# Fireflies-17/Speech-Inpainting

Measured on AMD Instinct MI355X. Metric: real-time factor (audio-sec/wall-sec) per GPU, 4 s clips @16 kHz, 200 ms mask, higher is better.
Workload: dtype encoder GEMMs and attention products: bf16 MFMA, fp32 accumulate (softmax, LayerNorm, head, arg-max in fp32); vocoder: fp16 MFMA (operands rounded to fp16, saturating), fp32 accumulate, activations stored as fp16; 1 GPU; BASELINE configs[1]: batch=32 x 4 s clips per GPU, 200 ms mask, HuBERT-base + HiFi-GAN V1; step = masked log-mel front-end -> encoder -> arg-max/splice -> vocoder on resident raw clips; global_batch=32, clip_samples=64000, mask_frames=10, parallelism=utterance-sharded x1

## Files before the change

### include/si_hip.h

```cpp
#ifndef SI_HIP_H
#define SI_HIP_H

#include <stddef.h>
#include <stdint.h>

#ifdef __cplusplus
extern "C" {
#endif

#define SI_ABI_VERSION 3

enum {
    SI_OK = 0,
    SI_EINVAL = -1,
    SI_ENOMEM = -2,
    SI_EHIP = -3,
    SI_ESTATE = -4,
    SI_EWEIGHTS = -5
};

enum {
    SI_MATH_F32 = 0,
    SI_MATH_BF16 = 1,
    SI_MATH_BF16X3 = 2,
// ... 224 lines not shown
    const int32_t* host_k0;
    const int32_t* host_k1;
    const int32_t* start;
    const int32_t* len;
    const int32_t* span_win;
    const int32_t* span_lim;
    const int32_t* win_ctx;
    const int32_t* win_start;
    const int32_t* win_len;
    const int32_t* chunk;
    const int32_t* k0;
    const int32_t* k1;
    const float* ramp;
} si_region_table;

int si_patch_regions(si_ctx* ctx, const float* orig, int N22, const si_region_table* table, const float* gen, int Lrow, const float* gain,
                     float* out_f32, int16_t* out_pcm, si_stream_t stream);

#define SI_SAMPLE_F32 0
#define SI_SAMPLE_S16 1
#define SI_SAMPLE_S24 2

int si_quiet_runs(si_ctx* ctx, const void* x, int is_pcm16, int n, float threshold, int min_len, int32_t* runs, int max_runs,
                  int32_t* n_runs, si_stream_t stream);

typedef struct si_rate_table {
    int32_t struct_size;
    int32_t num_contexts;
    int32_t num_windows;
    int32_t num_spans;
    int32_t num_chunks;
    int32_t fade;
    const int32_t* host_start;
    const int32_t* host_len;
    const int32_t* host_span_win;
    const int32_t* host_span_lim;
    const int32_t* host_win_ctx;
    const int32_t* host_win_start;
    const int32_t* host_win_len;
    const int32_t* host_win_lim;
    const int32_t* host_chunk;
    const int32_t* host_k0;
    const int32_t* host_k1;
    const int32_t* start;
    const int32_t* len;
    const int32_t* span_win;
    const int32_t* span_lim;
    const int32_t* win_ctx;
    const int32_t* win_start;
    const int32_t* win_len;
    const int32_t* win_lim;
    const int32_t* chunk;
    const int32_t* k0;
    const int32_t* k1;
    const float* ramp;
} si_rate_table;

int si_patch_rate(si_ctx* ctx, const void* orig, int is_pcm16, int n_file, int sr, const si_rate_table* table, const float* gen, int Lrow,
                  const float* gain, const si_sinc_filter* filt, void* out, si_stream_t stream);

#define SI_CUT_RATE_TILE 512
int si_cut_rate(si_ctx* ctx, const void* x, int is_pcm16, int n_file, int sr, const int32_t* host_start, const int32_t* start, int C, int L,
                const si_sinc_filter* filt, float* out, si_stream_t stream);

#define SI_MAX_CHANNELS 8
int si_quiet_runs_ch(si_ctx* ctx, const void* x, int is_pcm16, int n, int channels, int channel, float threshold, int min_len, int32_t* runs,
                     int max_runs, int32_t* n_runs, si_stream_t stream);
int si_cut_rate_ch(si_ctx* ctx, const void* x, int is_pcm16, int n_file, int channels, int channel, int sr, const int32_t* host_start,
                   const int32_t* start, int C, int L, const si_sinc_filter* filt, float* out, si_stream_t stream);
int si_patch_rate_ch(si_ctx* ctx, const void* orig, int is_pcm16, int n_file, int channels, int channel, int sr, const si_rate_table* table,
                     const float* gen, int Lrow, const float* gain, const si_sinc_filter* filt, void* out, si_stream_t stream);

#define SI_CUT_PAIR_FRAMES 1
int si_cut_pair(si_ctx* ctx, const void* x, int is_pcm16, int n_file, int sr, const int32_t* host_frame, const int32_t* frame, int C, int L22,
                int L16, const si_sinc_filter* filt22, const si_sinc_filter* filt16, float* out22, float* out16, si_stream_t stream);
int si_cut_pair_ch(si_ctx* ctx, const void* x, int is_pcm16, int n_file, int channels, int channel, int sr, const int32_t* host_frame,
                   const int32_t* frame, int C, int L22, int L16, const si_sinc_filter* filt22, const si_sinc_filter* filt16, float* out22,
                   float* out16, si_stream_t stream);

#define SI_DEAD_QUIET 1
#define SI_DEAD_HELD 2
int si_dead_runs(si_ctx* ctx, const void* x, int is_pcm16, int n, int channels, int channel, int kind, float threshold, float rel_threshold,
                 float held_tol, int min_len, int32_t* runs, int max_runs, int32_t* n_runs, float* threshold_out, si_stream_t stream);

#define SI_LEVEL_MAX_HALF 1024
int si_level_runs(si_ctx* ctx, const void* x, int is_pcm16, int n, int channels, int channel, int half, float threshold, float rel_threshold,
                  int min_len, int32_t* runs, int max_runs, int32_t* n_runs, float* threshold_out, si_stream_t stream);

int si_burst_runs(si_ctx* ctx, const void* x, int is_pcm16, int n, int channels, int channel, int half, float threshold, float rel_threshold,
                  int min_len, int32_t* runs, int max_runs, int32_t* n_runs, float* threshold_out, si_stream_t stream);

int si_invalid_runs(si_ctx* ctx, const void* x, int is_pcm16, int n, int channels, int channel, float ceiling, int min_len, int32_t* runs,
                    int max_runs, int32_t* n_runs, si_stream_t stream);
int si_cut_rate_valid(si_ctx* ctx, const void* x, int is_pcm16, int n_file, int channels, int channel, int sr, const int32_t* host_start,
                      const int32_t* start, int C, int L, const si_sinc_filter* filt, float ceiling, float* out, si_stream_t stream);
int si_cut_pair_valid(si_ctx* ctx, const void* x, int is_pcm16, int n_file, int channels, int channel, int sr, const int32_t* host_frame,
                      const int32_t* frame, int C, int L22, int L16, const si_sinc_filter* filt22, const si_sinc_filter* filt16, float ceiling,
                      float* out22, float* out16, si_stream_t stream);
int si_cut_clips_valid(si_ctx* ctx, const float* src, int n_src, const int32_t* host_start, const int32_t* start, int C, int L, float ceiling,
                       float* out, si_stream_t stream);

#define SI_IMPULSE_MAX_ORDER 32
#define SI_IMPULSE_MAX_HALF 1024
#define SI_IMPULSE_MAX_GUARD 64
#define SI_IMPULSE_MAX_PAD 16
int si_impulse_runs(si_ctx* ctx, const void* x, int is_pcm16, int n, int channels, int channel, int order, int half, int guard, int pad,
                    float ratio, float threshold, float rel_threshold, int min_len, int32_t* runs, int max_runs, int32_t* n_runs,
                    float* threshold_out, si_stream_t stream);
int si_impulse_residual(si_ctx* ctx, const void* x, int is_pcm16, int n, int channels, int channel, int order, double* e, si_stream_t stream);

#define SI_MEND_MAX_LEN 64
#define SI_MEND_MAX_ORDER 32
#define SI_MEND_MAX_CONTEXT 1024
#define SI_MEND_MAX_RUNS 65536
#define SI_MEND_LONG 0
#define SI_MEND_AR 1
#define SI_MEND_LINE 2
#define SI_MEND_EDGE 3
#define SI_MEND_NEAR 4
#define SI_MEND_NONFINITE 5
#define SI_MEND_BADROW 6
int si_mend_runs(si_ctx* ctx, void* x, int is_pcm16, int n, int channels, int channel, const int32_t* runs, int n_runs, int max_len,
                 int order, int context, int32_t* status, si_stream_t stream);

int si_num_frames(const si_ctx* ctx, int N);
int si_vocoder_samples(const si_ctx* ctx, int Tm, int stretch);

typedef struct si_profile_entry {
    char name[48];
    int32_t launches;
    int32_t reserved;
    double ms;
    double flops;
    double bytes;
} si_profile_entry;
int si_profile_start(si_ctx* ctx, int max_launches);
int si_profile_filter(si_ctx* ctx, const char* family);
int si_profile_stop(si_ctx* ctx, si_profile_entry* out, int capacity, int* count);

int si_debug_capture(si_ctx* ctx, const char* name, float* dst, long capacity);
long si_debug_size(si_ctx* ctx, const char* name);

#define SI_WS_ENCODER 0
#define SI_WS_VOCODER 1
#define SI_WS_MEL 2
#define SI_WS_MAX_REGIONS 32
typedef struct si_ws_region {
    char name[24];
    uint64_t offset;
    uint64_t bytes;
} si_ws_region;
int si_debug_ws_regions(si_ctx* ctx, int which, si_ws_region* out, int capacity, int* count);

#ifdef __cplusplus
}
#endif
#endif
```

### speech_inpainting_amd/csrc/api.hip

```cpp
#include <cmath>
#include <cstdarg>
#include <cstdio>
#include <cstdlib>
#include <cstring>
#include <map>
#include <sstream>
#include <string>
#include <vector>

#include "common.h"

using namespace siw;

struct si_ctx {
    int device = 0;
    si_model_desc d{};
    char err[512] = {0};
    Layout lay;
    char* wdev = nullptr;
    bool weights_ready = false;
    bool weights_verified = false;
    std::map<std::string, long> dbg_size;
    std::map<std::string, std::pair<float*, long>> dbg_capture;
    struct ProfRec { int name; hipEvent_t a, b; double flops, bytes; };
    bool prof_on = false;
    std::string prof_filter;
    std::vector<std::string> prof_names;
    std::vector<ProfRec> prof_recs;
    std::vector<hipEvent_t> prof_pool;
    size_t prof_used = 0;
    int prof_open = -1;
    int num_cus = 0;
    std::map<const void*, size_t> dyn_lds;
    PackOpts popt;
    bool opt_enc_opready = true, opt_att_bf16 = true, opt_enc_lingemm = true;
    bool opt_enc_posconv = true;
    int opt_ln_fuse = 1;
    int opt_voc_upsgemm = 1;
    int opt_ffn_pad = 64;
    int opt_gemmcu = 1;
    int opt_voc_chain = 1;
    int opt_voc_fuse = 1;
    char* fe_dev = nullptr;
    size_t fe_dft = 0, fe_hann = 0, fe_basis = 0, fe_lo = 0, fe_hi = 0;
    std::vector<int32_t> vl_host;
    static constexpr int VL_SLOTS = 4;
    int32_t* vl_pin[VL_SLOTS] = {nullptr, nullptr, nullptr, nullptr};
    size_t vl_pin_ints[VL_SLOTS] = {0, 0, 0, 0};
    hipEvent_t vl_ev[VL_SLOTS] = {nullptr, nullptr, nullptr, nullptr};
    int vl_next = 0;
    float* km_cnorm = nullptr;
    int km_cnorm_cap = 0;
    char* det_scratch = nullptr;
    size_t det_scratch_cap = 0;
    size_t ws_zone = 0;
    struct WsRegion { const char* name; size_t offset, bytes; };
    struct WsLog { int n = 0; WsRegion r[SI_WS_MAX_REGIONS]; };
    WsLog ws_log[3];
};

int si_fail(si_ctx* ctx, int code, const char* fmt, ...) {
    char* dst = ctx ? ctx->err : g_create_err;
    va_list ap;
    va_start(ap, fmt);
    vsnprintf(dst, 512, fmt, ap);
    va_end(ap);
    return code;
}
int si_fail_hip(si_ctx* ctx, hipError_t e, const char* what, const char* file, int line) {
    return si_fail(ctx, SI_EHIP, "HIP error %d (%s) at %s:%d: %s", (int)e, hipGetErrorString(e), file, line, what);
}

struct TapSrc { const void* p; long n; int esize = 4; long cols = 0, ld = 0; };
static int si_tap(si_ctx* ctx, hipStream_t st, TapSrc s, const char* fmt, int a = 0, int b = 0, int c = 0) {
    if (ctx->dbg_capture.empty() && strchr(fmt, '%')) return SI_OK;
    char name[48];
    snprintf(name, sizeof(name), fmt, a, b, c);
    ctx->dbg_size[name] = s.n;
    auto it = ctx->dbg_capture.find(name);
    if (it == ctx->dbg_capture.end()) return SI_OK;
    const long m = s.n < it->second.second ? s.n : it->second.second;
    if (m <= 0) return SI_OK;
    if (s.ld > s.cols && s.cols > 0) {
        if (m / s.cols > 0)
            SI_HIP_CHECK(hipMemcpy2DAsync(it->second.first, (size_t)s.cols * s.esize, s.p, (size_t)s.ld * s.esize, (size_t)s.cols * s.esize,
                                          (size_t)(m / s.cols), hipMemcpyDeviceToDevice, st));
    } else {
        SI_HIP_CHECK(hipMemcpyAsync(it->second.first, s.p, (size_t)m * s.esize, hipMemcpyDeviceToDevice, st));
    }
    return SI_OK;
}

void si_prof_begin(si_ctx* ctx, const char* name, double flops, double bytes, hipStream_t st) {
    if (!ctx->prof_on || ctx->prof_used + 2 > ctx->prof_pool.size()) { ctx->prof_open = -1; return; }
    if (!ctx->prof_filter.empty() && ctx->prof_filter != name) { ctx->prof_open = -1; return; }
    int id = -1;
    for (size_t i = 0; i < ctx->prof_names.size(); ++i) if (ctx->prof_names[i] == name) { id = (int)i; break; }
    if (id < 0) { id = (int)ctx->prof_names.size(); ctx->prof_names.push_back(name); }
    si_ctx::ProfRec r{id, ctx->prof_pool[ctx->prof_used], ctx->prof_pool[ctx->prof_used + 1], flops, bytes};
    ctx->prof_used += 2;
    (void)hipEventRecord(r.a, st);
    ctx->prof_open = (int)ctx->prof_recs.size();
    ctx->prof_recs.push_back(r);
}
const char* si_prof_shape_name(const char* name, long M, int N, int K) {
    static const bool on = getenv("SI_PROF_SHAPES") && atoi(getenv("SI_PROF_SHAPES")) != 0;
    if (!on) return name;
    static thread_local char buf[48];
    snprintf(buf, sizeof(buf), "%s_%ldx%dx%d", name, M, N, K);
    return buf;
}
int si_ensure_dyn_lds(si_ctx* ctx, const void* kern, size_t bytes) {
    if (bytes <= 64 * 1024) return SI_OK;
    size_t& have = ctx->dyn_lds[kern];
    if (bytes > have) {
        SI_HIP_CHECK(hipFuncSetAttribute(kern, hipFuncAttributeMaxDynamicSharedMemorySize, (int)bytes));
        have = bytes;
    }
    return SI_OK;
}
int si_opt_gemmcu(const si_ctx* ctx) { return ctx->opt_gemmcu; }
int si_num_cus(si_ctx* ctx) {
    if (ctx->num_cus <= 0) {
        int n = 0;
        if (hipDeviceGetAttribute(&n, hipDeviceAttributeMultiprocessorCount, ctx->device) != hipSuccess || n <= 0) n = 256;
        ctx->num_cus = n;
    }
    return ctx->num_cus;
}
static int vl_upload(si_ctx* ctx, int32_t* dst, hipStream_t st) {
    const size_t n = ctx->vl_host.size();
    const int slot = ctx->vl_next;
    ctx->vl_next = (slot + 1) % si_ctx::VL_SLOTS;
    if (!ctx->vl_ev[slot]) SI_HIP_CHECK(hipEventCreateWithFlags(&ctx->vl_ev[slot], hipEventDisableTiming));
    else SI_HIP_CHECK(hipEventSynchronize(ctx->vl_ev[slot]));
    if (ctx->vl_pin_ints[slot] < n) {
        if (ctx->vl_pin[slot]) SI_HIP_CHECK(hipHostFree(ctx->vl_pin[slot]));
        ctx->vl_pin[slot] = nullptr; ctx->vl_pin_ints[slot] = 0;
        SI_HIP_CHECK(hipHostMalloc(reinterpret_cast<void**>(&ctx->vl_pin[slot]), std::max<size_t>(n, 4096) * sizeof(int32_t), hipHostMallocDefault));
        ctx->vl_pin_ints[slot] = std::max<size_t>(n, 4096);
    }
    memcpy(ctx->vl_pin[slot], ctx->vl_host.data(), n * sizeof(int32_t));
    SI_HIP_CHECK(hipMemcpyAsync(dst, ctx->vl_pin[slot], n * sizeof(int32_t), hipMemcpyHostToDevice, st));
    SI_HIP_CHECK(hipEventRecord(ctx->vl_ev[slot], st));
    return SI_OK;
}
void si_prof_end(si_ctx* ctx, hipStream_t st) {
    if (ctx->prof_open < 0) return;
    (void)hipEventRecord(ctx->prof_recs[ctx->prof_open].b, st);
    ctx->prof_open = -1;
}

namespace {

int stage_channels(const si_ctx* ctx, int i) { return siw::stage_channels(ctx->d, ctx->popt, i); }
BlobHeader blob_header(const si_ctx* ctx) { return siw::blob_header(ctx->d, ctx->popt, ctx->lay); }
Err ctx_err(si_ctx* ctx) { return ctx ? Err{ctx->err, sizeof(ctx->err)} : Err{g_create_err, sizeof(g_create_err)}; }

inline size_t align_up(size_t v, size_t a) { return (v + a - 1) / a * a; }

struct Carver {
    char* base; size_t cap; size_t zone; si_ctx::WsLog* log; size_t cur; bool ok = true;
    const char* failed = "";
    float* floats(size_t n, const char* name) { return reinterpret_cast<float*>(bytes(n * 4, name)); }
    char* bytes(size_t n, const char* name) {
        size_t o = cur; cur = align_up(cur + n, 256) + zone;
        if (cur > cap || log->n >= SI_WS_MAX_REGIONS) { if (ok) failed = name; ok = false; return base; }
        log->r[log->n++] = {name, o, n};
        return base + o;
    }
};
Carver carver(si_ctx* ctx, int which, void* workspace, size_t workspace_bytes) {
    ctx->ws_log[which].n = 0;
    return Carver{static_cast<char*>(workspace), workspace_bytes, ctx->ws_zone, &ctx->ws_log[which], ctx->ws_zone};
}
constexpr int ENC_WS_ZONES = 18, VOC_WS_ZONES = 15, MEL_WS_ZONES = 5;

struct VlTable { const int32_t* host = nullptr; int32_t* dev = nullptr; };
template <class Fill>
int vl_table(si_ctx* ctx, Carver& W, size_t ints, hipStream_t st, const char* what, VlTable& t, Fill fill) {
    ctx->vl_host.assign(ints, 0);
    if (int rc = fill(ctx->vl_host.data())) return rc;
    t.dev = reinterpret_cast<int32_t*>(W.bytes(ints * 4, "lengths"));
    if (!W.ok) return si_fail(ctx, SI_ENOMEM, "internal: %s workspace carve exceeded its own estimate at region '%s'", what, W.failed);
    if (int rc = vl_upload(ctx, t.dev, st)) return rc;
    t.host = ctx->vl_host.data();
    return SI_OK;
}

struct EncDims { int T; std::vector<int> L; };
EncDims enc_dims(const si_model_desc& d, int N) {
    EncDims e; e.L.push_back(N);
    int n = N;
    for (int i = 0; i < d.num_conv; ++i) { n = n >= d.conv_kernel[i] ? (n - d.conv_kernel[i]) / d.conv_stride[i] + 1 : 0; e.L.push_back(n); }
    e.T = n;
    return e;
}

size_t encoder_ws_bytes(const si_ctx* ctx, int B, int N) {
    const si_model_desc& d = ctx->d;
    EncDims e = enc_dims(d, N);
    size_t cmax = 0;
    for (int i = 0; i < d.num_conv; ++i) cmax = std::max(cmax, (size_t)e.L[i + 1] * d.conv_dim[i]);
    const size_t BT = (size_t)B * std::max(e.T, 1);
    size_t f = 2 * (size_t)B * cmax + BT * d.conv_dim[d.num_conv - 1] + BT * d.hidden_size * 3 + BT * 3 * d.hidden_size + BT * d.intermediate_size +
               (size_t)B * d.conv_dim[0] * 2 + BT * 2;
    const size_t h16 = (BT * d.conv_dim[d.num_conv - 1] + 2 * BT * d.hidden_size + BT * (d.intermediate_size + 128)) * 2;
    return f * 4 + h16 + (size_t)B * 16 + (size_t)B * 4 + si_conv0_partials_bytes(B, N) + 41 * 256 +
           align_up((size_t)(SI_MAX_CONV + 3) * (B + 1) * 4, 256) +
           ENC_WS_ZONES * ctx->ws_zone;
}

int vocoder_chunk(const si_model_desc& d, int B) { int c = d.vocoder_chunk > 0 ? d.vocoder_chunk : 32; return std::min(c, std::max(B, 1)); }

long voc_tout(int Tm, int stretch) { return stretch ? (long)std::floor((double)Tm * (441.0 / 256.0)) : Tm; }

size_t vocoder_ws_bytes(const si_ctx* ctx, int B, int Tm, int stretch) {
    const si_model_desc& d = ctx->d;
    const int Bc = vocoder_chunk(d, B);
    const long Tout = voc_tout(Tm, stretch);
    size_t lc_max = (size_t)Tout * d.up_initial_channel;
    long L = Tout; int c = d.up_initial_channel;
    for (int i = 0; i < d.num_ups; ++i) { L *= d.up_rates[i]; c = stage_channels(ctx, i); lc_max = std::max(lc_max, (size_t)L * c); }
    const size_t f = (size_t)Bc * Tout * ctx->lay.mel_ld + 9 * (size_t)Bc * lc_max;
    return f * 4 + 32 * 256 + align_up((size_t)(2 * SI_MAX_UPS + 3) * B * 4, 256) +
           VOC_WS_ZONES * ctx->ws_zone;
}

TapGemmParams gemm_params(const si_ctx* ctx, const GemmW& G) {
    TapGemmParams p{};
    p.w = ctx->wdev + G.w;
    p.w_lo = G.math == SI_MATH_BF16X3 ? ctx->wdev + G.w_lo : nullptr;
    p.bias = G.has_bias ? reinterpret_cast<const float*>(ctx->wdev + G.bias) : nullptr;
    p.Cin = G.Cin; p.N = G.N; p.Npad = G.Npad; p.ntaps = G.ntaps; p.groups = G.groups;
    p.stride = 1; p.dil = 1; p.pad = 0; p.pro_slope = 1.f; p.act = SI_ACT_NONE; p.alpha = 1.f; p.accumulate = 0;
    p.out16_slope = 1.f;
    p.nseg = 1;
    return p;
}

struct UpsGeom { int u, pad; long Lout; int M; };
UpsGeom ups_geom(const si_model_desc& d, int i, long Lin) {
    const int u = d.up_rates[i], pad = (d.up_kernels[i] - u) / 2;
    const long Lout = Lin * u;
    return UpsGeom{u, pad, Lout, (int)((pad + Lout - 1) / u + 1)};
}

struct ResLn { const float* stats = nullptr; const float* gamma = nullptr; const float* beta = nullptr; };
struct LinearIo { const unsigned short* x16 = nullptr; unsigned short* y16 = nullptr; int ld_in = 0, ld_out = 0; ResLn res_ln; };
int linear(si_ctx* ctx, const GemmW& G, const float* x, float* y, long rows, int act, const float* res, hipStream_t st, const LinearIo& io = LinearIo()) {
    TapGemmParams p = gemm_params(ctx, G);
    p.x = io.x16 ? nullptr : x; p.x16 = io.x16; p.out = y; p.out16 = io.y16; p.res = res; p.act = act;
    p.res_stats = io.res_ln.stats; p.res_gamma = io.res_ln.gamma; p.res_beta = io.res_ln.beta;
    p.nseg = 1; p.Lin = (int)rows; p.M = (int)rows; p.ldx = io.ld_in ? io.ld_in : G.Cin; p.x_seg_stride = 0;
    p.ldo = io.ld_out ? io.ld_out : G.N; p.o_seg_stride = 0; p.ooff = 0; p.olimit = rows * p.ldo;
    p.lingemm = ctx->opt_enc_lingemm;
    return si_launch_tapgemm(ctx, G.math, p, st);
}

const float* wf(const si_ctx* ctx, size_t off) { return reinterpret_cast<const float*>(ctx->wdev + off); }

}

static int hubert_run(si_ctx* ctx, const float* wav, const int32_t* mask_start, const int32_t* mask_len, const int32_t* valid_len,
                      int normalize, float norm_eps, const double* pre_add, int output_layer, int B, int N, float* out_feats, float* out_hidden,
                      void* workspace, size_t workspace_bytes, si_stream_t stream, const int32_t* host_len = nullptr, const SiSpans* spans = nullptr);

static int check_span_table(si_ctx* ctx, const char* who, const si_span_table* t, int B, SiSpans& out) {
    if (!t || t->struct_size != (int32_t)sizeof(si_span_table)) return si_fail(ctx, SI_EINVAL, "%s: si_span_table size mismatch", who);
    if (!t->host_off || !t->span_off) return si_fail(ctx, SI_EINVAL, "%s: span table with NULL offsets", who);
    if (t->num_clips != B) return si_fail(ctx, SI_EINVAL, "%s: span table for %d clips, batch of %d", who, t->num_clips, B);
    if (t->host_off[0] != 0 || t->host_off[B] != t->num_spans || t->num_spans < 0)
        return si_fail(ctx, SI_EINVAL, "%s: span offsets run 0 .. %d but the table holds %d spans", who, t->host_off[B], t->num_spans);
    if (t->num_spans > 0 && (!t->host_start || !t->host_len || !t->span_start || !t->span_len))
        return si_fail(ctx, SI_EINVAL, "%s: span table with NULL start / len", who);
    for (int b = 0; b < B; ++b) {
        const int k0 = t->host_off[b], k1 = t->host_off[b + 1];
        if (k1 < k0 || k1 > t->num_spans) return si_fail(ctx, SI_EINVAL, "%s: span offsets of clip %d decrease or leave the table", who, b);
        if (k1 - k0 > SI_MAX_SPANS) return si_fail(ctx, SI_EINVAL, "%s: clip %d has %d spans, more than SI_MAX_SPANS = %d", who, b, k1 - k0, SI_MAX_SPANS);
        for (int k = k0; k < k1; ++k) {
            const long s = t->host_start[k], l = t->host_len[k];
            if (s < 0 || l < 0 || s + l > 0x7fffffffL) return si_fail(ctx, SI_EINVAL, "%s: clip %d span %d = [%ld, +%ld) is not a sample range", who, b, k - k0, s, l);
            if (k > k0 && s < (long)t->host_start[k - 1] + t->host_len[k - 1])
                return si_fail(ctx, SI_EINVAL, "%s: clip %d span %d overlaps or precedes span %d (spans must be sorted and disjoint)", who, b, k - k0, k - k0 - 1);
        }
    }
    out = SiSpans{t->span_off, t->span_start, t->span_len};
    return SI_OK;
}

extern "C" {

int si_version(void) { return SI_ABI_VERSION; }

const char* si_last_error(const si_ctx* ctx) { return ctx ? ctx->err : g_create_err; }

int si_create(si_ctx** out, int device_id, const si_model_desc* desc) {
    if (!out) return si_fail(nullptr, SI_EINVAL, "si_create: out is NULL");
    *out = nullptr;
    int rc = check_desc(desc, ctx_err(nullptr));
    if (rc) return rc;
    int ndev = 0;
    if (hipGetDeviceCount(&ndev) != hipSuccess || device_id < 0 || device_id >= ndev)
        return si_fail(nullptr, SI_EHIP, "si_create: device %d not available (%d HIP devices visible)", device_id, ndev);
    si_ctx* ctx = new si_ctx();
    ctx->device = device_id;
    ctx->d = *desc;
    ctx->popt = pack_opts_from_env();
    ctx->opt_voc_fuse = getenv("SI_VOC_FUSE") ? atoi(getenv("SI_VOC_FUSE")) : 1;
    ctx->opt_voc_chain = getenv("SI_VOC_CHAIN") ? atoi(getenv("SI_VOC_CHAIN")) : 1;
    ctx->opt_enc_opready = env_flag("SI_ENC_OPREADY");
    ctx->opt_att_bf16 = env_flag("SI_ATT_BF16");
    ctx->opt_enc_lingemm = env_flag("SI_ENC_LINGEMM");
    ctx->opt_enc_posconv = env_flag("SI_ENC_POSCONV");
    ctx->opt_gemmcu = getenv("SI_ENC_GEMMCU") ? atoi(getenv("SI_ENC_GEMMCU")) : 1;
    ctx->opt_ln_fuse = getenv("SI_ENC_LNFUSE") ? atoi(getenv("SI_ENC_LNFUSE")) : 1;
    ctx->opt_voc_upsgemm = getenv("SI_VOC_UPSGEMM") ? atoi(getenv("SI_VOC_UPSGEMM")) : 1;
    ctx->opt_ffn_pad = getenv("SI_ENC_FFNPAD") ? std::min(128, std::max(0, atoi(getenv("SI_ENC_FFNPAD")) / 8 * 8)) : 64;
    ctx->ws_zone = getenv("SI_WS_REDZONE") ? (size_t)std::min(1L << 20, std::max(0L, atol(getenv("SI_WS_REDZONE")))) / 256 * 256 : 0;
    plan_layout(ctx->d, ctx->popt, ctx->lay);
    *out = ctx;
    return SI_OK;
}

void si_destroy(si_ctx* ctx) {
    if (!ctx) return;
    if (ctx->wdev) { (void)hipSetDevice(ctx->device); (void)hipFree(ctx->wdev); }
    if (ctx->fe_dev) { (void)hipSetDevice(ctx->device); (void)hipFree(ctx->fe_dev); }
    if (ctx->km_cnorm) { (void)hipSetDevice(ctx->device); (void)hipFree(ctx->km_cnorm); }
    if (ctx->det_scratch) { (void)hipSetDevice(ctx->device); (void)hipFree(ctx->det_scratch); }
    for (hipEvent_t e : ctx->prof_pool) (void)hipEventDestroy(e);
    for (int i = 0; i < si_ctx::VL_SLOTS; ++i) {
        if (ctx->vl_ev[i]) { (void)hipEventSynchronize(ctx->vl_ev[i]); (void)hipEventDestroy(ctx->vl_ev[i]); }
        if (ctx->vl_pin[i]) (void)hipHostFree(ctx->vl_pin[i]);
    }
    delete ctx;
}

int si_alloc_weights(si_ctx* ctx) {
    if (!ctx) return SI_EINVAL;
    SI_HIP_CHECK(hipSetDevice(ctx->device));
    if (!ctx->wdev) SI_HIP_CHECK(hipMalloc(reinterpret_cast<void**>(&ctx->wdev), ctx->lay.total));
    ctx->weights_ready = true;
    ctx->weights_verified = false;
    return SI_OK;
}

int si_load_weights(si_ctx* ctx, const void* host_blob, size_t nbytes, const char* index) {
    if (!ctx || !host_blob || !index) return si_fail(ctx, SI_EINVAL, "si_load_weights: NULL argument");
    std::vector<char> image;
    int rc = pack_image(ctx->d, ctx->popt, ctx->lay, host_blob, nbytes, index, image, ctx_err(ctx));
    if (rc) return rc;
    SI_HIP_CHECK(hipSetDevice(ctx->device));
    if (!ctx->wdev) SI_HIP_CHECK(hipMalloc(reinterpret_cast<void**>(&ctx->wdev), ctx->lay.total));
    SI_HIP_CHECK(hipMemcpy(ctx->wdev, image.data(), ctx->lay.total, hipMemcpyHostToDevice));
    ctx->weights_ready = true;
    ctx->weights_verified = true;
    return SI_OK;
}

int si_weights_check(si_ctx* ctx) {
    if (!ctx) return SI_EINVAL;
    if (!ctx->wdev) return si_fail(ctx, SI_ESTATE, "weights are not allocated: call si_load_weights or si_alloc_weights first");
    SI_HIP_CHECK(hipSetDevice(ctx->device));
    BlobHeader got{};
    SI_HIP_CHECK(hipMemcpy(&got, ctx->wdev, sizeof(got), hipMemcpyDeviceToHost));
    const BlobHeader want = blob_header(ctx);
    if (got.magic != want.magic || got.version != want.version || got.fingerprint != want.fingerprint || got.total != want.total)
        return si_fail(ctx, SI_EWEIGHTS, "the weight blob in this context was packed for a different layout (fingerprint %016llx / %llu bytes, this "
                       "context plans %016llx / %llu): the source rank's model desc or SI_VOC_* environment differs, or the broadcast has not arrived",
                       (unsigned long long)got.fingerprint, (unsigned long long)got.total, (unsigned long long)want.fingerprint, (unsigned long long)want.total);
    ctx->weights_verified = true;
    return SI_OK;
}

int si_weights_device_ptr(si_ctx* ctx, void** ptr, size_t* nbytes) {
    if (!ctx || !ptr || !nbytes) return si_fail(ctx, SI_EINVAL, "si_weights_device_ptr: NULL argument");
    if (!ctx->wdev) return si_fail(ctx, SI_ESTATE, "weights are not allocated: call si_load_weights or si_alloc_weights first");
    *ptr = ctx->wdev;
    *nbytes = ctx->lay.total;
    return SI_OK;
}

int si_num_frames(const si_ctx* ctx, int N) { return ctx ? enc_dims(ctx->d, N).T : SI_EINVAL; }

int si_vocoder_samples(const si_ctx* ctx, int Tm, int stretch) {
    if (!ctx) return SI_EINVAL;
    long L = voc_tout(Tm, stretch);
    for (int i = 0; i < ctx->d.num_ups; ++i) L *= ctx->d.up_rates[i];
    return (int)L;
}

int si_workspace_bytes(si_ctx* ctx, int B, int N, int Tm, size_t* out) {
    if (!ctx || !out || B <= 0) return si_fail(ctx, SI_EINVAL, "si_workspace_bytes: bad argument");
    size_t a = N > 0 ? encoder_ws_bytes(ctx, B, N) : 0;
    size_t b = Tm > 0 ? vocoder_ws_bytes(ctx, B, Tm, 1) : 0;
    *out = std::max(a, b);
    return SI_OK;
}

int si_hubert_forward(si_ctx* ctx, const float* wav, const int32_t* mask_start, const int32_t* mask_len, int normalize, int B, int N,
                      float* out_feats, void* workspace, size_t workspace_bytes, si_stream_t stream) {
    return si_hubert_forward_padded(ctx, wav, mask_start, mask_len, nullptr, normalize, B, N, out_feats, workspace, workspace_bytes, stream);
}

int si_hubert_forward_padded(si_ctx* ctx, const float* wav, const int32_t* mask_start, const int32_t* mask_len, const int32_t* valid_len,
                             int normalize, int B, int N, float* out_feats, void* workspace, size_t workspace_bytes, si_stream_t stream) {
    if (!ctx) return SI_EINVAL;
    if (!out_feats) return si_fail(ctx, SI_EINVAL, "si_hubert_forward: NULL / empty argument");
    return hubert_run(ctx, wav, mask_start, mask_len, valid_len, normalize, 1e-7f, nullptr, 0, B, N, out_feats, nullptr, workspace,
                      workspace_bytes, stream);
}

int si_hubert_forward_varlen(si_ctx* ctx, const float* wav, const int32_t* mask_start, const int32_t* mask_len, const int32_t* sample_len,
                             int normalize, int B, int N, float* out_feats, void* workspace, size_t workspace_bytes, si_stream_t stream) {
    if (!ctx) return SI_EINVAL;
    if (!out_feats || !sample_len) return si_fail(ctx, SI_EINVAL, "si_hubert_forward_varlen: NULL argument");
    return hubert_run(ctx, wav, mask_start, mask_len, nullptr, normalize, 1e-7f, nullptr, 0, B, N, out_feats, nullptr, workspace, workspace_bytes,
                      stream, sample_len);
}

int si_hubert_extract_features(si_ctx* ctx, const si_extract_desc* x, const float* wav, const int32_t* mask_start, const int32_t* mask_len,
                               const double* pre_mask_add, int B, int N, float* out_hidden, void* workspace, size_t workspace_bytes,
                               si_stream_t stream) {
    if (!ctx) return SI_EINVAL;
    if (!x || x->struct_size != (int32_t)sizeof(si_extract_desc)) return si_fail(ctx, SI_EINVAL, "si_hubert_extract_features: si_extract_desc size mismatch");
    if (!out_hidden) return si_fail(ctx, SI_EINVAL, "si_hubert_extract_features: NULL output");
    if (x->output_layer < 1 || x->output_layer > ctx->d.num_layers)
        return si_fail(ctx, SI_EINVAL, "output_layer %d outside 1..%d", x->output_layer, ctx->d.num_layers);
    if (x->normalize < 0 || x->normalize > 2) return si_fail(ctx, SI_EINVAL, "normalize mode %d unknown (0 none, 1 processor, 2 layer_norm)", x->normalize);
    return hubert_run(ctx, wav, mask_start, mask_len, nullptr, x->normalize != 0, x->normalize == 2 ? 1e-5f : 1e-7f, pre_mask_add,
                      x->output_layer, B, N, nullptr, out_hidden, workspace, workspace_bytes, stream);
}

int si_hubert_forward_spans(si_ctx* ctx, const float* wav, const si_span_table* spans, const int32_t* sample_len, int normalize,
                            int B, int N, float* out_feats, void* workspace, size_t workspace_bytes, si_stream_t stream) {
    if (!ctx) return SI_EINVAL;
    if (!out_feats || B <= 0) return si_fail(ctx, SI_EINVAL, "si_hubert_forward_spans: NULL / empty argument");
    SiSpans sp;
    if (int rc = check_span_table(ctx, "si_hubert_forward_spans", spans, B, sp)) return rc;
    return hubert_run(ctx, wav, nullptr, nullptr, nullptr, normalize, 1e-7f, nullptr, 0, B, N, out_feats, nullptr, workspace, workspace_bytes,
                      stream, sample_len, &sp);
}

int si_code_splice(si_ctx* ctx, const int64_t* code_clean, const int64_t* code_masked, const int32_t* first, const int32_t* last, int B, int T,
                   int64_t* out, si_stream_t stream) {
    if (!ctx) return SI_EINVAL;
    if (!code_clean || !code_masked || !first || !last || !out || B <= 0 || T <= 0) return si_fail(ctx, SI_EINVAL, "si_code_splice: NULL / empty argument");
    SI_HIP_CHECK(hipSetDevice(ctx->device));
    return si_launch_code_splice(ctx, code_clean, code_masked, first, last, B, T, out, static_cast<hipStream_t>(stream));
}

}

static int hubert_run(si_ctx* ctx, const float* wav, const int32_t* mask_start, const int32_t* mask_len, const int32_t* valid_len,
                      int normalize, float norm_eps, const double* pre_add, int output_layer, int B, int N, float* out_feats, float* out_hidden,
                      void* workspace, size_t workspace_bytes, si_stream_t stream, const int32_t* host_len, const SiSpans* spans) {
    if (!ctx->weights_ready) return si_fail(ctx, SI_ESTATE, "si_hubert_forward before weights were loaded");
    if (!ctx->weights_verified) if (int rcw = si_weights_check(ctx)) return rcw;
    if (!wav || !workspace || B <= 0) return si_fail(ctx, SI_EINVAL, "si_hubert_forward: NULL / empty argument");
    const si_model_desc& d = ctx->d;
    const Layout& L = ctx->lay;
    hipStream_t st = static_cast<hipStream_t>(stream);
// ... 408 lines not shown
            int Tc = T, cin = d->in_width;
            for (int i = 0; i < d->down_t; ++i) {
                const int To = (Tc + 2 * ds.pad - ds.k) / d->stride_t + 1;
                macs += (double)B * To * d->width * (double)cin * ds.k + (double)d->depth * B * To * ((double)d->n_state * d->width * 3 + (double)d->width * d->n_state);
                Tc = To; cin = d->width;
            }
            macs += (double)B * Tc * d->out_width * (double)d->width * 3;
            const int frc = si_launch_f0enc_fused(ctx, weights, f0, B, T, h_out, d->in_width, d->out_width, d->width, d->n_state, d->depth, d->down_t,
                                                  d->stride_t, d->dilation_growth, ds.k, ds.pad, macs, st);
            if (frc <= 0) return frc;
        }
    }
    const size_t slot = need / 3 / sizeof(float);
    float* buf[3] = {static_cast<float*>(workspace), static_cast<float*>(workspace) + slot, static_cast<float*>(workspace) + 2 * slot};
    const float* w = weights;
    const float* x = f0;
    int cin = d->in_width, Tc = T, cur = -1;
    int rc;
    for (int i = 0; i < d->down_t; ++i) {
        const int To = (Tc + 2 * ds.pad - ds.k) / d->stride_t + 1;
        const float* cw = w; w += (size_t)d->width * cin * ds.k;
        const float* cb = w; w += d->width;
        const int o = (cur + 1) % 3;
        if ((rc = si_launch_small_conv1d(ctx, x, cw, cb, nullptr, buf[o], B, cin, Tc, d->width, To, ds.k, d->stride_t, 1, ds.pad, 0, 0, st))) return rc;
        cur = o; x = buf[cur]; cin = d->width; Tc = To;
        long dil = 1;
        for (int j = 0; j < d->depth; ++j) {
            const float* w3 = w; w += (size_t)d->n_state * d->width * 3;
            const float* b3 = w; w += d->n_state;
            const float* w1 = w; w += (size_t)d->width * d->n_state;
            const float* b1 = w; w += d->width;
            const int t1 = (cur + 1) % 3, t2 = (cur + 2) % 3;
            if ((rc = si_launch_small_conv1d(ctx, x, w3, b3, nullptr, buf[t1], B, d->width, Tc, d->n_state, Tc, 3, 1, (int)dil, (int)dil, 1, 0, st))) return rc;
            if ((rc = si_launch_small_conv1d(ctx, buf[t1], w1, b1, x, buf[t2], B, d->n_state, Tc, d->width, Tc, 1, 1, 1, 0, 1, 0, st))) return rc;
            cur = t2; x = buf[cur];
            dil *= d->dilation_growth;
            if (dil > (1 << 20)) return si_fail(ctx, SI_EINVAL, "si_f0_encoder_forward: dilation overflow");
        }
    }
    const float* fw = w; w += (size_t)d->out_width * d->width * 3;
    return si_launch_small_conv1d(ctx, x, fw, w, nullptr, h_out, B, d->width, Tc, d->out_width, Tc, 3, 1, 1, 1, 0, 1, st);
}

int si_unit_frontend(si_ctx* ctx, const int64_t* code, int Fc, const int64_t* f0_code, int Fp, const float* spk_emb, const float* emb_c,
                     int Kc, const float* emb_p, int Kp, int E, int B, float* out, si_stream_t stream) {
    if (!ctx) return SI_EINVAL;
    if (!code || !emb_c || !out || B <= 0 || Fc <= 0 || E <= 0 || Kc <= 0) return si_fail(ctx, SI_EINVAL, "si_unit_frontend: NULL / empty argument");
    if (f0_code && (!emb_p || Fp <= 0 || Kp <= 0)) return si_fail(ctx, SI_EINVAL, "si_unit_frontend: f0_code needs its embedding table");
    if (f0_code) {
        const int F = Fp > Fc ? Fp : Fc, s = Fp > Fc ? Fc : Fp;
        if (F % s) return si_fail(ctx, SI_EINVAL, "si_unit_frontend: %d and %d frames: misalignment between condition features", Fc, Fp);
    }
    SI_HIP_CHECK(hipSetDevice(ctx->device));
    return si_launch_unit_frontend(ctx, code, Fc, f0_code, Fp, spk_emb, emb_c, Kc, emb_p, Kp, E, B, out, static_cast<hipStream_t>(stream));
}

int si_resample_poly(si_ctx* ctx, const float* x, int B, int n_in, const float* taps, int ntaps, int up, int down,
                     int pre_remove, int n_out, float* y, si_stream_t stream) {
    if (!ctx) return SI_EINVAL;
    if (!x || !taps || !y || B <= 0 || n_in <= 0) return si_fail(ctx, SI_EINVAL, "si_resample_poly: NULL / empty argument");
    SI_HIP_CHECK(hipSetDevice(ctx->device));
    return si_launch_resample_poly(ctx, x, B, n_in, taps, ntaps, up, down, pre_remove, n_out, y, static_cast<hipStream_t>(stream));
}

static int hifigan_run(si_ctx* ctx, const float* mel, int B, int Tm, int stretch, float* wav_out, void* workspace,
                       size_t workspace_bytes, si_stream_t stream, const int32_t* host_len);

int si_resample_sinc(si_ctx* ctx, const float* x, const int32_t* n_len, int B, int n_in, const si_sinc_filter* f, int n_out, float* y,
                     si_stream_t stream) {
    if (!ctx) return SI_EINVAL;
    if (!x || !y || !f || !f->win || !f->dwin || !f->time_reg || B <= 0 || n_in <= 0) return si_fail(ctx, SI_EINVAL, "si_resample_sinc: NULL / empty argument");
    if (f->struct_size != (int32_t)sizeof(si_sinc_filter)) return si_fail(ctx, SI_EINVAL, "si_resample_sinc: si_sinc_filter size mismatch");
    if (n_out > f->n_time) return si_fail(ctx, SI_EINVAL, "si_resample_sinc: %d outputs but the time-register table holds %d", n_out, f->n_time);
    SI_HIP_CHECK(hipSetDevice(ctx->device));
    return si_launch_resample_sinc(ctx, x, n_len, B, n_in, f->win, f->dwin, f->nwin, f->num_table, f->step, f->scale, f->ratio, f->time_reg, n_out, y,
                                   static_cast<hipStream_t>(stream));
}

int si_extend_mel(si_ctx* ctx, const float* mel, int B, int Tm, float* out, si_stream_t stream) {
    if (!ctx) return SI_EINVAL;
    if (!mel || !out || B <= 0 || Tm <= 0) return si_fail(ctx, SI_EINVAL, "si_extend_mel: NULL / empty argument");
    const long Tout = voc_tout(Tm, 1);
    if (Tout < 1) return si_fail(ctx, SI_EINVAL, "mel of %d frames stretches to nothing", Tm);
    SI_HIP_CHECK(hipSetDevice(ctx->device));
    return si_launch_extend_mel_cf(ctx, mel, B, ctx->d.num_mels, Tm, (int)Tout, out, static_cast<hipStream_t>(stream));
}

int si_pcm16(si_ctx* ctx, const float* wav, int64_t n, int16_t* out, si_stream_t stream) {
    if (!ctx) return SI_EINVAL;
    if (!wav || !out || n < 0) return si_fail(ctx, SI_EINVAL, "si_pcm16: NULL / bad argument");
    SI_HIP_CHECK(hipSetDevice(ctx->device));
    return si_launch_pcm16(ctx, wav, (long)n, out, static_cast<hipStream_t>(stream));
}

int si_hifigan_forward(si_ctx* ctx, const float* mel, int B, int Tm, int stretch, float* wav_out, void* workspace,
                       size_t workspace_bytes, si_stream_t stream) {
    return hifigan_run(ctx, mel, B, Tm, stretch, wav_out, workspace, workspace_bytes, stream, nullptr);
}

int si_hifigan_forward_varlen(si_ctx* ctx, const float* mel, const int32_t* mel_len, int B, int Tm, int stretch, float* wav_out, void* workspace,
                              size_t workspace_bytes, si_stream_t stream) {
    if (!ctx) return SI_EINVAL;
    if (!mel_len) return si_fail(ctx, SI_EINVAL, "si_hifigan_forward_varlen: NULL lengths");
    return hifigan_run(ctx, mel, B, Tm, stretch, wav_out, workspace, workspace_bytes, stream, mel_len);
}

static int hifigan_run(si_ctx* ctx, const float* mel, int B, int Tm, int stretch, float* wav_out, void* workspace,
                       size_t workspace_bytes, si_stream_t stream, const int32_t* host_len) {
    if (!ctx) return SI_EINVAL;
    if (!ctx->weights_ready) return si_fail(ctx, SI_ESTATE, "si_hifigan_forward before weights were loaded");
    if (!ctx->weights_verified) if (int rcw = si_weights_check(ctx)) return rcw;
    if (!mel || !wav_out || !workspace || B <= 0 || Tm <= 0) return si_fail(ctx, SI_EINVAL, "si_hifigan_forward: NULL / empty argument");
    const si_model_desc& d = ctx->d;
    const Layout& Ly = ctx->lay;
    hipStream_t st = static_cast<hipStream_t>(stream);
    const size_t need = vocoder_ws_bytes(ctx, B, Tm, stretch);
    if (workspace_bytes < need) return si_fail(ctx, SI_ENOMEM, "workspace of %zu bytes < %zu needed for B=%d Tm=%d", workspace_bytes, need, B, Tm);
    SI_HIP_CHECK(hipSetDevice(ctx->device));
    const int Bc_max = vocoder_chunk(d, B);
    const long Tout = voc_tout(Tm, stretch);
    if (Tout < 1) return si_fail(ctx, SI_EINVAL, "mel of %d frames stretches to nothing", Tm);
    size_t lc_max = (size_t)Tout * d.up_initial_channel;
    {
        long L = Tout; int c = d.up_initial_channel;
        for (int i = 0; i < d.num_ups; ++i) { L *= d.up_rates[i]; c = stage_channels(ctx, i); lc_max = std::max(lc_max, (size_t)L * c); }
    }
    const long Lwav = si_vocoder_samples(ctx, Tm, stretch);
    Carver W = carver(ctx, SI_WS_VOCODER, workspace, workspace_bytes);
    const bool vl = host_len != nullptr;
    VlTable tab;
    if (vl) {
        if (int trc = vl_table(ctx, W, (size_t)(2 * d.num_ups + 2) * B, st, "vocoder", tab, [&](int32_t* t) -> int {
            for (int b = 0; b < B; ++b) {
                if (host_len[b] < 1 || host_len[b] > Tm) return si_fail(ctx, SI_EINVAL, "ragged batch: clip %d holds %d mel frames, outside 1..%d", b, host_len[b], Tm);
                long Lb = voc_tout(host_len[b], stretch);
                if (Lb < 1) return si_fail(ctx, SI_EINVAL, "ragged batch: clip %d (%d mel frames) stretches to nothing", b, host_len[b]);
                t[b] = host_len[b];
                t[(size_t)B + b] = (int32_t)Lb;
                for (int i = 0; i < d.num_ups; ++i) {
                    const UpsGeom g = ups_geom(d, i, Lb);
                    t[(size_t)(2 + i) * B + b] = (int32_t)g.Lout;
                    t[(size_t)(2 + d.num_ups + i) * B + b] = g.M;
                    Lb = g.Lout;
                }
            }
            return SI_OK;
        })) return trc;
        SI_HIP_CHECK(hipMemsetAsync(wav_out, 0, (size_t)B * Lwav * sizeof(float), st));
    }
    float* ext_ws = W.floats((size_t)Bc_max * Tout * Ly.mel_ld, "ext");
    const size_t nbuf = (size_t)Bc_max * lc_max;
    float* buf_ws[6] = {W.floats(nbuf, "buf0"), W.floats(nbuf, "buf1"), W.floats(nbuf, "buf2"), W.floats(nbuf, "buf3"), W.floats(nbuf, "buf4"), W.floats(nbuf, "buf5")};
    char* const h16_raw[6] = {W.bytes(nbuf * 2, "h16_0"), W.bytes(nbuf * 2, "h16_1"), W.bytes(nbuf * 2, "h16_2"),
                              W.bytes(nbuf * 2, "h16_3"), W.bytes(nbuf * 2, "h16_4"), W.bytes(nbuf * 2, "h16_5")};
    unsigned short* h16_ws[6];
    for (int i = 0; i < 6; ++i) h16_ws[i] = reinterpret_cast<unsigned short*>(h16_raw[i]);
    const bool opr = ctx->popt.voc_opready && (d.vocoder_math == SI_MATH_BF16 || d.vocoder_math == SI_MATH_F16);
    const bool r16 = opr && ctx->popt.voc_res16 && d.vocoder_math == SI_MATH_F16;
    const int fuse_mask = ctx->opt_voc_fuse == 1 ? ~0 : ctx->opt_voc_fuse;
    if (!W.ok) return si_fail(ctx, SI_ENOMEM, "internal: vocoder workspace carve exceeded its own estimate at region '%s'", W.failed);
    const int nk = d.num_rb;
    static const char* upn[] = {"ups0", "ups1", "ups2", "ups3", "ups4", "ups5", "ups6", "ups7"};
    static const char* stn[] = {"stage0", "stage1", "stage2", "stage3", "stage4", "stage5", "stage6", "stage7"};

    auto run = [&](int b0, int Bc, float* ext, float* const* buf, unsigned short* const* h16, hipStream_t st) -> int {
        int rc;
        auto tap16 = [&](const void* src, long n, const char* fmt, int a = 0, int b = 0, int c = 0) -> int {
            return (r16 && !ctx->dbg_capture.empty()) ? si_tap(ctx, st, {src, n, 2}, fmt, a, b, c) : SI_OK;
        };
        auto tap32 = [&](TapSrc s, const char* fmt, int a = 0, int b = 0, int c = 0) -> int {
            return (!r16 && !ctx->dbg_capture.empty()) ? si_tap(ctx, st, s, fmt, a, b, c) : SI_OK;
        };
        const int32_t* dTm = vl ? tab.dev + b0 : nullptr;
        auto dLs = [&](int sidx) -> const int32_t* { return vl ? tab.dev + (size_t)(1 + sidx) * B + b0 : nullptr; };
        auto hLs = [&](int sidx) -> const int32_t* { return vl ? tab.host + (size_t)(1 + sidx) * B + b0 : nullptr; };
        auto rows_of = [&](const int32_t* h, long uniform) { if (!h) return (double)Bc * uniform; double r = 0; for (int b = 0; b < Bc; ++b) r += h[b]; return r; };
        auto stage_conv = [&](const GemmW& G, int sidx, long L, int ld_in, int cin, int dil) {
            TapGemmParams p = gemm_params(ctx, G);
            p.nseg = Bc; p.Lin = (int)L; p.M = (int)L; p.ldx = ld_in; p.x_seg_stride = L * ld_in;
            p.dil = dil; p.pad = dil * (G.ntaps - 1) / 2; p.ldo = G.N; p.o_seg_stride = L * G.N; p.olimit = p.o_seg_stride;
            p.algo_macs = rows_of(hLs(sidx), L) * G.N * (double)cin * G.ntaps;
            if (vl) { p.seg_lin = p.seg_m = p.seg_orows = dLs(sidx); p.olim_mul = p.ldo; p.seg_m_host = hLs(sidx); }
            return p;
        };
        auto ups_desc = [&](int i, long Lc, int c, const float* x, const unsigned short* x16, float* U, unsigned short* U16) {
            const UpsGeom g = ups_geom(d, i, Lc);
            const int cout = stage_channels(ctx, i);
            TapGemmParams p = gemm_params(ctx, Ly.ups[i]);
            p.x = x; p.out = U;
            if (opr) { p.x = nullptr; p.x16 = x16; p.out16 = U16; p.out16_slope = r16 ? 1.f : 0.1f; }
            if (r16) p.out = nullptr;
            p.nseg = Bc; p.Lin = (int)Lc; p.M = g.M; p.ldx = c; p.x_seg_stride = Lc * c;
            p.dil = -1; p.ldo = g.u * cout; p.o_seg_stride = g.Lout * cout; p.ooff = -(long)g.pad * cout; p.olimit = g.Lout * cout;
            p.algo_macs = rows_of(hLs(i), Lc) * (double)(d.up_initial_channel >> i) * (double)(d.up_initial_channel >> (i + 1)) * d.up_kernels[i];
            const size_t mrow = (size_t)(2 + d.num_ups + i) * B + b0;
            if (vl) { p.seg_lin = dLs(i); p.seg_m = tab.dev + mrow; p.seg_orows = dLs(i + 1); p.olim_mul = cout; p.seg_m_host = tab.host + mrow; }
            return p;
        };
        auto ups_takes_activated = [&](int i, long Lc, int c) -> bool {
            if (!r16 || !ctx->opt_voc_upsgemm || i >= d.num_ups || Ly.ups[i].math != SI_MATH_F16 || !Ly.ups[i].has_bias) return false;
            return si_gemmcu_tc_covers(ctx, ups_desc(i, Lc, c, nullptr, h16[0], nullptr, h16[2]), true);
        };
        if ((rc = si_launch_extend_mel(ctx, mel + (size_t)b0 * d.num_mels * Tm, Bc, d.num_mels, Tm, (int)Tout, stretch, ext, Ly.mel_ld, st, dTm, dLs(0)))) return rc;
        float *x = buf[0], *xs = buf[1];
        unsigned short *x16 = h16[0], *xs16 = h16[1], *U16 = h16[2], *t16 = h16[3];
        const float in_slope = (opr && !r16) ? 1.f : 0.1f;
        bool act_in = ups_takes_activated(0, Tout, d.up_initial_channel);
        TapGemmParams pre = stage_conv(Ly.pre, 0, Tout, Ly.mel_ld, d.num_mels, 1);
        pre.x = ext; pre.out = x;
        if (opr) { pre.out16 = x16; pre.out16_slope = (r16 && !act_in) ? 1.f : 0.1f; }
        if (r16) pre.out = nullptr;
        if ((rc = si_launch_tapgemm(ctx, Ly.pre.math, pre, st))) return rc;
        if ((rc = tap16(x16, (long)Bc * Tout * d.up_initial_channel, "pre.f16"))) return rc;
        if ((rc = tap32({x, (long)Bc * Tout * d.up_initial_channel}, "pre"))) return rc;
        long Lc = Tout; int c = d.up_initial_channel;
        for (int i = 0; i < d.num_ups; ++i) {
            const GemmW& G = Ly.ups[i];
            const int cout = stage_channels(ctx, i);
            const long Lo = Lc * d.up_rates[i];
            float* U = buf[2];
            TapGemmParams p = ups_desc(i, Lc, c, x, x16, U, U16);
            bool ups_done = false;
            if (r16 && (fuse_mask & 2) && d.up_rates[i] == 2 && d.up_kernels[i] == 4 &&
                G.has_bias && G.Npad == G.N && G.math == SI_MATH_F16) {
                UpsampleParams q{};
                q.x16 = p.x16; q.w = static_cast<const unsigned short*>(p.w); q.bias = p.bias; q.out16 = p.out16;
                q.B = p.nseg; q.Lin = p.Lin; q.M = p.M; q.Cin = p.ldx; q.N = p.ldo; q.taps = p.ntaps;
                q.ooff = -p.ooff; q.o_clip_stride = p.o_seg_stride; q.o_clip_elems = p.olimit;
                q.lens_lin = p.seg_lin; q.lens_m = p.seg_m; q.lens_m_host = p.seg_m_host;
                rc = si_launch_upsample_stream(ctx, q, st);
                if (rc < 0) return rc;
                ups_done = rc == 0;
            }
            if (!ups_done) {
                p.pro_slope = act_in ? 1.f : in_slope;
                const int urc = act_in ? si_launch_gemmcu_tc(ctx, p, st, true) : 1;
                if (urc < 0) return urc;
                if (urc > 0 && (rc = si_launch_tapgemm(ctx, G.math, p, st))) return rc;
            }
            const long nst = (long)Bc * Lo * cout;
            if (!r16 && (rc = si_tap(ctx, st, {U, nst}, upn[i]))) return rc;
            if ((rc = tap16(U16, nst, "ups%d.f16", i))) return rc;
            const bool act_next = ups_takes_activated(i + 1, Lo, cout);
            struct BlockOut { float alpha; int accumulate; bool copy16; float slope16; };
            auto block_out = [&](int j, bool last) {
                const bool completes = last && j == nk - 1;
                return BlockOut{last ? 1.0f / nk : 1.f, last && j > 0, r16 || !last || (completes && i + 1 < d.num_ups),
                                (r16 && !(completes && act_next)) ? 1.f : 0.1f};
            };
            for (int j = 0; j < nk; ++j) {
                const ResW& R = Ly.rbs[(size_t)i * nk + j];
                const int rk = d.rb_kernels[j];
                const float* y = U;
                const unsigned short* y16 = U16;
                const BlockOut whole = block_out(j, true);
                if (r16 && d.resblock_type != 2 && (fuse_mask & cout) && ctx->opt_voc_chain && d.num_dil == 3 && whole.slope16 == 1.f) {
                    ResChainParams cp{};
                    cp.y16 = U16; cp.out16 = xs16; cp.B = Bc; cp.L = (int)Lo; cp.k = rk; cp.alpha = whole.alpha; cp.accumulate = whole.accumulate;
                    cp.lens = dLs(i + 1); cp.lens_host = hLs(i + 1);
                    for (int n = 0; n < 3; ++n) {
                        const TapGemmParams w1 = gemm_params(ctx, R.c1[n]), w2 = gemm_params(ctx, R.c2[n]);
                        cp.w1[n] = static_cast<const unsigned short*>(w1.w); cp.w2[n] = static_cast<const unsigned short*>(w2.w);
                        cp.b1[n] = w1.bias; cp.b2[n] = w2.bias; cp.dil[n] = d.rb_dilations[j][n];
                    }
                    const int crc = si_launch_reschain(ctx, cout, cp, st);
                    if (crc < 0) return crc;
                    if (crc == 0) {
                        if ((rc = tap16(xs16, nst, "stage%d.rb%d.p%d.f16", i, j, d.num_dil - 1))) return rc;
                        continue;
                    }
                }
                for (int n = 0; n < d.num_dil; ++n) {
                    const int dl = d.rb_dilations[j][n];
                    const bool last = (n == d.num_dil - 1);
                    float* ynext = last ? xs : buf[4 + (n & 1)];
                    unsigned short* ynext16 = last ? xs16 : h16[4 + (n & 1)];
                    const BlockOut o = block_out(j, last);
                    auto residual_conv = [&](const GemmW& G, int dil, float slope, const float* in, const unsigned short* in16) {
                        TapGemmParams q = stage_conv(G, i + 1, Lo, cout, cout, dil);
                        q.x = in; q.out = ynext; q.res = y; q.pro_slope = slope;
                        if (opr) {
                            q.x = nullptr; q.x16 = in16;
                            if (r16) { q.res = nullptr; q.res16 = y16; q.out = nullptr; }
                            if (o.copy16) { q.out16 = ynext16; q.out16_slope = o.slope16; }
                        }
                        q.alpha = o.alpha; q.accumulate = o.accumulate; q.acc16 = r16 && o.accumulate;
                        return si_launch_tapgemm(ctx, G.math, q, st);
                    };
                    if (d.resblock_type == 2) {
                        if ((rc = residual_conv(R.c1[n], dl, in_slope, y, y16))) return rc;
                    } else {
                        int frc = 1;
                        if (r16 && (fuse_mask & cout)) {
                            const TapGemmParams w1 = gemm_params(ctx, R.c1[n]), w2 = gemm_params(ctx, R.c2[n]);
                            frc = si_launch_respair(ctx, cout, y16, ynext16, w1.w, w2.w, w1.bias, w2.bias, Bc, (int)Lo, rk, dl, o.alpha, o.accumulate, st,
                                                    dLs(i + 1), hLs(i + 1), o.slope16);
                            if (frc < 0) return frc;
                        }
                        if (frc > 0) {
                            float* t = buf[3];
                            TapGemmParams p = stage_conv(R.c1[n], i + 1, Lo, cout, cout, dl);
                            p.x = y; p.out = t; p.pro_slope = in_slope;
                            if (opr) { p.x = nullptr; p.x16 = y16; p.out = nullptr; p.out16 = t16; p.out16_slope = 0.1f; }
                            if ((rc = si_launch_tapgemm(ctx, R.c1[n].math, p, st))) return rc;
                            if ((rc = !opr ? tap32({t, nst}, "stage%d.rb%d.t%d", i, j, n)
                                           : tap32({t16, nst, 2}, d.vocoder_math == SI_MATH_F16 ? "stage%d.rb%d.t%d.f16" : "stage%d.rb%d.t%d.bf16", i, j, n))) return rc;
                            if ((rc = residual_conv(R.c2[n], 1, opr ? 1.f : 0.1f, t, t16))) return rc;
                        }
                    }
                    if ((rc = tap16(ynext16, nst, "stage%d.rb%d.p%d.f16", i, j, n))) return rc;
                    if ((rc = tap32({ynext, nst}, "stage%d.rb%d.p%d", i, j, n))) return rc;
                    y = ynext;
                    y16 = ynext16;
                }
            }
            if (!r16 && (rc = si_tap(ctx, st, {xs, nst}, stn[i]))) return rc;
            if ((rc = tap16(xs16, nst, "stage%d.f16", i))) return rc;
            std::swap(x, xs);
            std::swap(x16, xs16);
            Lc = Lo; c = cout; act_in = act_next;
        }
        return si_launch_conv_post(ctx, x, wf(ctx, Ly.post_w), wf(ctx, Ly.post_b), Bc, (int)Lc, c, 7, wav_out + (size_t)b0 * Lwav, st,
                                   r16 ? x16 : nullptr, dLs(d.num_ups), hLs(d.num_ups));
    };

    for (int b0 = 0; b0 < B; b0 += Bc_max) {
        const int Bc = std::min(Bc_max, B - b0);
        if (int rc = run(b0, Bc, ext_ws, buf_ws, h16_ws, st)) return rc;
    }
    return SI_OK;
}

}

namespace {

constexpr int FE_NFFT = 1024, FE_HOP = 441, FE_PAD = 312, FE_NMEL = 80, FE_SR = 22050, FE_NBIN = FE_NFFT / 2 + 1;
constexpr double FE_FMIN = 0.0, FE_FMAX = 8000.0;
constexpr int FE_KC = 528, FE_KS = 512;
constexpr int FE_FRAME = FE_KC + FE_KS;
constexpr int FE_IMOFF = 516;
constexpr int FE_LDSPEC = 1032;

double hz_to_mel(double f) {
    const double f_sp = 200.0 / 3, min_log_hz = 1000.0, min_log_mel = min_log_hz / f_sp, logstep = std::log(6.4) / 27.0;
    return f >= min_log_hz ? min_log_mel + std::log(f / min_log_hz) / logstep : f / f_sp;
}
double mel_to_hz(double m) {
    const double f_sp = 200.0 / 3, min_log_hz = 1000.0, min_log_mel = min_log_hz / f_sp, logstep = std::log(6.4) / 27.0;
    return m >= min_log_mel ? min_log_hz * std::exp(logstep * (m - min_log_mel)) : f_sp * m;
}

size_t fe_round(size_t b) { return (b + 255) / 256 * 256; }

int ensure_frontend(si_ctx* ctx) {
    if (ctx->fe_dev) return SI_OK;
    const int npad = si_round_up(FE_NBIN, si_pick_bn(FE_NBIN));
    ctx->fe_dft = 0;
    ctx->fe_hann = ctx->fe_dft + fe_round((size_t)npad * FE_FRAME * 4);
    ctx->fe_basis = ctx->fe_hann + fe_round((size_t)FE_NFFT * 4);
    ctx->fe_lo = ctx->fe_basis + fe_round((size_t)FE_NBIN * FE_NMEL * 4);
    ctx->fe_hi = ctx->fe_lo + fe_round((size_t)FE_NMEL * 4);
    const size_t total = ctx->fe_hi + fe_round((size_t)FE_NMEL * 4);
    std::vector<char> host(total, 0);
    float* dft = reinterpret_cast<float*>(host.data() + ctx->fe_dft);
    float* hann = reinterpret_cast<float*>(host.data() + ctx->fe_hann);
    float* basis_t = reinterpret_cast<float*>(host.data() + ctx->fe_basis);
    int32_t* lo = reinterpret_cast<int32_t*>(host.data() + ctx->fe_lo);
    int32_t* hi = reinterpret_cast<int32_t*>(host.data() + ctx->fe_hi);
    const double two_pi = 6.283185307179586476925286766559;
    for (int k = 0; k < FE_NFFT; ++k) hann[k] = (float)(0.5 - 0.5 * std::cos(two_pi * k / FE_NFFT));
    float* dsin = dft + (size_t)npad * FE_KC;
    for (int n = 0; n < FE_NBIN; ++n)
        for (int k = 0; k <= FE_NFFT / 2; ++k) {
            const double a = two_pi * ((long)n * k % FE_NFFT) / FE_NFFT;
            dft[(size_t)n * FE_KC + k] = (float)std::cos(a);
            if (k >= 1 && k < FE_NFFT / 2) dsin[(size_t)n * FE_KS + k] = (float)-std::sin(a);
        }
    std::vector<double> mel_f(FE_NMEL + 2);
    const double m0 = hz_to_mel(FE_FMIN), m1 = hz_to_mel(FE_FMAX);
    for (int i = 0; i < FE_NMEL + 2; ++i) mel_f[i] = mel_to_hz(m0 + (m1 - m0) * i / (FE_NMEL + 1));
    for (int i = 0; i < FE_NMEL; ++i) {
        const double enorm = 2.0 / (mel_f[i + 2] - mel_f[i]);
        int first = FE_NBIN, last = -1;
        for (int f = 0; f < FE_NBIN; ++f) {
            const double hz = (double)FE_SR / 2.0 * f / (FE_NBIN - 1);
            const double lower = (hz - mel_f[i]) / (mel_f[i + 1] - mel_f[i]);
            const double upper = (mel_f[i + 2] - hz) / (mel_f[i + 2] - mel_f[i + 1]);
            const double w = std::max(0.0, std::min(lower, upper)) * enorm;
            const float wf32 = (float)w;
            basis_t[(size_t)f * FE_NMEL + i] = wf32;
            if (wf32 != 0.f) { first = std::min(first, f); last = f; }
        }
        lo[i] = last < 0 ? 0 : first;
        hi[i] = last < 0 ? 0 : last + 1;
    }
    SI_HIP_CHECK(hipSetDevice(ctx->device));
    char* dev = nullptr;
    SI_HIP_CHECK(hipMalloc(reinterpret_cast<void**>(&dev), total));
    hipError_t e = hipMemcpy(dev, host.data(), total, hipMemcpyHostToDevice);
    if (e != hipSuccess) { (void)hipFree(dev); return si_fail_hip(ctx, e, "front-end table upload", __FILE__, __LINE__); }
    ctx->fe_dev = dev;
    return SI_OK;
}

size_t mel_ws_bytes(const si_ctx* ctx, int B, int N22) {
    const long Tm = (N22 + 2 * FE_PAD - FE_NFFT) / FE_HOP + 1;
    if (Tm < 1) return 0;
    return fe_round((size_t)B * 4) + fe_round((size_t)B * Tm * FE_FRAME * 4) + fe_round((size_t)B * Tm * FE_LDSPEC * 4) + 256 +
           fe_round((size_t)2 * B * 4) +
           MEL_WS_ZONES * ctx->ws_zone;
}

}

extern "C" {

int si_mel_frames(int n22) { return n22 + 2 * FE_PAD < FE_NFFT ? 0 : (n22 + 2 * FE_PAD - FE_NFFT) / FE_HOP + 1; }

int si_mel_workspace_bytes(si_ctx* ctx, int B, int N22, size_t* out) {
    if (!ctx || !out || B <= 0 || si_mel_frames(N22) < 1) return si_fail(ctx, SI_EINVAL, "si_mel_workspace_bytes: bad argument");
    *out = mel_ws_bytes(ctx, B, N22);
    return SI_OK;
}

static int mel_run(si_ctx* ctx, const float* wave22, const int32_t* mask_start, const int32_t* mask_end, int normalize, int B,
                   int N22, float* mel_out, void* workspace, size_t workspace_bytes, si_stream_t stream, const int32_t* host_len,
                   const SiSpans* spans = nullptr);

// ... 739 lines not shown
```

### speech_inpainting_amd/csrc/common.h

```cpp
#pragma once
#include <hip/hip_runtime.h>
#include <stdint.h>

#include <type_traits>

#include "../../include/si_hip.h"
#include "weights_host.h"

#define SI_HIP_CHECK(expr)                                                                      \
    do {                                                                                        \
        hipError_t _e = (expr);                                                                 \
        if (_e != hipSuccess) return si_fail_hip(ctx, _e, #expr, __FILE__, __LINE__);           \
    } while (0)

int si_fail_hip(si_ctx* ctx, hipError_t e, const char* what, const char* file, int line);
int si_fail(si_ctx* ctx, int code, const char* fmt, ...);
void si_prof_begin(si_ctx* ctx, const char* name, double flops, double bytes, hipStream_t st);
void si_prof_end(si_ctx* ctx, hipStream_t st);
const char* si_prof_shape_name(const char* name, long M, int N, int K);
int si_ensure_dyn_lds(si_ctx* ctx, const void* kern, size_t bytes);
int si_num_cus(si_ctx* ctx);

typedef unsigned short bf16_t;

struct SiS24 {
    uint8_t b[3];
    SiS24() = default;
    __host__ __device__ explicit SiS24(int v) : b{(uint8_t)v, (uint8_t)(v >> 8), (uint8_t)(v >> 16)} {}
    __host__ __device__ int value() const { return (int)((unsigned)b[0] << 8 | (unsigned)b[1] << 16 | (unsigned)b[2] << 24) >> 8; }
};
static_assert(sizeof(SiS24) == 3 && alignof(SiS24) == 1, "SiS24 is three packed bytes");

inline int si_sample_format(int is_pcm16) { return is_pcm16 == SI_SAMPLE_S24 ? SI_SAMPLE_S24 : is_pcm16 != 0 ? SI_SAMPLE_S16 : SI_SAMPLE_F32; }
inline double si_sample_bytes(int fmt) { return fmt == SI_SAMPLE_S24 ? 3.0 : fmt == SI_SAMPLE_S16 ? 2.0 : 4.0; }
template <class F>
inline void si_with_sample(int fmt, F&& f) {
    if (fmt == SI_SAMPLE_S24) f(static_cast<const SiS24*>(nullptr));
    else if (fmt == SI_SAMPLE_S16) f(static_cast<const int16_t*>(nullptr));
    else f(static_cast<const float*>(nullptr));
}

__device__ __forceinline__ bool si_invalid(float v, float c) { return !(__builtin_fabsf(v) <= __builtin_fminf(c, __FLT_MAX__)); }
__device__ __forceinline__ bool si_invalid(int16_t v, float c) { const int a = v; return !((float)(a < 0 ? -a : a) <= c); }
__device__ __forceinline__ bool si_invalid(SiS24 v, float c) { const int a = v.value(); return !((float)(a < 0 ? -a : a) <= c); }

struct SiVlTile { int b, row0, L; };
#ifdef __HIPCC__
__device__ __forceinline__ SiVlTile si_vl_tile(const int32_t* __restrict__ lens, int B, int step, int t) {
    const int lane = (int)__builtin_amdgcn_mbcnt_hi(~0u, __builtin_amdgcn_mbcnt_lo(~0u, 0u));
    int base = 0;
    for (int s0 = 0; s0 < B; s0 += 64) {
        const int s = s0 + lane;
        const int Lb = s < B ? lens[s] : 0;
        const int nb = Lb > 0 ? (Lb + step - 1) / step : 0;
        int incl = nb;
#pragma unroll
        for (int o = 1; o < 64; o <<= 1) {
            const int v = __shfl_up(incl, o, 64);
            if (lane >= o) incl += v;
        }
        const int tot = __shfl(incl, 63, 64);
        if (t < base + tot) {
            const unsigned long long m = __ballot(base + incl > t);
            const int l = (int)__builtin_ctzll(m);
            SiVlTile r;
            r.b = s0 + l;
            r.row0 = (t - base - __shfl(incl - nb, l, 64)) * step;
            r.L = __shfl(Lb, l, 64);
            return r;
        }
        base += tot;
    }
    return SiVlTile{B, 0, 0};
}
#endif
static inline long si_vl_tiles(const int32_t* lens, int B, int step) {
    long n = 0;
    for (int b = 0; b < B; ++b) if (lens[b] > 0) n += (lens[b] + step - 1) / step;
    return n;
}

enum { SI_ACT_NONE = 0, SI_ACT_GELU = 1 };

struct TapGemmParams {
    const float* x;
    const unsigned short* x16;
    const void* w;
    const void* w_lo;
    const float* bias;
    const float* res;
    const float* res_stats; const float* res_gamma; const float* res_beta;
    const unsigned short* res16;
    int acc16;
    float* out;
    unsigned short* out16;
    float out16_slope;
    int nseg, Lin, M;
    int ldx;
    long x_seg_stride;
    int Cin;
    int N, Npad;
    int ntaps, stride, dil, pad;
    int groups;
    int ldo;
    long o_seg_stride;
    long ooff;
    long olimit;
    float pro_slope;
    int act;
    float alpha;
    int accumulate;
    double algo_macs;
    int wide_epilogue;
    int lingemm;
    const int32_t* seg_lin;
    const int32_t* seg_m;
    const int32_t* seg_orows;
    int olim_mul;
    const int32_t* seg_row_off;
    const int32_t* seg_m_host;
};


int si_launch_tapgemm(si_ctx* ctx, int math, const TapGemmParams& p, hipStream_t st);

struct LinGemmParams {
    const unsigned short* x16; int x_bytes;
    int lda; long x_seg_stride;
    int nseg, M, K;
    const unsigned short* w; int w_bytes;
    int N, Cin, ntaps; long w_tap_stride;
    const float* bias; const float* res;
    const float* res_stats; const float* res_gamma; const float* res_beta;
    float* out; unsigned short* out16;
    int ldo; long o_seg_stride;
    int act;
    int xcd_rows;
    const int32_t* seg_m;
    const int32_t* seg_m_host;
    int tc_dil, tc_rows_in; float tc_slope; long tc_ooff, tc_olimit;
    const int32_t* tc_seg_lin; const int32_t* tc_seg_orows; int tc_olim_mul;
};
int si_launch_lingemm(si_ctx* ctx, const LinGemmParams& p, hipStream_t st);
int si_launch_gemmcu(si_ctx* ctx, const LinGemmParams& p, hipStream_t st);
int si_launch_gemmcu_tc(si_ctx* ctx, const TapGemmParams& p, hipStream_t st, bool always = false);
bool si_gemmcu_tc_covers(si_ctx* ctx, const TapGemmParams& p, bool always = false);
int si_opt_gemmcu(const si_ctx* ctx);

struct WaveNormParams {
    const float* wav;
    const int32_t* mask_start;
    const int32_t* mask_len;
    int B, N, L1;
    int C, K, S;
    int normalize;
// ... 57 lines not shown

int si_launch_codebook_splice(si_ctx* ctx, const float* feats, int B, int T, int D, const si_cb_frames& fr, const float* cb_centered ,
                              const float* cb_raw , const float* cb_rnorm , int K, float* mel, int Tm, int64_t* labels,
                              hipStream_t st);

int si_launch_code_splice(si_ctx* ctx, const int64_t* clean, const int64_t* masked, const int32_t* first, const int32_t* last, int B, int T,
                          int64_t* out, hipStream_t st);

int si_launch_codebook_gather(si_ctx* ctx, const int64_t* labels, int B, int D, const si_cb_frames& fr, const float* cb_raw, int K, float* mel,
                              int Tm, hipStream_t st);

int si_launch_kmeans_assign(si_ctx* ctx, const float* x, long rows, int D, const float* cent, int K, int64_t* labels, float* dist,
                            hipStream_t st, float* cnorm_scratch = nullptr);

int si_launch_codebook_metrics(si_ctx* ctx, const float* feats, int B, int T, int D, const si_cb_frames& fr, const float* cb_centered,
                               const float* cb_rnorm, int K, const int64_t* target, float* terms, float* loss, int64_t* pred, float* cos_pt,
                               hipStream_t st);

int si_launch_mel_metrics(si_ctx* ctx, const float* a, const float* b, int B, int D, int L, const float* center, float* out, hipStream_t st);
int si_launch_sisdr(si_ctx* ctx, const float* est, const float* ref, int B, int n, float* out, hipStream_t st);

int si_launch_wave_peak(si_ctx* ctx, const float* wav, const int32_t* ms, const int32_t* me, int B, int N, float* peak,
                        hipStream_t st, const int32_t* n_len = nullptr, const SiSpans* sp = nullptr );
int si_launch_mel_frames(si_ctx* ctx, const float* wav, const int32_t* ms, const int32_t* me, const float* peak,
                         const float* hann, int B, int N, int Tm, int hop, int pad, int nfft, int kc, int normalize, float* frames,
                         hipStream_t st, const int32_t* n_len = nullptr, const int32_t* tm_len = nullptr, const SiSpans* sp = nullptr);
int si_launch_mel_project(si_ctx* ctx, const float* spec, int ld_spec, int nbin, int im_off, const float* basis_t, const int32_t* lo,
                          const int32_t* hi, int nmel, int B, int Tm, float* mel, hipStream_t st, const int32_t* tm_len = nullptr);

int si_launch_resample_poly(si_ctx* ctx, const float* x, int B, int n_in, const float* taps, int ntaps, int up, int down,
                            int pre_remove, int n_out, float* y, hipStream_t st);

int si_launch_resample_sinc(si_ctx* ctx, const float* x, const int32_t* n_len, int B, int n_in, const double* win, const double* dwin, int nwin,
                            int num_table, int step, double scale, double ratio, const double* time_reg, int n_out, float* y, hipStream_t st);
int si_launch_pcm16(si_ctx* ctx, const float* wav, long n, int16_t* out, hipStream_t st);

struct SiPatch { const int32_t* win_start; const int32_t* win_len; const int32_t* span_win; const int32_t* lim; const float* ramp; int fade; };
int si_launch_gather_windows(si_ctx* ctx, const float* ext, const int32_t* win, int W, int D, int Tout, int Wmax, float* out, hipStream_t st);
int si_launch_patch_compose(si_ctx* ctx, const float* orig, const SiSpans& sp, const SiPatch& pt, const float* gen, int Lrow, const float* gain,
                            int B, int N22, float* out, int16_t* pcm, hipStream_t st);
int si_launch_cut_clips(si_ctx* ctx, const float* src, const int32_t* start, int C, int L, float* out, hipStream_t st);
struct SiRegions {
    const int32_t* start; const int32_t* len; const int32_t* span_win; const int32_t* span_lim;
    const int32_t* win_ctx; const int32_t* win_start; const int32_t* chunk; const int32_t* k0; const int32_t* k1;
    const float* ramp; int fade;
};
int si_launch_patch_regions(si_ctx* ctx, const float* orig, const SiRegions& rt, int Q, const float* gen, int Lrow, const float* gain,
                            int N22, float* out, int16_t* pcm, hipStream_t st);

size_t si_detect_scratch_bytes(int n);
enum SiDetRoute {
    SI_DET_QUIET,
    SI_DET_DEAD,
    SI_DET_LEVEL,
    SI_DET_BURST,
    SI_DET_INVALID,
    SI_DET_IMPULSE,
};
struct SiDetect {
    int route;
    float rel;
    float* thr_out;
    int half;
    int kind;
    float tol;
    float ceiling;
    int order, guard, pad;
    float ratio;
};
int si_launch_detect(si_ctx* ctx, const void* x, int fmt, int n, int channels, int channel, float thr, int min_len, int32_t* runs, int max_runs,
                     int32_t* n_runs, char* scratch, hipStream_t st, SiDetect d);
int si_launch_impulse_residual(si_ctx* ctx, const void* x, int fmt, int n, int channels, int channel, int order, double* e, hipStream_t st);

struct SiRate {
    const int32_t* start; const int32_t* len; const int32_t* span_win; const int32_t* span_lim;
    const int32_t* win_ctx; const int32_t* win_start; const int32_t* win_len; const int32_t* win_lim;
    const int32_t* chunk; const int32_t* k0; const int32_t* k1;
    const float* ramp; int fade;
    const double* win; const double* dwin; int nwin, num_table, step; double scale;
    int P, Q, H, row_cap;
};
int si_launch_patch_rate(si_ctx* ctx, const void* orig, int fmt, int n_file, const SiRate& rt, int num_chunks, const float* gen, int Lrow,
                         const float* gain, void* out, hipStream_t st);
int si_launch_patch_rate_ch(si_ctx* ctx, const void* orig, int fmt, int n_file, int ch, int channel, const SiRate& rt, int num_chunks,
                            const float* gen, int Lrow, const float* gain, void* out, hipStream_t st);

constexpr int RF_TILE = SI_CUT_RATE_TILE;
struct SiFeed {
    const double* win; const double* dwin; int nwin, num_table, step; double scale;
    int P, Q, H, cap, N22;
};
int si_launch_cut_rate(si_ctx* ctx, const void* x, int fmt, int n_file, const int32_t* start, int C, int L, const SiFeed& fd, float* out,
                       hipStream_t st);
int si_launch_cut_rate_ch(si_ctx* ctx, const void* x, int fmt, int n_file, int ch, int channel, const int32_t* start, int C, int L,
                          const SiFeed& fd, float* out, hipStream_t st);

constexpr int RF_PAIR_FRAMES = SI_CUT_PAIR_FRAMES;
struct SiPairRate {
    const double* win; const double* dwin; int nwin, num_table, step; double scale;
    int P, Q, H;
};
struct SiPair {
    SiPairRate r22, r16;
    int cap, N22, N16, lim16, direct16;
};
int si_launch_cut_pair(si_ctx* ctx, const void* x, int fmt, int n_file, int ch, int channel, const int32_t* frame, int C, int L22, int L16,
                       const SiPair& pr, float* out22, float* out16, hipStream_t st);

int si_launch_cut_rate_valid(si_ctx* ctx, const void* x, int fmt, int n_file, int ch, int channel, const int32_t* start, int C, int L,
                             const SiFeed& fd, float ceiling, float* out, hipStream_t st);
int si_launch_cut_pair_valid(si_ctx* ctx, const void* x, int fmt, int n_file, int ch, int channel, const int32_t* frame, int C, int L22,
                             int L16, const SiPair& pr, float ceiling, float* out22, float* out16, hipStream_t st);
int si_launch_cut_clips_valid(si_ctx* ctx, const float* src, const int32_t* start, int C, int L, float ceiling, float* out, hipStream_t st);

int si_launch_mend_runs(si_ctx* ctx, void* x, int fmt, int n, int ch, int channel, const int32_t* runs, int n_runs, int max_len, int order,
                        int context, int32_t* status, hipStream_t st);

__device__ __forceinline__ float si_gelu_fast(float x) {
    const float z = x * 0.70710678118654752440f;
    const float az = __builtin_fabsf(z);
    const float t = __builtin_amdgcn_rcpf(fmaf(0.3275911f, az, 1.0f));
    float poly = fmaf(1.061405429f, t, -1.453152027f);
    poly = fmaf(poly, t, 1.421413741f);
    poly = fmaf(poly, t, -0.284496736f);
    poly = fmaf(poly, t, 0.254829592f);
    poly *= t;
    const float e = __builtin_amdgcn_exp2f(-az * az * 1.4426950408889634f);
    const float erf = __builtin_copysignf(fmaf(-poly, e, 1.0f), z);
    return 0.5f * x * (1.0f + erf);
}

__device__ __forceinline__ float si_ln_apply(float x, float mean, float rstd, float g, float b) { return fmaf((x - mean) * rstd, g, b); }

__device__ __forceinline__ float si_lrelu01(float v) {
    float r;
    asm("v_max_f32 %0, %1, %2" : "=v"(r) : "v"(v), "v"(0.1f * v));
    return r;
}

struct UpsampleParams {
    const unsigned short* x16;
    const unsigned short* w;
    const float* bias;
    unsigned short* out16;
    int B, Lin, M;
    int Cin, N, taps;
    long ooff;
    long o_clip_stride, o_clip_elems;
    const int32_t* lens_lin; const int32_t* lens_m; const int32_t* lens_m_host;
    int total_tiles;
};
int si_launch_upsample_stream(si_ctx* ctx, const UpsampleParams& p, hipStream_t st);

struct ResPairParams {
    const unsigned short* y16;
    unsigned short* out16;
    const unsigned short* w1;
    const unsigned short* w2;
    const float* b1;
    const float* b2;
    int B, L, k, dil;
    float alpha;
    int accumulate;
    const int32_t* lens; const int32_t* lens_host;
    int total_tiles;
    float out_slope;
};
int si_launch_respair_wide(si_ctx* ctx, int C, const ResPairParams& p, hipStream_t st);
struct ResChainParams {
    const unsigned short* y16;
    unsigned short* out16;
    const unsigned short* w1[3];
    const unsigned short* w2[3];
    const float* b1[3];
    const float* b2[3];
    int B, L, k;
    int dil[3];
    float alpha;
    int accumulate;
    const int32_t* lens; const int32_t* lens_host;
    int total_tiles;
};
int si_launch_reschain(si_ctx* ctx, int C, const ResChainParams& p, hipStream_t st);
int si_launch_respair(si_ctx* ctx, int C, const unsigned short* y16, unsigned short* out16, const void* w1, const void* w2,
                      const float* b1, const float* b2, int B, int L, int k, int dil, float alpha, int accumulate, hipStream_t st,
                      const int32_t* lens = nullptr, const int32_t* lens_host = nullptr, float out_slope = 1.f);

int si_launch_extend_mel(si_ctx* ctx, const float* mel, int B, int D, int Tm, int Tout, int stretch, float* out, int ldo,
                         hipStream_t st, const int32_t* tm_len = nullptr, const int32_t* tout_len = nullptr);
int si_launch_extend_mel_cf(si_ctx* ctx, const float* mel, int B, int D, int Tm, int Tout, float* out, hipStream_t st);
int si_launch_small_conv1d(si_ctx* ctx, const float* x, const float* w, const float* bias, const float* res, float* y, int B, int Cin,
                           int Tin, int Cout, int Tout, int K, int stride, int dil, int pad, int relu_in, int channels_last, hipStream_t st);
int si_launch_f0enc_fused(si_ctx* ctx, const float* weights, const float* f0, int B, int T, float* h_out, int in_width, int out_width, int width,
                          int n_state, int depth, int down_t, int stride_t, int growth, int dk, int dpad, double macs, hipStream_t st);
int si_launch_unit_frontend(si_ctx* ctx, const int64_t* code, int Fc, const int64_t* f0_code, int Fp, const float* spk_emb,
                            const float* emb_c, int Kc, const float* emb_p, int Kp, int E, int B, float* out, hipStream_t st);
int si_launch_conv_post(si_ctx* ctx, const float* x, const float* w , const float* bias, int B, int L, int C, int k,
                        float* wav, hipStream_t st, const unsigned short* x16 = nullptr ,
                        const int32_t* lens = nullptr, const int32_t* lens_host = nullptr);
```

### speech_inpainting_amd/csrc/respair.hip

```cpp
#include <algorithm>
#include <cstdio>
#include <cstdlib>
#include <type_traits>

#include "common.h"

typedef float f32x4 __attribute__((ext_vector_type(4)));
typedef unsigned int u32x4 __attribute__((ext_vector_type(4)));
typedef unsigned int u32x2 __attribute__((ext_vector_type(2)));
typedef _Float16 f16x8 __attribute__((ext_vector_type(8)));
typedef _Float16 f16x4 __attribute__((ext_vector_type(4)));

constexpr int RPN_HALO = 50;

template <int ROWB>
__device__ __forceinline__ int rpn_swz(int row) {
    if constexpr (ROWB == 128) return (row & 7) << 4;
    else return ((row >> 1) & 3) << 4;
}

template <int C, int R1, int WARPS_M, int TPS, bool ACC, bool VL>
__global__ __launch_bounds__(64 * WARPS_M, 2) void respair_kernel(const ResPairParams p) {
    static_assert(R1 == WARPS_M * 64 && (C == 32 || C == 64), "64-row wave tiles over all C channels");
    constexpr int NT = 64 * WARPS_M;
    constexpr int ROWB = C * 2;
    constexpr int ROWBO = C * 4;
    constexpr int CPR = C / 8;
    constexpr int KS = C / 32;
    constexpr int TN = C / 16;
    constexpr int YPAD = C == 64 ? 32 : 0;
    constexpr int YS = ROWB + YPAD;
    constexpr int YBYTES = (R1 + RPN_HALO) * YS;
    constexpr int WBYTES = TPS * C * ROWB;
    constexpr int WSLOTS = (WBYTES / 16 + NT - 1) / NT;
    constexpr int YRPP = NT / CPR;
    constexpr int YSLOTS = (R1 + RPN_HALO + YRPP - 1) / YRPP;
    constexpr int OXM = (C / 4 - 1) < 15 ? (C / 4 - 1) : 15;
    static_assert(R1 * ROWBO <= YBYTES + 2 * WBYTES, "the output image reuses the operand region (not the biases behind it)");

    __builtin_amdgcn_s_setreg((0 << 11) | (23 << 6) | 1, 1);
    extern __shared__ __attribute__((aligned(16))) char smem[];
    char* const Ys = smem;
    char* const Ws = smem + YBYTES;
    float* const Bs = reinterpret_cast<float*>(smem + YBYTES + 2 * WBYTES);

    const int tid = threadIdx.x, lane = tid & 63, wave = tid >> 6;
    const int r16 = lane & 15, kg = lane >> 4;
    const int wm0 = wave * 64;
    const int k = p.k, d = p.dil;
    const int p1 = d * (k - 1) / 2, p2 = (k - 1) / 2;
    const int BMo = R1 - (k - 1);
    const int R0 = R1 + (k - 1) * d;
    const int tiles_x = (p.L + BMo - 1) / BMo;
    const int total = VL ? p.total_tiles : tiles_x * p.B;
    auto tile_of = [&](int t, int& tb, int& tm0, int& tL) {
        if constexpr (VL) { const SiVlTile v = si_vl_tile(p.lens, p.B, BMo, t); tb = v.b; tm0 = v.row0; tL = v.L; }
        else { tb = t / tiles_x; tm0 = (t - tb * tiles_x) * BMo; tL = p.L; }
    };
    const __amdgpu_buffer_rsrc_t w1rsrc = __builtin_amdgcn_make_buffer_rsrc(const_cast<unsigned short*>(p.w1), 0, k * C * C * 2, 0x00020000);
    const __amdgpu_buffer_rsrc_t w2rsrc = __builtin_amdgcn_make_buffer_rsrc(const_cast<unsigned short*>(p.w2), 0, k * C * C * 2, 0x00020000);

    const int NS1 = (k + TPS - 1) / TPS, NS = 2 * NS1;
    u32x4 rw[WSLOTS];
    auto issueW = [&](int s) {
        const bool second = s >= NS1;
        const int soff = __builtin_amdgcn_readfirstlane((second ? s - NS1 : s) * WBYTES);
#pragma unroll
        for (int i = 0; i < WSLOTS; ++i)
            rw[i] = __builtin_amdgcn_raw_buffer_load_b128(second ? w2rsrc : w1rsrc, (tid + i * NT) * 16, soff, 0);
    };
    auto storeW = [&](char* dst) {
#pragma unroll
        for (int i = 0; i < WSLOTS; ++i) {
            const int q = tid + i * NT;
            if (WBYTES / 16 % NT == 0 || q < WBYTES / 16) {
                const int r = q / CPR, c = q - r * CPR;
                *reinterpret_cast<u32x4*>(dst + r * ROWB + ((c << 4) ^ rpn_swz<ROWB>(r))) = rw[i];
            }
        }
    };

    const int yc = tid % CPR, yr0 = tid / CPR;
    u32x4 ry[YSLOTS];
    auto issueY = [&](int t) {
        int tb, tm0, tL;
        tile_of(t, tb, tm0, tL);
        const int trow0 = tm0 - p2 - p1;
        const __amdgpu_buffer_rsrc_t rs = __builtin_amdgcn_make_buffer_rsrc(const_cast<unsigned short*>(p.y16 + (long)tb * p.L * C), 0, tL * C * 2, 0x00020000);
#pragma unroll
        for (int i = 0; i < YSLOTS; ++i)
            ry[i] = __builtin_amdgcn_raw_buffer_load_b128(rs, ((trow0 + yr0 + i * YRPP) * C + 8 * yc) * 2, 0, 0);
    };

    issueW(0);
    issueY(blockIdx.x);
    if (tid < C / 2) {
        const int which = tid / (C / 4), c4 = (tid % (C / 4)) * 4;
        *reinterpret_cast<f32x4*>(Bs + which * C + c4) = *reinterpret_cast<const f32x4*>((which ? p.b2 : p.b1) + c4);
    }

  for (int tile = blockIdx.x; tile < total; tile += gridDim.x) {
    const int nxt = tile + (int)gridDim.x < total ? tile + (int)gridDim.x : tile;
    int b, m0, Lb;
    tile_of(tile, b, m0, Lb);
    const int t_row0 = m0 - p2;
    const long seg = (long)b * p.L * C;
    const __amdgpu_buffer_rsrc_t yrsrc = __builtin_amdgcn_make_buffer_rsrc(const_cast<unsigned short*>(p.y16 + seg), 0, Lb * C * 2, 0x00020000);
    const __amdgpu_buffer_rsrc_t orsrc = __builtin_amdgcn_make_buffer_rsrc(p.out16 + seg, 0, Lb * C * 2, 0x00020000);

    storeW(Ws);
    issueW(1);
#pragma unroll
    for (int i = 0; i < YSLOTS; ++i) {
        const int r = yr0 + i * YRPP;
        if ((i + 1) * YRPP <= R1 || r < R0) {
            f16x8 h = __builtin_bit_cast(f16x8, ry[i]);
            h = __builtin_elementwise_max(h, h * (_Float16)0.1f);
            *reinterpret_cast<f16x8*>(Ys + r * YS + (YPAD ? yc << 4 : (yc << 4) ^ rpn_swz<ROWB>(r))) = h;
        }
    }
    __syncthreads();

    f32x4 acc[4][TN];
    auto init_acc = [&](const float* bias) {
#pragma unroll
        for (int j = 0; j < TN; ++j) {
            const f32x4 bv = *reinterpret_cast<const f32x4*>(bias + 16 * j + 4 * kg);
#pragma unroll
            for (int i = 0; i < 4; ++i) acc[i][j] = bv;
        }
    };
    init_acc(Bs);
    const int lin0 = (wm0 + r16) * YS + (kg << 4);
    int preW[KS];
#pragma unroll
    for (int ks = 0; ks < KS; ++ks) preW[ks] = r16 * ROWB + (rpn_swz<ROWB>(r16) ^ (kg << 4) ^ (ks * 64));
    auto compute = [&](int tap0, bool second, int ntap, const char* Wc) {
        const int nsteps = ntap * KS;
        auto load = [&](f16x8 (&y)[4], f16x8 (&w)[TN], int q, const int ks) {
            const int tl = KS == 1 ? q : q >> 1;
            const int soff = (second ? tap0 + tl : (tap0 + tl) * d) * YS + ks * 64;
            const int lin = lin0 + soff;
            const char* yp = Ys + (YPAD ? lin : lin ^ ((lin >> 3) & 0x30));
#pragma unroll
            for (int i = 0; i < 4; ++i) y[i] = *reinterpret_cast<const f16x8*>(yp + i * (16 * YS));
            const char* wp = Wc + tl * (C * ROWB) + preW[ks];
#pragma unroll
            for (int j = 0; j < TN; ++j) w[j] = *reinterpret_cast<const f16x8*>(wp + j * (16 * ROWB));
        };
        auto mma = [&](const f16x8 (&y)[4], const f16x8 (&w)[TN]) {
#pragma unroll
            for (int i = 0; i < 4; ++i)
#pragma unroll
                for (int j = 0; j < TN; ++j) acc[i][j] = __builtin_amdgcn_mfma_f32_16x16x32_f16(w[j], y[i], acc[i][j], 0, 0, 0);
        };
        f16x8 ya[4], wa[TN], yb[4], wb[TN];
        load(ya, wa, 0, 0);
        for (int q = 0; q < nsteps; q += 2) {
            load(yb, wb, q + 1 < nsteps ? q + 1 : nsteps - 1, KS - 1);
            __builtin_amdgcn_sched_barrier(0);
            __builtin_amdgcn_s_setprio(1);
            mma(ya, wa);
            __builtin_amdgcn_s_setprio(0);
            __builtin_amdgcn_sched_barrier(0);
            load(ya, wa, q + 2 < nsteps ? q + 2 : nsteps - KS, 0);
            __builtin_amdgcn_sched_barrier(0);
            if (q + 1 < nsteps) {
                __builtin_amdgcn_s_setprio(1);
                mma(yb, wb);
                __builtin_amdgcn_s_setprio(0);
            }
            __builtin_amdgcn_sched_barrier(0);
        }
    };

    for (int s = 0; s < NS; ++s) {
        const bool second = s >= NS1;
        const int q = second ? s - NS1 : s;
        const int tap0 = q * TPS;
        if (s == NS - 1) {
            issueW(0);
            if constexpr (!ACC) issueY(nxt);
        }
        compute(tap0, second, min(TPS, k - tap0), Ws + (s & 1) * WBYTES);
        if (s == NS1 - 1) {
            __syncthreads();
            auto epi1 = [&](auto edge_tag) {
                constexpr bool EDGE = decltype(edge_tag)::value;
#pragma unroll
            for (int ip = 0; ip < 2; ++ip) {
                float inside[2];
#pragma unroll
                for (int u = 0; u < 2; ++u) {
                    const int grow = t_row0 + wm0 + 16 * (2 * ip + u) + r16;
                    inside[u] = (!EDGE || (grow >= 0 && grow < Lb)) ? 1.f : 0.f;
                }
                const int ms = wm0 + 16 * (2 * ip + (kg & 1)) + r16;
#pragma unroll
                for (int j = 0; j < TN; ++j) {
                    u32x2 pk[2];
#pragma unroll
                    for (int u = 0; u < 2; ++u) {
                        f16x4 hv;
#pragma unroll
                        for (int e = 0; e < 4; ++e) hv[e] = (_Float16)(EDGE ? si_lrelu01(acc[2 * ip + u][j][e]) * inside[u] : si_lrelu01(acc[2 * ip + u][j][e]));
                        pk[u] = __builtin_bit_cast(u32x2, hv);
                    }
#pragma unroll
                    for (int q = 0; q < 2; ++q) {
                        const auto r = __builtin_amdgcn_permlane16_swap(pk[0][q], pk[1][q], false, false);
                        pk[0][q] = r[0]; pk[1][q] = r[1];
                    }
                    const int ch = 2 * j + (kg >> 1);
                    *reinterpret_cast<u32x4*>(Ys + ms * YS + (YPAD ? ch << 4 : (ch << 4) ^ rpn_swz<ROWB>(ms))) = u32x4{pk[0][0], pk[0][1], pk[1][0], pk[1][1]};
                }
            }
            };
            if (t_row0 >= 0 && t_row0 + R1 <= Lb) epi1(std::false_type{});
            else epi1(std::true_type{});
            init_acc(Bs + C);
        }
        if (s + 1 < NS) {
            storeW(Ws + ((s + 1) & 1) * WBYTES);
            if (s + 2 < NS) issueW(s + 2);
        }
        __syncthreads();
    }

    constexpr int ORPP = NT / CPR;
    constexpr int OPASS = R1 / ORPP;
    const int c8 = tid % CPR, or0 = tid / CPR;
    u32x4 res[OPASS], prev[ACC ? OPASS : 1];
    int goff[OPASS];
#pragma unroll
    for (int it = 0; it < OPASS; ++it) {
        const int o = or0 + it * ORPP;
        const int grow = m0 + o;
        goff[it] = (o < BMo && grow < Lb) ? (grow * C + 8 * c8) * 2 : (int)0x80000000;
        res[it] = __builtin_amdgcn_raw_buffer_load_b128(yrsrc, goff[it], 0, 0);
        if constexpr (ACC) prev[it] = __builtin_amdgcn_raw_buffer_load_b128(orsrc, goff[it], 0, 0);
    }
#pragma unroll
    for (int i = 0; i < 4; ++i) {
        const int m = wm0 + 16 * i + r16;
#pragma unroll
        for (int j = 0; j < TN; ++j) {
            const int co = 4 * j + kg;
            *reinterpret_cast<f32x4*>(smem + m * ROWBO + ((co ^ (m & OXM)) << 4)) = acc[i][j];
        }
    }
    __syncthreads();
    {
#pragma unroll
        for (int it = 0; it < OPASS; ++it) {
            const int o = or0 + it * ORPP;
            const f32x4 a0 = *reinterpret_cast<const f32x4*>(smem + o * ROWBO + (((2 * c8) ^ (o & OXM)) << 4));
            const f32x4 a1 = *reinterpret_cast<const f32x4*>(smem + o * ROWBO + (((2 * c8 + 1) ^ (o & OXM)) << 4));
            const f16x8 rh = __builtin_bit_cast(f16x8, res[it]);
            f16x8 ph = {};
            if constexpr (ACC) ph = __builtin_bit_cast(f16x8, prev[it]);
            f16x8 out;
#pragma unroll
            for (int e = 0; e < 8; ++e) {
                const float a = e < 4 ? a0[e] : a1[e - 4];
                float v = (a + (float)rh[e]) * p.alpha;
                if constexpr (ACC) v += (float)ph[e];
                out[e] = (_Float16)v;
            }
            __builtin_amdgcn_raw_buffer_store_b128(__builtin_bit_cast(u32x4, out), orsrc, goff[it], 0, 0);
        }
    }
    if constexpr (ACC) issueY(nxt);
    __syncthreads();
  }
}

template <int C, int R1, int WARPS_M, int TPS>
static int respair_launch(si_ctx* ctx, const ResPairParams& p, hipStream_t st) {
    const int BMo = R1 - (p.k - 1);
    const size_t lds = (size_t)(R1 + RPN_HALO) * (C * 2 + (C == 64 ? 32 : 0)) + 2 * (size_t)TPS * C * C * 2 + 2 * (size_t)C * 4;
    const bool vl = p.lens != nullptr;
    auto kern = vl ? (p.accumulate ? respair_kernel<C, R1, WARPS_M, TPS, true, true> : respair_kernel<C, R1, WARPS_M, TPS, false, true>)
                   : (p.accumulate ? respair_kernel<C, R1, WARPS_M, TPS, true, false> : respair_kernel<C, R1, WARPS_M, TPS, false, false>);
    if (int rc = si_ensure_dyn_lds(ctx, reinterpret_cast<const void*>(kern), lds)) return rc;
    const int total = vl ? (int)si_vl_tiles(p.lens_host, p.B, BMo) : ((p.L + BMo - 1) / BMo) * p.B;
    if (total <= 0) return SI_OK;
    ResPairParams pk = p;
    pk.total_tiles = total;
    const int grid = std::min(total, si_num_cus(ctx) * (WARPS_M == 4 ? 2 : 1));
    char name[48];
    snprintf(name, sizeof(name), p.accumulate ? "respair_f16_c%d_acc" : "respair_f16_c%d", C);
    double rows = (double)p.B * p.L;
    if (vl) { rows = 0; for (int b = 0; b < p.B; ++b) rows += p.lens_host[b]; }
    const double elems = rows * C;
    si_prof_begin(ctx, name, 2.0 * 2.0 * elems * C * p.k, elems * (2.0 + 2.0 + (p.accumulate ? 2.0 : 0.0)) + 2.0 * 2.0 * p.k * C * C, st);
    hipLaunchKernelGGL(kern, dim3(grid), dim3(64 * WARPS_M), lds, st, pk);
    si_prof_end(ctx, st);
    SI_HIP_CHECK(hipGetLastError());
    return SI_OK;
}

int si_launch_respair(si_ctx* ctx, int C, const unsigned short* y16, unsigned short* out16, const void* w1, const void* w2,
                      const float* b1, const float* b2, int B, int L, int k, int dil, float alpha, int accumulate, hipStream_t st,
                      const int32_t* lens, const int32_t* lens_host, float out_slope) {
    if ((C != 32 && C != 64 && C != 128 && C != 256) || k < 3 || k > 11 || (k & 1) == 0 || (k - 1) * dil > 50 ||
        ((long)L + 1024) * C * 2 >= (1L << 31)) return 1;
    if (!b1 || !b2) return 1;
    if ((lens == nullptr) != (lens_host == nullptr)) return si_fail(ctx, SI_EINVAL, "respair: ragged batches need the lengths on the device and on the host");
    ResPairParams p{y16, out16, static_cast<const unsigned short*>(w1), static_cast<const unsigned short*>(w2), b1, b2, B, L, k, dil, alpha, accumulate, lens, lens_host, 0, out_slope};
    if (out_slope != 1.f && C < 128) return 1;
    if (C >= 128) return si_launch_respair_wide(ctx, C, p, st);
    return C == 32 ? respair_launch<32, 256, 4, 11>(ctx, p, st) : respair_launch<64, 512, 8, 4>(ctx, p, st);
}
```

### speech_inpainting_amd/csrc/respair_wide.hip

```cpp
#include <algorithm>
#include <cstdio>
#include <cstdlib>

#include "common.h"

typedef float f32x4 __attribute__((ext_vector_type(4)));
typedef unsigned int u32x4 __attribute__((ext_vector_type(4)));
typedef unsigned int u32x2 __attribute__((ext_vector_type(2)));
typedef _Float16 f16x8 __attribute__((ext_vector_type(8)));
typedef _Float16 f16x4 __attribute__((ext_vector_type(4)));

template <int ROWB>
__device__ __forceinline__ int swz16(int row) {
    if constexpr (ROWB >= 256) return (row & 7) << 5;
    else return ((row >> 1) & 3) << 5;
}

#ifdef RPW_TIMELINE
__device__ unsigned long long rpw_tl[2][10];
#define RPW_TL_DECL unsigned long long tl_t = wall_clock64(); unsigned long long tl_acc[6] = {0, 0, 0, 0, 0, 0}; unsigned long long tl_tiles = 0; unsigned long long tl_w = 0, tl_sub[2] = {0, 0};
#define RPW_TL_W0 tl_w = wall_clock64();
#define RPW_TL_W1(q) tl_sub[q] += wall_clock64() - tl_w;
#define RPW_TL(ph) { const unsigned long long n_ = wall_clock64(); tl_acc[ph] += n_ - tl_t; tl_t = n_; }
#define RPW_TL_TILE ++tl_tiles;
#define RPW_TL_FLUSH if (threadIdx.x == 0) { for (int q_ = 0; q_ < 6; ++q_) atomicAdd(&rpw_tl[C == 256][q_], tl_acc[q_]); atomicAdd(&rpw_tl[C == 256][6], tl_tiles); atomicAdd(&rpw_tl[C == 256][7], 1ull); atomicAdd(&rpw_tl[C == 256][8], tl_sub[0]); atomicAdd(&rpw_tl[C == 256][9], tl_sub[1]); }
extern "C" int si_debug_rpw_timeline(unsigned long long* out, int reset) {
    if (hipMemcpyFromSymbol(out, HIP_SYMBOL(rpw_tl), sizeof(rpw_tl)) != hipSuccess) return -1;
    if (reset) { unsigned long long z[2][10] = {}; if (hipMemcpyToSymbol(HIP_SYMBOL(rpw_tl), z, sizeof(z)) != hipSuccess) return -1; }
    return 0;
}
#else
#define RPW_TL_DECL
#define RPW_TL_W0
#define RPW_TL_W1(q)
#define RPW_TL(ph)
#define RPW_TL_TILE
#define RPW_TL_FLUSH
#endif

constexpr int RPW_HALO = 50;

template <int C, int R1, int WARPS_M, int WARPS_N, int BKW, bool ACC, bool VL>
__global__ __launch_bounds__(64 * WARPS_M * WARPS_N, 2) void respair_wide_kernel(const ResPairParams p) {
    static_assert((WARPS_M * WARPS_N == 8 || WARPS_M * WARPS_N == 4) && R1 == WARPS_M * 64 && C == WARPS_N * 64, "64 x 64 wave tiles");
    static_assert(BKW == 128 || BKW == 64, "weight-slab depth");
    constexpr int NT = 64 * WARPS_M * WARPS_N;
    constexpr int ROWBY = C * 2;
    constexpr int ROWBW = BKW * 2;
    constexpr int ROWBO = C * 4;
    constexpr int CPRY = C / 8, CPRW = BKW / 8;
    constexpr int NCH = C / BKW;
    constexpr int KS = BKW / 32;
    constexpr int YBYTES = (R1 + RPW_HALO) * ROWBY;
    constexpr int WBYTES = C * ROWBW;
    constexpr int WSLOTS = C * CPRW / NT;
    constexpr int YSLOTS = ((R1 + RPW_HALO) * CPRY + NT - 1) / NT;
    constexpr int YRPP = NT / CPRY, WRPP = NT / CPRW;
    static_assert(C * CPRW % NT == 0 && NT % CPRY == 0 && NT % CPRW == 0, "staging maps");
    static_assert(R1 * ROWBO <= YBYTES + 2 * WBYTES, "the output image reuses the operand region (not the biases behind it)");

    __builtin_amdgcn_s_setreg((0 << 11) | (23 << 6) | 1, 1);
    extern __shared__ __attribute__((aligned(16))) char smem[];
    char* const Ys = smem;
    char* const Ws = smem + YBYTES;
    float* const Bs = reinterpret_cast<float*>(smem + YBYTES + 2 * WBYTES);

    const int tid = threadIdx.x, lane = tid & 63, wave = tid >> 6;
    const int r16 = lane & 15, kg = lane >> 4;
    const int wm0 = (wave / WARPS_N) * 64, wn0 = (wave % WARPS_N) * 64;
    const int k = p.k, d = p.dil;
    const int p1 = d * (k - 1) / 2, p2 = (k - 1) / 2;
    const int BMo = R1 - (k - 1);
    const int R0 = R1 + (k - 1) * d;
    const int tiles_x = (p.L + BMo - 1) / BMo;
    const int total = VL ? p.total_tiles : tiles_x * p.B;
    auto tile_of = [&](int t, int& tb, int& tm0, int& tL) {
        if constexpr (VL) { const SiVlTile v = si_vl_tile(p.lens, p.B, BMo, t); tb = v.b; tm0 = v.row0; tL = v.L; }
        else { tb = t / tiles_x; tm0 = (t - tb * tiles_x) * BMo; tL = p.L; }
    };
    const __amdgpu_buffer_rsrc_t w1rsrc = __builtin_amdgcn_make_buffer_rsrc(const_cast<unsigned short*>(p.w1), 0, k * C * C * 2, 0x00020000);
    const __amdgpu_buffer_rsrc_t w2rsrc = __builtin_amdgcn_make_buffer_rsrc(const_cast<unsigned short*>(p.w2), 0, k * C * C * 2, 0x00020000);

    const int NS1 = k * NCH, NS = 2 * NS1;
    const int wc = tid % CPRW, wr0 = tid / CPRW;
    u32x4 rw[WSLOTS];
    auto issueW1 = [&](int s, int i) {
        const bool second = s >= NS1;
        const int q = second ? s - NS1 : s;
        const int tap = q / NCH, ch = q - tap * NCH;
        const int soff = __builtin_amdgcn_readfirstlane((tap * C * C + ch * BKW) * 2);
        const int n = wr0 + i * WRPP;
        rw[i] = __builtin_amdgcn_raw_buffer_load_b128(second ? w2rsrc : w1rsrc, (n * C + 8 * wc) * 2, soff, 0);
    };
    auto issueW = [&](int s) {
#pragma unroll
        for (int i = 0; i < WSLOTS; ++i) issueW1(s, i);
    };
    auto storeW1 = [&](char* dst, int i) {
        const int n = wr0 + i * WRPP;
        *reinterpret_cast<u32x4*>(dst + n * ROWBW + ((wc << 4) ^ swz16<ROWBW>(n))) = rw[i];
    };
    auto storeW = [&](char* dst) {
#pragma unroll
        for (int i = 0; i < WSLOTS; ++i) storeW1(dst, i);
    };
    const int yc = tid % CPRY, yr0 = tid / CPRY;
    u32x4 ry[YSLOTS];
    auto issueY = [&](int t) {
        int tb, tm0, tL;
        tile_of(t, tb, tm0, tL);
        const int trow0 = tm0 - p2 - p1;
        const __amdgpu_buffer_rsrc_t rs = __builtin_amdgcn_make_buffer_rsrc(const_cast<unsigned short*>(p.y16 + (long)tb * p.L * C), 0, tL * C * 2, 0x00020000);
#pragma unroll
        for (int i = 0; i < YSLOTS; ++i)
            ry[i] = __builtin_amdgcn_raw_buffer_load_b128(rs, ((trow0 + yr0 + i * YRPP) * C + 8 * yc) * 2, 0, 0);
    };

    if (tid < C / 2) {
        const int which = tid / (C / 4), c4 = (tid % (C / 4)) * 4;
        *reinterpret_cast<f32x4*>(Bs + which * C + c4) = *reinterpret_cast<const f32x4*>((which ? p.b2 : p.b1) + c4);
    }
    const int preW = (wn0 + r16) * ROWBW + (swz16<ROWBW>(wn0 + r16) ^ (kg << 4));
    issueW(0);
    issueY(blockIdx.x);
    RPW_TL_DECL

  for (int tile = blockIdx.x; tile < total; tile += gridDim.x) {
    const int nxt = tile + (int)gridDim.x < total ? tile + (int)gridDim.x : tile;
    int b, m0, Lb;
    tile_of(tile, b, m0, Lb);
    const int t_row0 = m0 - p2;
    const long seg = (long)b * p.L * C;
    const __amdgpu_buffer_rsrc_t yrsrc = __builtin_amdgcn_make_buffer_rsrc(const_cast<unsigned short*>(p.y16 + seg), 0, Lb * C * 2, 0x00020000);
    const __amdgpu_buffer_rsrc_t orsrc = __builtin_amdgcn_make_buffer_rsrc(p.out16 + seg, 0, Lb * C * 2, 0x00020000);

    storeW(Ws);
    issueW(1);
#pragma unroll
    for (int i = 0; i < YSLOTS; ++i) {
        const int r = yr0 + i * YRPP;
        if ((i + 1) * YRPP <= R1 || r < R0) {
            f16x8 h = __builtin_bit_cast(f16x8, ry[i]);
            h = __builtin_elementwise_max(h, h * (_Float16)0.1f);
            *reinterpret_cast<f16x8*>(Ys + r * ROWBY + ((yc << 4) ^ swz16<ROWBY>(r))) = h;
        }
    }
    __syncthreads();
    RPW_TL(0)

    f32x4 acc[4][4];
    auto init_acc = [&](const float* bias) {
#pragma unroll
        for (int j = 0; j < 4; ++j) {
            const f32x4 bv = *reinterpret_cast<const f32x4*>(bias + wn0 + 16 * j + 4 * kg);
#pragma unroll
            for (int i = 0; i < 4; ++i) acc[i][j] = bv;
        }
    };
    init_acc(Bs);
    auto compute = [&](int roff, int cb16, const char* Wc, auto&& hook) {
        const int r0 = wm0 + r16 + roff;
        const int preY = r0 * ROWBY + (swz16<ROWBY>(r0) ^ (kg << 4));
        auto load = [&](f16x8 (&y)[4], f16x8 (&w)[4], int ks) {
            const char* yp = Ys + (preY ^ (cb16 + ks * 64));
            const char* wp = Wc + (preW ^ (ks * 64));
#pragma unroll
            for (int i = 0; i < 4; ++i) y[i] = *reinterpret_cast<const f16x8*>(yp + i * (16 * ROWBY));
#pragma unroll
            for (int j = 0; j < 4; ++j) w[j] = *reinterpret_cast<const f16x8*>(wp + j * (16 * ROWBW));
        };
        auto mma = [&](const f16x8 (&y)[4], const f16x8 (&w)[4]) {
#pragma unroll
            for (int i = 0; i < 4; ++i)
#pragma unroll
                for (int j = 0; j < 4; ++j) acc[i][j] = __builtin_amdgcn_mfma_f32_16x16x32_f16(w[j], y[i], acc[i][j], 0, 0, 0);
        };
        f16x8 ya[4], wa[4], yb[4], wb[4];
        load(ya, wa, 0);
#pragma unroll
        for (int ks = 0; ks < KS; ks += 2) {
            load(yb, wb, ks + 1);
            __builtin_amdgcn_sched_barrier(0);
            __builtin_amdgcn_s_setprio(1);
            mma(ya, wa);
            __builtin_amdgcn_s_setprio(0);
            __builtin_amdgcn_sched_barrier(0);
            hook(ks);
            if (ks + 2 < KS) load(ya, wa, ks + 2);
            __builtin_amdgcn_sched_barrier(0);
            __builtin_amdgcn_s_setprio(1);
            mma(yb, wb);
            __builtin_amdgcn_s_setprio(0);
            __builtin_amdgcn_sched_barrier(0);
            hook(ks + 1);
        }
    };

    int tap = 0, ch = 0;
    for (int s = 0; s < NS - 1; ++s) {
        const bool second = s >= NS1;
        char* const Wn = Ws + ((s + 1) & 1) * WBYTES;
        static_assert(WSLOTS % KS == 0, "the slab's stores are spread evenly over its k-steps");
        compute(second ? tap : tap * d, ch * (BKW * 2), Ws + (s & 1) * WBYTES, [&](int ks) {
            const int s2 = s + 2 < NS ? s + 2 : NS - 1;
#pragma unroll
            for (int i = 0; i < WSLOTS / KS; ++i) {
                storeW1(Wn, ks * (WSLOTS / KS) + i);
                issueW1(s2, ks * (WSLOTS / KS) + i);
            }
        });
        if (s == NS1 - 1) {
            __syncthreads();
            RPW_TL(1)
#pragma unroll
            for (int ip = 0; ip < 2; ++ip) {
                float inside[2];
#pragma unroll
                for (int u = 0; u < 2; ++u) {
                    const int grow = t_row0 + wm0 + 16 * (2 * ip + u) + r16;
                    inside[u] = (grow >= 0 && grow < Lb) ? 1.f : 0.f;
                }
                const int ms = wm0 + 16 * (2 * ip + (kg & 1)) + r16;
#pragma unroll
                for (int j = 0; j < 4; ++j) {
                    u32x2 pk[2];
#pragma unroll
                    for (int u = 0; u < 2; ++u) {
                        f16x4 hv;
#pragma unroll
                        for (int e = 0; e < 4; ++e) hv[e] = (_Float16)(si_lrelu01(acc[2 * ip + u][j][e]) * inside[u]);
                        pk[u] = __builtin_bit_cast(u32x2, hv);
                    }
#pragma unroll
                    for (int q = 0; q < 2; ++q) {
                        const auto r = __builtin_amdgcn_permlane16_swap(pk[0][q], pk[1][q], false, false);
                        pk[0][q] = r[0]; pk[1][q] = r[1];
                    }
                    const int ch = ((wn0 + 16 * j) >> 3) + (kg >> 1);
                    *reinterpret_cast<u32x4*>(Ys + ms * ROWBY + ((ch << 4) ^ swz16<ROWBY>(ms))) = u32x4{pk[0][0], pk[0][1], pk[1][0], pk[1][1]};
                }
            }
            init_acc(Bs + C);
            RPW_TL(2)
        }
        if (++ch == NCH) { ch = 0; if (++tap == k) tap = 0; }
        __syncthreads();
    }
    if constexpr (!ACC) issueY(nxt);
    __builtin_amdgcn_sched_barrier(0);
    compute(tap, ch * (BKW * 2), Ws + ((NS - 1) & 1) * WBYTES, [](int) {});
    RPW_TL(3)
    constexpr int ORPP = NT / CPRY;
    constexpr int OPASS = R1 / ORPP;
    const int c8 = tid % CPRY, or0 = tid / CPRY;
    u32x4 res[OPASS], prev[ACC ? OPASS : 1];
    int goff[OPASS];
#pragma unroll
    for (int it = 0; it < OPASS; ++it) {
        const int o = or0 + it * ORPP;
        const int grow = m0 + o;
        goff[it] = (o < BMo && grow < Lb) ? (grow * C + 8 * c8) * 2 : (int)0x80000000;
        res[it] = __builtin_amdgcn_raw_buffer_load_b128(yrsrc, goff[it], 0, 0);
        if constexpr (ACC) prev[it] = __builtin_amdgcn_raw_buffer_load_b128(orsrc, goff[it], 0, 0);
    }
    RPW_TL_W0
    __syncthreads();
    RPW_TL_W1(0)
    RPW_TL_W0

#pragma unroll
    for (int i = 0; i < 4; ++i) {
        const int m = wm0 + 16 * i + r16;
#pragma unroll
        for (int j = 0; j < 4; ++j) {
            const int co = ((wn0 + 16 * j) >> 2) + kg;
            *reinterpret_cast<f32x4*>(smem + m * ROWBO + ((co ^ (m & 15)) << 4)) = acc[i][j];
        }
    }
    RPW_TL_W1(1)
    __syncthreads();
    RPW_TL(4)
    issueW(0);
    {
        const bool oact = p.out_slope != 0.f && p.out_slope != 1.f;
#pragma unroll
        for (int it = 0; it < OPASS; ++it) {
            const int o = or0 + it * ORPP;
            const f32x4 a0 = *reinterpret_cast<const f32x4*>(smem + o * ROWBO + (((2 * c8) ^ (o & 15)) << 4));
            const f32x4 a1 = *reinterpret_cast<const f32x4*>(smem + o * ROWBO + (((2 * c8 + 1) ^ (o & 15)) << 4));
            const f16x8 rh = __builtin_bit_cast(f16x8, res[it]);
            f16x8 ph = {};
            if constexpr (ACC) ph = __builtin_bit_cast(f16x8, prev[it]);
            f16x8 out;
#pragma unroll
            for (int e = 0; e < 8; ++e) {
                const float a = e < 4 ? a0[e] : a1[e - 4];
                float v = (a + (float)rh[e]) * p.alpha;
                if constexpr (ACC) v += (float)ph[e];
                if (oact) v = v > 0.f ? v : v * p.out_slope;
                out[e] = (_Float16)v;
            }
            __builtin_amdgcn_raw_buffer_store_b128(__builtin_bit_cast(u32x4, out), orsrc, goff[it], 0, 0);
        }
    }
    if constexpr (ACC) issueY(nxt);
    __syncthreads();
    RPW_TL(5)
    RPW_TL_TILE
  }
  RPW_TL_FLUSH
}

template <int C, int R1, int WARPS_M, int WARPS_N, int BKW>
static int respair_wide_launch(si_ctx* ctx, const ResPairParams& p0, hipStream_t st) {
    const ResPairParams& p = p0;
    const int BMo = R1 - (p.k - 1);
    const size_t lds = (size_t)(R1 + RPW_HALO) * C * 2 + 2 * (size_t)C * BKW * 2 + 2 * (size_t)C * 4;
    const bool vl = p0.lens != nullptr;
    auto kern = vl ? (p.accumulate ? respair_wide_kernel<C, R1, WARPS_M, WARPS_N, BKW, true, true> : respair_wide_kernel<C, R1, WARPS_M, WARPS_N, BKW, false, true>)
                   : (p.accumulate ? respair_wide_kernel<C, R1, WARPS_M, WARPS_N, BKW, true, false> : respair_wide_kernel<C, R1, WARPS_M, WARPS_N, BKW, false, false>);
    if (int rc = si_ensure_dyn_lds(ctx, reinterpret_cast<const void*>(kern), lds)) return rc;
    const int total = vl ? (int)si_vl_tiles(p.lens_host, p.B, BMo) : ((p.L + BMo - 1) / BMo) * p.B;
    if (total <= 0) return SI_OK;
    ResPairParams pk = p0;
    pk.total_tiles = total;
    const int grid = std::min(total, si_num_cus(ctx) * (WARPS_M * WARPS_N == 4 ? 2 : 1));
    char name[48];
    snprintf(name, sizeof(name), p.accumulate ? "respair_f16_c%d_acc" : "respair_f16_c%d", C);
    double rows = (double)p.B * p.L;
    if (vl) { rows = 0; for (int b = 0; b < p.B; ++b) rows += p.lens_host[b]; }
    const double elems = rows * C;
    si_prof_begin(ctx, name, 2.0 * 2.0 * elems * C * p.k, elems * (2.0 + 2.0 + (p.accumulate ? 2.0 : 0.0)) + 2.0 * 2.0 * p.k * C * C, st);
    hipLaunchKernelGGL(kern, dim3(grid), dim3(64 * WARPS_M * WARPS_N), lds, st, pk);
    si_prof_end(ctx, st);
    SI_HIP_CHECK(hipGetLastError());
    return SI_OK;
}

int si_launch_respair_wide(si_ctx* ctx, int C, const ResPairParams& p, hipStream_t st) {
    if (C == 128) return respair_wide_launch<128, 256, 4, 2, 128>(ctx, p, st);
    if (C == 256) return respair_wide_launch<256, 128, 2, 4, 64>(ctx, p, st);
    return 1;
}
```

### speech_inpainting_amd/native.py

```python
from __future__ import annotations

import ctypes as C
import os
from typing import Optional, Tuple

import numpy as np
import torch

from .arch import HubertArch, VocoderArch

_HERE = os.path.dirname(os.path.abspath(__file__))
LIB_PATH = os.environ.get("SI_HIP_LIB") or os.path.join(_HERE, "libsi_hip.so")

SI_MATH = {"fp32": 0, "f32": 0, "bf16": 1, "bf16x3": 2, "fp16": 3, "f16": 3}
SI_MAX_CONV, SI_MAX_UPS, SI_MAX_RB, SI_MAX_DIL = 8, 8, 4, 4

EXPORTS = ["si_version", "si_create", "si_destroy", "si_last_error", "si_load_weights", "si_alloc_weights",
           "si_weights_device_ptr", "si_weights_check", "si_workspace_bytes", "si_hubert_forward", "si_hubert_forward_padded", "si_hubert_forward_varlen", "si_hubert_extract_features", "si_code_splice", "si_codebook_splice",
           "si_codebook_splice_varlen", "si_hifigan_forward_varlen", "si_mel_frontend_varlen",
           "si_codebook_splice_labels", "si_codebook_metrics", "si_kmeans_assign", "si_mel_metrics", "si_sisdr", "si_unit_frontend",
           "si_f0_encoder_weight_floats", "si_f0_encoder_frames", "si_f0_encoder_workspace_bytes", "si_f0_encoder_forward",
           "si_resample_poly", "si_resample_sinc", "si_pcm16", "si_extend_mel", "si_hifigan_forward", "si_mel_frames", "si_mel_workspace_bytes", "si_mel_frontend", "si_num_frames",
           "si_vocoder_samples", "si_profile_start", "si_profile_filter", "si_profile_stop",
           "si_debug_capture", "si_debug_size", "si_debug_ws_regions",
           "si_hubert_forward_spans", "si_mel_frontend_spans", "si_codebook_splice_spans", "si_codebook_splice_labels_spans",
           "si_codebook_metrics_spans", "si_wave_peak", "si_gather_windows", "si_patch_compose",
           "si_cut_clips", "si_patch_regions", "si_quiet_runs", "si_patch_rate", "si_cut_rate",
           "si_quiet_runs_ch", "si_cut_rate_ch", "si_patch_rate_ch", "si_dead_runs", "si_level_runs", "si_cut_pair", "si_cut_pair_ch",
           "si_plan_weights", "si_pack_weights_host", "si_burst_runs",
           "si_invalid_runs", "si_cut_rate_valid", "si_cut_pair_valid", "si_cut_clips_valid", "si_mend_runs",
           "si_impulse_runs", "si_impulse_residual"]
SI_MAX_SPANS = 16
SI_MAX_CHANNELS = 8
SAMPLE_F32, SAMPLE_S16, SAMPLE_S24 = 0, 1, 2
DEAD_QUIET, DEAD_HELD = 1, 2
LEVEL_MAX_HALF = 1024
IMPULSE_MAX_ORDER, IMPULSE_MAX_HALF, IMPULSE_MAX_GUARD, IMPULSE_MAX_PAD = 32, 1024, 64, 16
MEND_MAX_LEN, MEND_MAX_ORDER, MEND_MAX_CONTEXT, MEND_MAX_RUNS = 64, 32, 1024, 65536
MEND_LONG, MEND_AR, MEND_LINE, MEND_EDGE, MEND_NEAR, MEND_NONFINITE, MEND_BADROW = 0, 1, 2, 3, 4, 5, 6
MEND_STATUS = ("LONG", "AR", "LINE", "EDGE", "NEAR", "NONFINITE", "BADROW")
CUT_RATE_TILE = 512
CUT_PAIR_FRAMES = 1


def cut_pair_lds_floats(sr: int, reach22: int, reach16: int) -> int:
    return -(-CUT_PAIR_FRAMES * int(sr) // 50) + 2 + 2 * max(int(reach22), int(reach16))


class _F0EncStruct(C.Structure):
    _fields_ = [(n, C.c_int32) for n in ("in_width", "out_width", "width", "n_state", "depth", "down_t", "stride_t", "dilation_growth")]


class F0EncDesc:

    def __init__(self, in_width=1, out_width=128, width=32, depth=4, down_t=4, stride_t=2, dilation_growth=3, m_conv=1.0):
        self.in_width, self.out_width, self.width, self.depth = int(in_width), int(out_width), int(width), int(depth)
        self.down_t, self.stride_t, self.dilation_growth = int(down_t), int(stride_t), int(dilation_growth)
        self.n_state = int(m_conv * width)

    def as_struct(self) -> _F0EncStruct:
        return _F0EncStruct(self.in_width, self.out_width, self.width, self.n_state, self.depth, self.down_t, self.stride_t, self.dilation_growth)

    def down_kernel(self):
        s = self.stride_t
        return (2 * s, s // 2) if s % 2 == 0 else (2 * s + 1, s // 2 + 1)


class SincFilter(C.Structure):
    _fields_ = [("struct_size", C.c_int32), ("nwin", C.c_int32), ("num_table", C.c_int32), ("step", C.c_int32), ("n_time", C.c_int32),
                ("reserved", C.c_int32), ("scale", C.c_double), ("ratio", C.c_double), ("win", C.c_void_p), ("dwin", C.c_void_p),
                ("time_reg", C.c_void_p)]


class SpanTableStruct(C.Structure):
    _fields_ = [("struct_size", C.c_int32), ("num_clips", C.c_int32), ("num_spans", C.c_int32), ("reserved", C.c_int32),
                ("host_off", C.c_void_p), ("host_start", C.c_void_p), ("host_len", C.c_void_p),
                ("span_off", C.c_void_p), ("span_start", C.c_void_p), ("span_len", C.c_void_p)]


class SpanTable:

    @staticmethod
    def words(spans) -> int:
        return len(spans) + 2 + 2 * sum(len(c) for c in spans)

    def __init__(self, spans, device, staged=None):
        from .gaps import csr
        off, st, ln = csr(spans)
        self.B, self.n = len(off) - 1, len(st)
        vals = np.array(off + st + ln + [0], dtype=np.int32)
        if staged is None:
            self.host = np.ascontiguousarray(vals)
            self.dev = torch.from_numpy(self.host).to(device, non_blocking=True)
        else:
            self.host, self.dev = staged
            if self.host.size != vals.size or self.dev.numel() != vals.size:
                raise ValueError(f"SpanTable: staged views of {self.host.size} / {self.dev.numel()} words, the table has {vals.size}")
            np.copyto(self.host, vals)

    def spans(self):
        B, n, h = self.B, self.n, self.host
        return [[(int(h[B + 1 + k]), int(h[B + 1 + n + k])) for k in range(int(h[b]), int(h[b + 1]))] for b in range(B)]

    def struct(self) -> SpanTableStruct:
        h, d, B, n = self.host.ctypes.data, self.dev.data_ptr(), self.B, self.n
        return SpanTableStruct(C.sizeof(SpanTableStruct), B, n, 0, h, h + 4 * (B + 1), h + 4 * (B + 1 + n),
                               d, d + 4 * (B + 1), d + 4 * (B + 1 + n))


class PatchTableStruct(C.Structure):
    _fields_ = [("struct_size", C.c_int32), ("num_clips", C.c_int32), ("num_windows", C.c_int32), ("num_spans", C.c_int32),
                ("fade", C.c_int32), ("reserved", C.c_int32),
                ("host_win_clip", C.c_void_p), ("host_win_start", C.c_void_p), ("host_win_len", C.c_void_p), ("host_span_win", C.c_void_p),
                ("host_lim", C.c_void_p),
                ("win_start", C.c_void_p), ("win_len", C.c_void_p), ("span_win", C.c_void_p), ("lim", C.c_void_p), ("ramp", C.c_void_p)]


class PatchTable:

    @staticmethod
    def words(n_windows: int, n_spans: int, n_clips: int, fade: int) -> int:
        return 3 * n_windows + n_spans + n_clips + fade + 1

    def __init__(self, windows, span_win, lim, fade: int, device, staged=None):
        from .gaps import fade_ramp
        self.W, self.S, self.B, self.fade = len(windows), len(span_win), len(lim), int(fade)
        cols = [[int(w[j]) for w in windows] for j in range(3)]
        ints = np.array(cols[0] + cols[1] + cols[2] + [int(k) for k in span_win] + [int(n) for n in lim], dtype=np.int32)
        vals = np.concatenate([ints, fade_ramp(self.fade).view(np.int32), np.zeros(1, np.int32)])
        if staged is None:
            self.host = np.ascontiguousarray(vals)
            self.dev = torch.from_numpy(self.host).to(device, non_blocking=True)
        else:
            self.host, self.dev = staged
            if self.host.size != vals.size or self.dev.numel() != vals.size:
                raise ValueError(f"PatchTable: staged views of {self.host.size} / {self.dev.numel()} words, the table has {vals.size}")
            np.copyto(self.host, vals)

    def struct(self) -> PatchTableStruct:
        h, d, W, S, B = self.host.ctypes.data, self.dev.data_ptr(), self.W, self.S, self.B
        o = [0, 4 * W, 8 * W, 12 * W, 12 * W + 4 * S, 12 * W + 4 * S + 4 * B]
        return PatchTableStruct(C.sizeof(PatchTableStruct), B, W, S, self.fade, 0, h + o[0], h + o[1], h + o[2], h + o[3], h + o[4],
                                d + o[1], d + o[2], d + o[3], d + o[4], d + o[5])


class RegionTableStruct(C.Structure):
    _HOST = ("start", "len", "span_win", "span_lim", "win_ctx", "win_start", "win_len", "chunk", "k0", "k1")
    _fields_ = ([(n, C.c_int32) for n in ("struct_size", "num_contexts", "num_windows", "num_spans", "num_chunks", "fade")] +
                [("host_" + n, C.c_void_p) for n in _HOST] + [(n, C.c_void_p) for n in _HOST] + [("ramp", C.c_void_p)])


class RegionTable:

    def __init__(self, spans, windows, chunks, n_contexts: int, fade: int, device):
        from .gaps import fade_ramp
        self.K, self.W, self.Q, self.C, self.fade = len(spans), len(windows), len(chunks), int(n_contexts), int(fade)
        cols = [[int(r[j]) for r in rows] for rows, n in ((spans, 4), (windows, 3), (chunks, 3)) for j in range(n)]
        ints = np.array([v for col in cols for v in col], dtype=np.int32)
        self.host = np.ascontiguousarray(np.concatenate([ints, fade_ramp(self.fade).view(np.int32), np.zeros(1, np.int32)]))
        self.dev = torch.from_numpy(self.host).to(device, non_blocking=True)

    def struct(self) -> RegionTableStruct:
        h, d, K, W, Q = self.host.ctypes.data, self.dev.data_ptr(), self.K, self.W, self.Q
        o = [4 * x for x in (0, K, 2 * K, 3 * K, 4 * K, 4 * K + W, 4 * K + 2 * W, 4 * K + 3 * W, 4 * K + 3 * W + Q, 4 * K + 3 * W + 2 * Q,
                             4 * K + 3 * W + 3 * Q)]
        return RegionTableStruct(C.sizeof(RegionTableStruct), self.C, W, K, Q, self.fade, *[h + x for x in o[:10]], *[d + x for x in o[:10]], d + o[10])


class RateTableStruct(C.Structure):
    _HOST = ("start", "len", "span_win", "span_lim", "win_ctx", "win_start", "win_len", "win_lim", "chunk", "k0", "k1")
    _fields_ = ([(n, C.c_int32) for n in ("struct_size", "num_contexts", "num_windows", "num_spans", "num_chunks", "fade")] +
                [("host_" + n, C.c_void_p) for n in _HOST] + [(n, C.c_void_p) for n in _HOST] + [("ramp", C.c_void_p)])


class RateTable:

    def __init__(self, spans, windows, chunks, n_contexts: int, fade: int, device):
        from .gaps import fade_ramp
        self.K, self.W, self.Q, self.C, self.fade = len(spans), len(windows), len(chunks), int(n_contexts), int(fade)
        for what, rows, n in (("span", spans, 4), ("window", windows, 4), ("chunk", chunks, 3)):
            for k, r in enumerate(rows):
                if len(r) != n or any(not -2 ** 31 <= int(v) < 2 ** 31 for v in r):
                    raise ValueError(f"RateTable: {what} {k} = {tuple(r)} is not {n} int32 values")
        cols = [[int(r[j]) for r in rows] for rows, n in ((spans, 4), (windows, 4), (chunks, 3)) for j in range(n)]
# ... 21 lines not shown

class WsRegion(C.Structure):
    _fields_ = [("name", C.c_char * 24), ("offset", C.c_uint64), ("bytes", C.c_uint64)]


class ModelDesc(C.Structure):
    _fields_ = [
        ("struct_size", C.c_int32),
        ("hidden_size", C.c_int32), ("num_layers", C.c_int32), ("num_heads", C.c_int32), ("intermediate_size", C.c_int32),
        ("num_conv", C.c_int32),
        ("conv_dim", C.c_int32 * SI_MAX_CONV), ("conv_kernel", C.c_int32 * SI_MAX_CONV), ("conv_stride", C.c_int32 * SI_MAX_CONV),
        ("conv_bias", C.c_int32), ("feat_norm_layer", C.c_int32), ("stable_layer_norm", C.c_int32),
        ("pos_conv_kernel", C.c_int32), ("pos_conv_groups", C.c_int32), ("feat_proj_layer_norm", C.c_int32),
        ("layer_norm_eps", C.c_float), ("codebook_dim", C.c_int32), ("num_clusters", C.c_int32),
        ("num_mels", C.c_int32), ("num_ups", C.c_int32),
        ("up_rates", C.c_int32 * SI_MAX_UPS), ("up_kernels", C.c_int32 * SI_MAX_UPS), ("up_initial_channel", C.c_int32),
        ("num_rb", C.c_int32), ("rb_kernels", C.c_int32 * SI_MAX_RB), ("num_dil", C.c_int32),
        ("rb_dilations", (C.c_int32 * SI_MAX_DIL) * SI_MAX_RB),
        ("encoder_math", C.c_int32), ("vocoder_math", C.c_int32), ("vocoder_chunk", C.c_int32), ("resblock_type", C.c_int32),
    ]


def make_desc(harch: HubertArch, varch: VocoderArch, num_clusters: int, encoder_math: str = "fp32",
              vocoder_math: str = "fp32", vocoder_chunk: int = 0) -> ModelDesc:
    d = ModelDesc()
    d.struct_size = C.sizeof(ModelDesc)
    d.hidden_size, d.num_layers = harch.hidden_size, harch.num_hidden_layers
    d.num_heads, d.intermediate_size = harch.num_attention_heads, harch.intermediate_size
    n = len(harch.conv_dim)
    if n > SI_MAX_CONV or not (len(harch.conv_kernel) == len(harch.conv_stride) == n):
        raise ValueError("unsupported conv stack")
    d.num_conv = n
    for i in range(n):
        d.conv_dim[i], d.conv_kernel[i], d.conv_stride[i] = harch.conv_dim[i], harch.conv_kernel[i], harch.conv_stride[i]
    d.conv_bias = int(harch.conv_bias)
    if harch.feat_extract_norm not in ("group", "layer"):
        raise ValueError(f"feat_extract_norm={harch.feat_extract_norm!r}")
    d.feat_norm_layer = int(harch.feat_extract_norm == "layer")
    d.stable_layer_norm = int(harch.do_stable_layer_norm)
    d.pos_conv_kernel, d.pos_conv_groups = harch.num_conv_pos_embeddings, harch.num_conv_pos_embedding_groups
    d.feat_proj_layer_norm = int(harch.feat_proj_layer_norm)
    d.layer_norm_eps = harch.layer_norm_eps
    d.codebook_dim, d.num_clusters = harch.codebook_dim, int(num_clusters)
    d.num_mels = varch.num_mels
    nu = len(varch.upsample_rates)
    if nu > SI_MAX_UPS or len(varch.upsample_kernel_sizes) != nu:
        raise ValueError("unsupported upsample stack")
    d.num_ups = nu
    for i in range(nu):
        d.up_rates[i], d.up_kernels[i] = varch.upsample_rates[i], varch.upsample_kernel_sizes[i]
    d.up_initial_channel = varch.upsample_initial_channel
    nr = len(varch.resblock_kernel_sizes)
    nd = len(varch.resblock_dilation_sizes[0])
    if nr > SI_MAX_RB or nd > SI_MAX_DIL or any(len(x) != nd for x in varch.resblock_dilation_sizes):
        raise ValueError("unsupported resblock shape")
    d.num_rb, d.num_dil = nr, nd
    for j in range(nr):
        d.rb_kernels[j] = varch.resblock_kernel_sizes[j]
        for k in range(nd):
            d.rb_dilations[j][k] = varch.resblock_dilation_sizes[j][k]
    d.encoder_math, d.vocoder_math = SI_MATH[encoder_math], SI_MATH[vocoder_math]
    d.vocoder_chunk = int(vocoder_chunk)
    if str(varch.resblock) not in ("1", "2"):
        raise ValueError(f"resblock={varch.resblock!r}: '1' or '2' (I_ea/hifi_gan/models.py:89)")
    d.resblock_type = int(varch.resblock)
    return d


_lib = None


def load_library(path: Optional[str] = None) -> C.CDLL:
    global _lib
    if _lib is not None and path is None:
        return _lib
    p = path or LIB_PATH
    if not os.path.exists(p):
        raise RuntimeError(
            f"{p} is missing: the HIP library has not been built (run `python -c 'import __graft_entry__ as g; g.build()'` "
            "or `make -C speech_inpainting_amd/csrc`).  There is no CPU fallback for the inpainting path.")
    lib = C.CDLL(p)
    vp, i32, sz = C.c_void_p, C.c_int, C.c_size_t
    lib.si_version.restype = i32
    lib.si_create.argtypes = [C.POINTER(vp), i32, C.POINTER(ModelDesc)]
    lib.si_destroy.argtypes = [vp]
    lib.si_destroy.restype = None
    lib.si_last_error.argtypes = [vp]
    lib.si_last_error.restype = C.c_char_p
    lib.si_load_weights.argtypes = [vp, vp, sz, C.c_char_p]
    lib.si_alloc_weights.argtypes = [vp]
    lib.si_weights_device_ptr.argtypes = [vp, C.POINTER(vp), C.POINTER(sz)]
    lib.si_weights_check.argtypes = [vp]
    lib.si_workspace_bytes.argtypes = [vp, i32, i32, i32, C.POINTER(sz)]
    lib.si_hubert_forward.argtypes = [vp, vp, vp, vp, i32, i32, i32, vp, vp, sz, vp]
    lib.si_hubert_forward_padded.argtypes = [vp, vp, vp, vp, vp, i32, i32, i32, vp, vp, sz, vp]
    lib.si_hubert_forward_varlen.argtypes = [vp, vp, vp, vp, vp, i32, i32, i32, vp, vp, sz, vp]
    lib.si_codebook_splice_varlen.argtypes = [vp, vp, i32, i32, vp, vp, i32, vp, i32, vp, vp]
    lib.si_hifigan_forward_varlen.argtypes = [vp, vp, vp, i32, i32, i32, vp, vp, sz, vp]
    lib.si_mel_frontend_varlen.argtypes = [vp, vp, vp, vp, vp, i32, i32, i32, vp, vp, sz, vp]
    lib.si_hubert_extract_features.argtypes = [vp, C.POINTER(ExtractDesc), vp, vp, vp, vp, i32, i32, vp, vp, sz, vp]
    lib.si_code_splice.argtypes = [vp, vp, vp, vp, vp, i32, i32, vp, vp]
    lib.si_codebook_splice.argtypes = [vp, vp, i32, i32, vp, i32, vp, i32, vp, vp]
    lib.si_codebook_splice_labels.argtypes = [vp, vp, i32, vp, i32, vp, i32, vp]
    lib.si_codebook_metrics.argtypes = [vp, vp, i32, i32, vp, i32, vp, vp, vp, vp, vp, vp]
    lib.si_kmeans_assign.argtypes = [vp, vp, C.c_int64, i32, vp, i32, vp, vp, vp]
    lib.si_mel_metrics.argtypes = [vp, vp, vp, i32, i32, i32, vp, vp, vp]
    lib.si_sisdr.argtypes = [vp, vp, vp, i32, i32, vp, vp]
    lib.si_unit_frontend.argtypes = [vp, vp, i32, vp, i32, vp, vp, i32, vp, i32, i32, i32, vp, vp]
    lib.si_f0_encoder_weight_floats.argtypes = [vp]
    lib.si_f0_encoder_weight_floats.restype = C.c_size_t
    lib.si_f0_encoder_frames.argtypes = [vp, i32]
    lib.si_f0_encoder_frames.restype = i32
    lib.si_f0_encoder_workspace_bytes.argtypes = [vp, i32, i32]
    lib.si_f0_encoder_workspace_bytes.restype = C.c_size_t
    lib.si_f0_encoder_forward.argtypes = [vp, vp, vp, vp, i32, i32, vp, vp, C.c_size_t, vp]
    lib.si_resample_poly.argtypes = [vp, vp, i32, i32, vp, i32, i32, i32, i32, i32, vp, vp]
    lib.si_resample_sinc.argtypes = [vp, vp, vp, i32, i32, C.POINTER(SincFilter), i32, vp, vp]
    lib.si_pcm16.argtypes = [vp, vp, C.c_int64, vp, vp]
    lib.si_extend_mel.argtypes = [vp, vp, i32, i32, vp, vp]
    lib.si_hifigan_forward.argtypes = [vp, vp, i32, i32, i32, vp, vp, sz, vp]
    lib.si_mel_frames.argtypes = [i32]
    lib.si_mel_workspace_bytes.argtypes = [vp, i32, i32, C.POINTER(sz)]
    lib.si_mel_frontend.argtypes = [vp, vp, vp, vp, i32, i32, i32, vp, vp, sz, vp]
    lib.si_hubert_forward_spans.argtypes = [vp, vp, C.POINTER(SpanTableStruct), vp, i32, i32, i32, vp, vp, sz, vp]
    lib.si_mel_frontend_spans.argtypes = [vp, vp, C.POINTER(SpanTableStruct), vp, i32, i32, i32, vp, vp, sz, vp]
    lib.si_codebook_splice_spans.argtypes = [vp, vp, i32, i32, vp, vp, i32, vp, i32, vp, vp]
    lib.si_codebook_splice_labels_spans.argtypes = [vp, vp, i32, vp, vp, i32, vp, i32, vp]
    lib.si_codebook_metrics_spans.argtypes = [vp, vp, i32, i32, vp, vp, i32, vp, vp, vp, vp, vp, vp]
    lib.si_wave_peak.argtypes = [vp, vp, C.POINTER(SpanTableStruct), vp, i32, i32, vp, vp]
    lib.si_gather_windows.argtypes = [vp, vp, i32, i32, vp, vp, i32, i32, vp, vp]
    lib.si_patch_compose.argtypes = [vp, vp, C.POINTER(SpanTableStruct), vp, C.POINTER(PatchTableStruct), vp, i32, vp, i32, i32, vp, vp, vp]
    lib.si_cut_clips.argtypes = [vp, vp, i32, vp, vp, i32, i32, vp, vp]
    lib.si_patch_regions.argtypes = [vp, vp, i32, C.POINTER(RegionTableStruct), vp, i32, vp, vp, vp, vp]
    lib.si_quiet_runs.argtypes = [vp, vp, i32, i32, C.c_float, i32, vp, i32, vp, vp]
    lib.si_patch_rate.argtypes = [vp, vp, i32, i32, i32, C.POINTER(RateTableStruct), vp, i32, vp, C.POINTER(SincFilter), vp, vp]
    lib.si_cut_rate.argtypes = [vp, vp, i32, i32, i32, vp, vp, i32, i32, C.POINTER(SincFilter), vp, vp]
    lib.si_quiet_runs_ch.argtypes = [vp, vp, i32, i32, i32, i32, C.c_float, i32, vp, i32, vp, vp]
    lib.si_cut_rate_ch.argtypes = [vp, vp, i32, i32, i32, i32, i32, vp, vp, i32, i32, C.POINTER(SincFilter), vp, vp]
    lib.si_patch_rate_ch.argtypes = [vp, vp, i32, i32, i32, i32, i32, C.POINTER(RateTableStruct), vp, i32, vp, C.POINTER(SincFilter), vp, vp]
    lib.si_dead_runs.argtypes = [vp, vp, i32, i32, i32, i32, i32, C.c_float, C.c_float, C.c_float, i32, vp, i32, vp, vp, vp]
    lib.si_level_runs.argtypes = [vp, vp, i32, i32, i32, i32, i32, C.c_float, C.c_float, i32, vp, i32, vp, vp, vp]
    lib.si_burst_runs.argtypes = [vp, vp, i32, i32, i32, i32, i32, C.c_float, C.c_float, i32, vp, i32, vp, vp, vp]
    lib.si_cut_pair.argtypes = [vp, vp, i32, i32, i32, vp, vp, i32, i32, i32, C.POINTER(SincFilter), C.POINTER(SincFilter), vp, vp, vp]
    lib.si_cut_pair_ch.argtypes = [vp, vp, i32, i32, i32, i32, i32, vp, vp, i32, i32, i32, C.POINTER(SincFilter), C.POINTER(SincFilter), vp, vp, vp]
    lib.si_invalid_runs.argtypes = [vp, vp, i32, i32, i32, i32, C.c_float, i32, vp, i32, vp, vp]
    lib.si_cut_rate_valid.argtypes = [vp, vp, i32, i32, i32, i32, i32, vp, vp, i32, i32, C.POINTER(SincFilter), C.c_float, vp, vp]
    lib.si_cut_pair_valid.argtypes = [vp, vp, i32, i32, i32, i32, i32, vp, vp, i32, i32, i32, C.POINTER(SincFilter), C.POINTER(SincFilter), C.c_float,
                                      vp, vp, vp]
    lib.si_cut_clips_valid.argtypes = [vp, vp, i32, vp, vp, i32, i32, C.c_float, vp, vp]
    lib.si_mend_runs.argtypes = [vp, vp, i32, i32, i32, i32, vp, i32, i32, i32, i32, vp, vp]
    lib.si_impulse_runs.argtypes = [vp, vp, i32, i32, i32, i32, i32, i32, i32, i32, C.c_float, C.c_float, C.c_float, i32, vp, i32, vp, vp, vp]
    lib.si_impulse_residual.argtypes = [vp, vp, i32, i32, i32, i32, i32, vp, vp]
    lib.si_plan_weights.argtypes = [C.POINTER(ModelDesc), C.POINTER(sz)]
    lib.si_pack_weights_host.argtypes = [C.POINTER(ModelDesc), vp, sz, C.c_char_p, vp, sz, C.POINTER(sz), C.c_char_p, sz]
    lib.si_num_frames.argtypes = [vp, i32]
    lib.si_vocoder_samples.argtypes = [vp, i32, i32]
    lib.si_debug_capture.argtypes = [vp, C.c_char_p, vp, C.c_long]
    lib.si_debug_size.argtypes = [vp, C.c_char_p]
    lib.si_debug_size.restype = C.c_long
    lib.si_debug_ws_regions.argtypes = [vp, i32, C.POINTER(WsRegion), i32, C.POINTER(i32)]
    lib.si_profile_start.argtypes = [vp, i32]
    lib.si_profile_filter.argtypes = [vp, C.c_char_p]
    lib.si_profile_stop.argtypes = [vp, C.POINTER(ProfileEntry), i32, C.POINTER(i32)]
    for name in EXPORTS:
        if name not in ("si_destroy", "si_last_error", "si_debug_size"):
            getattr(lib, name).restype = i32
    if path is None:
        _lib = lib
    return lib


class NativeError(RuntimeError):
    pass


def plan_weights(desc: ModelDesc):
    lib = load_library()
    n = C.c_size_t(0)
    rc = lib.si_plan_weights(C.byref(desc), C.byref(n))
    return rc, int(n.value), lib.si_last_error(None).decode()


def pack_weights_host(desc: ModelDesc, blob: np.ndarray, index: str, capacity: Optional[int] = None, slack: int = 0):
    lib = load_library()
    blob = np.ascontiguousarray(blob)
    if capacity is None:
        rc, capacity, msg = plan_weights(desc)
        if rc != 0:
            return rc, np.zeros(0, np.uint8), 0, msg
    out = np.full(int(capacity) + int(slack), 0xA5, dtype=np.uint8)
    need, err = C.c_size_t(0), C.create_string_buffer(512)
    rc = lib.si_pack_weights_host(C.byref(desc), blob.ctypes.data_as(C.c_void_p), blob.nbytes, index.encode(), out.ctypes.data_as(C.c_void_p),
                                  int(capacity), C.byref(need), err, 512)
    return rc, out, int(need.value), err.value.decode()


def _ptr(t: Optional[torch.Tensor]):
    return C.c_void_p(t.data_ptr()) if t is not None else C.c_void_p(0)


def _dev(t: torch.Tensor, dtype: torch.dtype, dim: Optional[int] = None, n: Optional[int] = None) -> torch.Tensor:
    assert t.is_cuda and t.dtype == dtype and t.is_contiguous() and (dim is None or t.dim() == dim) and (n is None or t.numel() == n)
    return t


def _f32(t: torch.Tensor, dim: Optional[int] = None) -> torch.Tensor:
    return _dev(t, torch.float32, dim)


def _i32(t: torch.Tensor, n: Optional[int] = None) -> torch.Tensor:
    return _dev(t, torch.int32, None, n)


def _i64(t: torch.Tensor, n: Optional[int] = None) -> torch.Tensor:
    return _dev(t, torch.int64, None, n)


class NativeContext:

    def __init__(self, desc: ModelDesc, device: torch.device):
        self.lib = load_library()
        if device.type != "cuda":
            raise RuntimeError(f"the HIP path needs a GPU device, got {device} (no CPU fallback)")
        self.device = device
        self.desc = desc
        self._h = C.c_void_p(0)
        idx = device.index if device.index is not None else torch.cuda.current_device()
        rc = self.lib.si_create(C.byref(self._h), idx, C.byref(desc))
        if rc != 0:
            raise NativeError(f"si_create failed ({rc}): {self.lib.si_last_error(None).decode()}")
        self._ws: Optional[torch.Tensor] = None

    def close(self):
        self._wholder = None
        self._ws = None
        self._ws_mel = self._ws_mel_old = None
        if getattr(self, "_h", None) and self._h.value:
            self.lib.si_destroy(self._h)
            self._h = C.c_void_p(0)

    def __del__(self):
        try:
            self.close()
        except Exception:
            pass

    def _check(self, rc: int, what: str):
        if rc != 0:
            raise NativeError(f"{what} failed ({rc}): {self.lib.si_last_error(self._h).decode()}")

    def _stream(self):
        return C.c_void_p(torch.cuda.current_stream(self.device).cuda_stream)

    def load_weights(self, blob: np.ndarray, index: str):
        blob = np.ascontiguousarray(blob)
        self._check(self.lib.si_load_weights(self._h, blob.ctypes.data_as(C.c_void_p), blob.nbytes, index.encode()),
                    "si_load_weights")

    def alloc_weights(self):
        self._check(self.lib.si_alloc_weights(self._h), "si_alloc_weights")

    def weights_check(self):
        self._check(self.lib.si_weights_check(self._h), "si_weights_check")

    def weights_ptr(self):
        p, n = C.c_void_p(0), C.c_size_t(0)
        self._check(self.lib.si_weights_device_ptr(self._h, C.byref(p), C.byref(n)), "si_weights_device_ptr")
        return int(p.value), int(n.value)

    def weights_tensor(self) -> torch.Tensor:
        p, n = C.c_void_p(0), C.c_size_t(0)
        self._check(self.lib.si_weights_device_ptr(self._h, C.byref(p), C.byref(n)), "si_weights_device_ptr")

        class _Holder:
            pass
        h = _Holder()
        h.__cuda_array_interface__ = {"shape": (n.value,), "typestr": "|u1", "data": (p.value, False), "version": 2}
        self._wholder = h
        t = torch.as_tensor(h, device=self.device)
        if t.data_ptr() != p.value or t.numel() != n.value:
            raise NativeError("weights_tensor: torch did not alias the library's weight blob")
        return t

    def num_frames(self, n: int) -> int:
        return int(self.lib.si_num_frames(self._h, n))

    def mel_frames(self, n22: int) -> int:
        return int(self.lib.si_mel_frames(int(n22)))

    def vocoder_samples(self, tm: int, stretch: bool = True) -> int:
        return int(self.lib.si_vocoder_samples(self._h, tm, int(stretch)))

    def workspace(self, B: int, N: int, Tm: int) -> torch.Tensor:
        need = C.c_size_t(0)
        self._check(self.lib.si_workspace_bytes(self._h, B, N, Tm, C.byref(need)), "si_workspace_bytes")
        if self._ws is None or self._ws.numel() < need.value:
            self._ws = None
            self._ws = torch.empty(need.value, dtype=torch.uint8, device=self.device)
        return self._ws

    def _encoder_call(self, name: str, wav: torch.Tensor, width: int, masks, mid, head=(), sample_len=None) -> torch.Tensor:
        B, N = _f32(wav, 2).shape
        lens = None if sample_len is None else self._host_lens(sample_len, B)
        T = self.num_frames(N)
        if T < 1:
            raise ValueError(f"clip of {N} samples is too short")
        for m in masks:
            assert m is None or _i32(m, B) is m
        out = torch.empty(B, T, width, dtype=torch.float32, device=self.device)
        ws = self.workspace(B, N, 0)
        self._check(getattr(self.lib, name)(self._h, *head, _ptr(wav), *mid(None if lens is None else lens.ctypes.data_as(C.c_void_p)), B, N,
                                            _ptr(out), _ptr(ws), ws.numel(), self._stream()), name)
        return out

    def hubert_forward(self, wav: torch.Tensor, mask_start: Optional[torch.Tensor], mask_len: Optional[torch.Tensor],
                       normalize: bool = True, valid_len: Optional[torch.Tensor] = None) -> torch.Tensor:
        return self._encoder_call("si_hubert_forward_padded", wav, self.desc.codebook_dim, (mask_start, mask_len, valid_len),
                                  lambda _: (_ptr(mask_start), _ptr(mask_len), _ptr(valid_len), int(normalize)))

    @staticmethod
    def _host_lens(lens, B: int):
        a = np.ascontiguousarray(np.asarray(lens, dtype=np.int32).reshape(-1))
        if a.size != B:
            raise ValueError(f"ragged batch: {a.size} lengths for {B} clips")
        return a

    def hubert_forward_varlen(self, wav: torch.Tensor, sample_len, mask_start: Optional[torch.Tensor] = None,
                              mask_len: Optional[torch.Tensor] = None, normalize: bool = True) -> torch.Tensor:
        return self._encoder_call("si_hubert_forward_varlen", wav, self.desc.codebook_dim, (mask_start, mask_len),
                                  lambda lens: (_ptr(mask_start), _ptr(mask_len), lens, int(normalize)), sample_len=sample_len)

    def codebook_splice_varlen(self, feats: torch.Tensor, frame_pos: torch.Tensor, frame_cnt: torch.Tensor, lm: int, mel: torch.Tensor) -> torch.Tensor:
        B, T, Tm = self._feats_mel(feats, mel)
# ... 588 lines not shown
```

Baseline: 11040 x real-time (audio-sec/wall-sec); `value` = whole-job aggregate over n_gpus, `value_per_gpu` = the per-GPU figure the metric names.

## Merge HiFi-GAN resblock conv pairs across kernel sizes into one multi-problem launch

The fused residual conv-pair kernel now takes up to three problems, one per resblock kernel size, in a single grouped launch. Tiles from all problems share one persistent grid, and each tile looks up its weights, bias, dilation and input from its problem. This cuts launch count and fills the GPU better for the short vocoder stages. In exchange the workspace grows with extra per-problem intermediate buffers, and the merged path skips the existing three-dilation chain kernel for the affected stages.

Result: no change. 11070 x real-time (audio-sec/wall-sec); `value` = whole-job aggregate over n_gpus, `value_per_gpu` = the per-GPU figure the metric names, median of 6 (+0.3%).

```diff
diff --git a/include/si_hip.h b/include/si_hip.h
--- a/include/si_hip.h
+++ b/include/si_hip.h
@@ -400,6 +400,8 @@
 } si_ws_region;
 int si_debug_ws_regions(si_ctx* ctx, int which, si_ws_region* out, int capacity, int* count);
 
+int si_respair_tile_table(int C, int B, int L, const int32_t* lens, int nprob, const int32_t* k, int32_t* table, int capacity, int32_t* counts);
+
 #ifdef __cplusplus
 }
 #endif
diff --git a/speech_inpainting_amd/csrc/api.hip b/speech_inpainting_amd/csrc/api.hip
--- a/speech_inpainting_amd/csrc/api.hip
+++ b/speech_inpainting_amd/csrc/api.hip
@@ -40,6 +40,7 @@
     int opt_ffn_pad = 64;
     int opt_gemmcu = 1;
     int opt_voc_chain = 1;
+    int opt_voc_merge = 1;
     int opt_voc_fuse = 1;
     char* fe_dev = nullptr;
     size_t fe_dft = 0, fe_hann = 0, fe_basis = 0, fe_lo = 0, fe_hi = 0;
@@ -175,6 +176,7 @@
     return Carver{static_cast<char*>(workspace), workspace_bytes, ctx->ws_zone, &ctx->ws_log[which], ctx->ws_zone};
 }
 constexpr int ENC_WS_ZONES = 18, VOC_WS_ZONES = 15, MEL_WS_ZONES = 5;
+constexpr int VOC_MID_SETS = SI_RESPAIR_MAX_PROBLEMS;
 
 struct VlTable { const int32_t* host = nullptr; int32_t* dev = nullptr; };
 template <class Fill>
@@ -222,7 +224,7 @@
     size_t lc_max = (size_t)Tout * d.up_initial_channel;
     long L = Tout; int c = d.up_initial_channel;
     for (int i = 0; i < d.num_ups; ++i) { L *= d.up_rates[i]; c = stage_channels(ctx, i); lc_max = std::max(lc_max, (size_t)L * c); }
-    const size_t f = (size_t)Bc * Tout * ctx->lay.mel_ld + 9 * (size_t)Bc * lc_max;
+    const size_t f = (size_t)Bc * Tout * ctx->lay.mel_ld + (9 + (VOC_MID_SETS - 1)) * (size_t)Bc * lc_max;
     return f * 4 + 32 * 256 + align_up((size_t)(2 * SI_MAX_UPS + 3) * B * 4, 256) +
            VOC_WS_ZONES * ctx->ws_zone;
 }
@@ -309,6 +311,7 @@
     ctx->popt = pack_opts_from_env();
     ctx->opt_voc_fuse = getenv("SI_VOC_FUSE") ? atoi(getenv("SI_VOC_FUSE")) : 1;
     ctx->opt_voc_chain = getenv("SI_VOC_CHAIN") ? atoi(getenv("SI_VOC_CHAIN")) : 1;
+    ctx->opt_voc_merge = getenv("SI_VOC_MERGE") ? atoi(getenv("SI_VOC_MERGE")) : 1;
     ctx->opt_enc_opready = env_flag("SI_ENC_OPREADY");
     ctx->opt_att_bf16 = env_flag("SI_ATT_BF16");
     ctx->opt_enc_lingemm = env_flag("SI_ENC_LINGEMM");
@@ -1023,7 +1026,7 @@
     const size_t nbuf = (size_t)Bc_max * lc_max;
     float* buf_ws[6] = {W.floats(nbuf, "buf0"), W.floats(nbuf, "buf1"), W.floats(nbuf, "buf2"), W.floats(nbuf, "buf3"), W.floats(nbuf, "buf4"), W.floats(nbuf, "buf5")};
     char* const h16_raw[6] = {W.bytes(nbuf * 2, "h16_0"), W.bytes(nbuf * 2, "h16_1"), W.bytes(nbuf * 2, "h16_2"),
-                              W.bytes(nbuf * 2, "h16_3"), W.bytes(nbuf * 2, "h16_4"), W.bytes(nbuf * 2, "h16_5")};
+                              W.bytes(nbuf * 2, "h16_3"), W.bytes(VOC_MID_SETS * nbuf * 2, "h16_4"), W.bytes(VOC_MID_SETS * nbuf * 2, "h16_5")};
     unsigned short* h16_ws[6];
     for (int i = 0; i < 6; ++i) h16_ws[i] = reinterpret_cast<unsigned short*>(h16_raw[i]);
     const bool opr = ctx->popt.voc_opready && (d.vocoder_math == SI_MATH_BF16 || d.vocoder_math == SI_MATH_F16);
@@ -1119,13 +1122,41 @@
                 return BlockOut{last ? 1.0f / nk : 1.f, last && j > 0, r16 || !last || (completes && i + 1 < d.num_ups),
                                 (r16 && !(completes && act_next)) ? 1.f : 0.1f};
             };
+            const bool merge = ctx->opt_voc_merge && r16 && d.resblock_type != 2 && (fuse_mask & cout) && cout >= 64 && si_respair_tile_rows(cout) &&
+                               nk >= 2 && nk <= SI_RESPAIR_MAX_PROBLEMS && d.num_dil >= 2;
+            auto mid16 = [&](int j, int n) { return h16[4 + (n & 1)] + (merge ? (size_t)j * nbuf : 0); };
+            int n_merged = 0;
+            if (merge) {
+                int order[SI_MAX_RB];
+                for (int j = 0; j < nk; ++j) order[j] = j;
+                std::stable_sort(order, order + nk, [&](int a, int b) { return d.rb_kernels[a] > d.rb_kernels[b]; });
+                for (int n = 0; n + 1 < d.num_dil; ++n) {
+                    ResPairParams mp{};
+                    mp.nprob = nk; mp.B = Bc; mp.L = (int)Lo; mp.lens = dLs(i + 1); mp.lens_host = hLs(i + 1);
+                    for (int q = 0; q < nk; ++q) {
+                        const int j = order[q];
+                        const ResW& R = Ly.rbs[(size_t)i * nk + j];
+                        const TapGemmParams w1 = gemm_params(ctx, R.c1[n]), w2 = gemm_params(ctx, R.c2[n]);
+                        const BlockOut o = block_out(j, false);
+                        mp.pr[q] = ResPairProblem{n == 0 ? U16 : mid16(j, n - 1), mid16(j, n), static_cast<const unsigned short*>(w1.w),
+                                                  static_cast<const unsigned short*>(w2.w), w1.bias, w2.bias, d.rb_kernels[j], d.rb_dilations[j][n],
+                                                  o.alpha, o.accumulate, o.slope16, 0, 0};
+                    }
+                    const int mrc = si_launch_respair_multi(ctx, cout, mp, st);
+                    if (mrc < 0) return mrc;
+                    if (mrc > 0) break;
+                    for (int j = 0; j < nk; ++j)
+                        if ((rc = tap16(mid16(j, n), nst, "stage%d.rb%d.p%d.f16", i, j, n))) return rc;
+                    n_merged = n + 1;
+                }
+            }
             for (int j = 0; j < nk; ++j) {
                 const ResW& R = Ly.rbs[(size_t)i * nk + j];
                 const int rk = d.rb_kernels[j];
                 const float* y = U;
-                const unsigned short* y16 = U16;
+                const unsigned short* y16 = n_merged ? mid16(j, n_merged - 1) : U16;
                 const BlockOut whole = block_out(j, true);
-                if (r16 && d.resblock_type != 2 && (fuse_mask & cout) && ctx->opt_voc_chain && d.num_dil == 3 && whole.slope16 == 1.f) {
+                if (!n_merged && r16 && d.resblock_type != 2 && (fuse_mask & cout) && ctx->opt_voc_chain && d.num_dil == 3 && whole.slope16 == 1.f) {
                     ResChainParams cp{};
                     cp.y16 = U16; cp.out16 = xs16; cp.B = Bc; cp.L = (int)Lo; cp.k = rk; cp.alpha = whole.alpha; cp.accumulate = whole.accumulate;
                     cp.lens = dLs(i + 1); cp.lens_host = hLs(i + 1);
@@ -1141,11 +1172,11 @@
                         continue;
                     }
                 }
-                for (int n = 0; n < d.num_dil; ++n) {
+                for (int n = n_merged; n < d.num_dil; ++n) {
                     const int dl = d.rb_dilations[j][n];
                     const bool last = (n == d.num_dil - 1);
                     float* ynext = last ? xs : buf[4 + (n & 1)];
-                    unsigned short* ynext16 = last ? xs16 : h16[4 + (n & 1)];
+                    unsigned short* ynext16 = last ? xs16 : mid16(j, n);
                     const BlockOut o = block_out(j, last);
                     auto residual_conv = [&](const GemmW& G, int dil, float slope, const float* in, const unsigned short* in16) {
                         TapGemmParams q = stage_conv(G, i + 1, Lo, cout, cout, dil);
diff --git a/speech_inpainting_amd/csrc/common.h b/speech_inpainting_amd/csrc/common.h
--- a/speech_inpainting_amd/csrc/common.h
+++ b/speech_inpainting_amd/csrc/common.h
@@ -1,6 +1,7 @@
 #pragma once
 #include <hip/hip_runtime.h>
 #include <stdint.h>
+#include <stdio.h>
 
 #include <type_traits>
 
@@ -364,21 +365,63 @@
 };
 int si_launch_upsample_stream(si_ctx* ctx, const UpsampleParams& p, hipStream_t st);
 
-struct ResPairParams {
+constexpr int SI_RESPAIR_MAX_PROBLEMS = 3;
+struct ResPairProblem {
     const unsigned short* y16;
     unsigned short* out16;
     const unsigned short* w1;
     const unsigned short* w2;
     const float* b1;
     const float* b2;
-    int B, L, k, dil;
+    int k, dil;
     float alpha;
     int accumulate;
+    float out_slope;
+    int tiles, tiles_x;
+};
+struct ResPairParams {
+    ResPairProblem pr[SI_RESPAIR_MAX_PROBLEMS];
+    int nprob;
+    int B, L;
     const int32_t* lens; const int32_t* lens_host;
     int total_tiles;
-    float out_slope;
-};
+};
+struct SiPairTile { int problem, local; };
+__host__ __device__ inline SiPairTile si_respair_problem_of(int tiles0, int tiles1, int t) {
+    const int c1 = tiles0 + tiles1;
+    const int pi = (t >= tiles0) + (t >= c1);
+    return {pi, t - (pi == 0 ? 0 : pi == 1 ? tiles0 : c1)};
+}
+constexpr int si_respair_tile_rows(int C) { return C == 32 ? 256 : C == 64 ? 512 : C == 128 ? 256 : C == 256 ? 128 : 0; }
+inline long si_respair_count_tiles(ResPairParams& p, int R1) {
+    long total = 0;
+    for (int q = 0; q < SI_RESPAIR_MAX_PROBLEMS; ++q) {
+        ResPairProblem& r = p.pr[q];
+        r.tiles = r.tiles_x = 0;
+        if (q >= p.nprob) continue;
+        const int BMo = R1 - (r.k - 1);
+        r.tiles_x = (p.L + BMo - 1) / BMo;
+        const long n = p.lens_host ? si_vl_tiles(p.lens_host, p.B, BMo) : (long)r.tiles_x * p.B;
+        r.tiles = (int)n;
+        total += n;
+    }
+    p.total_tiles = (int)total;
+    return total;
+}
+struct SiPairWork { double flops, bytes; };
+inline SiPairWork si_respair_work(const ResPairParams& p, int C) {
+    double rows = (double)p.B * p.L;
+    if (p.lens_host) { rows = 0; for (int b = 0; b < p.B; ++b) rows += p.lens_host[b]; }
+    const double elems = rows * C;
+    SiPairWork w{0, 0};
+    for (int q = 0; q < p.nprob; ++q) {
+        w.flops += 2.0 * 2.0 * elems * C * p.pr[q].k;
+        w.bytes += elems * (2.0 + 2.0 + (p.pr[q].accumulate ? 2.0 : 0.0)) + 2.0 * 2.0 * p.pr[q].k * C * C;
+    }
+    return w;
+}
 int si_launch_respair_wide(si_ctx* ctx, int C, const ResPairParams& p, hipStream_t st);
+int si_launch_respair_multi(si_ctx* ctx, int C, const ResPairParams& p, hipStream_t st);
 struct ResChainParams {
     const unsigned short* y16;
     unsigned short* out16;
diff --git a/speech_inpainting_amd/csrc/respair.hip b/speech_inpainting_amd/csrc/respair.hip
--- a/speech_inpainting_amd/csrc/respair.hip
+++ b/speech_inpainting_amd/csrc/respair.hip
@@ -47,27 +47,29 @@
     const int tid = threadIdx.x, lane = tid & 63, wave = tid >> 6;
     const int r16 = lane & 15, kg = lane >> 4;
     const int wm0 = wave * 64;
-    const int k = p.k, d = p.dil;
-    const int p1 = d * (k - 1) / 2, p2 = (k - 1) / 2;
-    const int BMo = R1 - (k - 1);
-    const int R0 = R1 + (k - 1) * d;
-    const int tiles_x = (p.L + BMo - 1) / BMo;
-    const int total = VL ? p.total_tiles : tiles_x * p.B;
-    auto tile_of = [&](int t, int& tb, int& tm0, int& tL) {
-        if constexpr (VL) { const SiVlTile v = si_vl_tile(p.lens, p.B, BMo, t); tb = v.b; tm0 = v.row0; tL = v.L; }
-        else { tb = t / tiles_x; tm0 = (t - tb * tiles_x) * BMo; tL = p.L; }
-    };
-    const __amdgpu_buffer_rsrc_t w1rsrc = __builtin_amdgcn_make_buffer_rsrc(const_cast<unsigned short*>(p.w1), 0, k * C * C * 2, 0x00020000);
-    const __amdgpu_buffer_rsrc_t w2rsrc = __builtin_amdgcn_make_buffer_rsrc(const_cast<unsigned short*>(p.w2), 0, k * C * C * 2, 0x00020000);
-
-    const int NS1 = (k + TPS - 1) / TPS, NS = 2 * NS1;
+    const int total = p.total_tiles;
+    const int tiles0 = p.pr[0].tiles, tiles1 = p.pr[1].tiles;
+    auto problem_of = [&](int t, int& local) -> const ResPairProblem& {
+        const SiPairTile pt = si_respair_problem_of(tiles0, tiles1, t);
+        local = pt.local;
+        return p.pr[__builtin_amdgcn_readfirstlane(pt.problem)];
+    };
+    auto tile_of = [&](const ResPairProblem& q, int local, int& tb, int& tm0, int& tL) {
+        const int bmo = R1 - (q.k - 1);
+        if constexpr (VL) {
+            const SiVlTile v = si_vl_tile(p.lens, p.B, bmo, local);
+            tb = __builtin_amdgcn_readfirstlane(v.b); tm0 = __builtin_amdgcn_readfirstlane(v.row0); tL = __builtin_amdgcn_readfirstlane(v.L);
+        }
+        else { tb = local / q.tiles_x; tm0 = (local - tb * q.tiles_x) * bmo; tL = p.L; }
+    };
+
     u32x4 rw[WSLOTS];
-    auto issueW = [&](int s) {
-        const bool second = s >= NS1;
-        const int soff = __builtin_amdgcn_readfirstlane((second ? s - NS1 : s) * WBYTES);
-#pragma unroll
-        for (int i = 0; i < WSLOTS; ++i)
-            rw[i] = __builtin_amdgcn_raw_buffer_load_b128(second ? w2rsrc : w1rsrc, (tid + i * NT) * 16, soff, 0);
+    auto issueW0 = [&](int t) {
+        int local;
+        const ResPairProblem& q = problem_of(t, local);
+        const __amdgpu_buffer_rsrc_t rs = __builtin_amdgcn_make_buffer_rsrc(const_cast<unsigned short*>(q.w1), 0, q.k * C * C * 2, 0x00020000);
+#pragma unroll
+        for (int i = 0; i < WSLOTS; ++i) rw[i] = __builtin_amdgcn_raw_buffer_load_b128(rs, (tid + i * NT) * 16, 0, 0);
     };
     auto storeW = [&](char* dst) {
 #pragma unroll
@@ -83,30 +85,51 @@
     const int yc = tid % CPR, yr0 = tid / CPR;
     u32x4 ry[YSLOTS];
     auto issueY = [&](int t) {
-        int tb, tm0, tL;
-        tile_of(t, tb, tm0, tL);
-        const int trow0 = tm0 - p2 - p1;
-        const __amdgpu_buffer_rsrc_t rs = __builtin_amdgcn_make_buffer_rsrc(const_cast<unsigned short*>(p.y16 + (long)tb * p.L * C), 0, tL * C * 2, 0x00020000);
+        int local, tb, tm0, tL;
+        const ResPairProblem& q = problem_of(t, local);
+        tile_of(q, local, tb, tm0, tL);
+        const int trow0 = tm0 - (q.k - 1) / 2 - q.dil * (q.k - 1) / 2;
+        const __amdgpu_buffer_rsrc_t rs = __builtin_amdgcn_make_buffer_rsrc(const_cast<unsigned short*>(q.y16 + (long)tb * p.L * C), 0, tL * C * 2, 0x00020000);
 #pragma unroll
         for (int i = 0; i < YSLOTS; ++i)
             ry[i] = __builtin_amdgcn_raw_buffer_load_b128(rs, ((trow0 + yr0 + i * YRPP) * C + 8 * yc) * 2, 0, 0);
     };
-
-    issueW(0);
+    const int bwhich = (tid / (C / 4)) & 1, bc4 = (tid % (C / 4)) * 4;
+    f32x4 rb;
+    auto issueB = [&](int t) {
+        int local;
+        const ResPairProblem& q = problem_of(t, local);
+        rb = *reinterpret_cast<const f32x4*>((bwhich ? q.b2 : q.b1) + bc4);
+    };
+
+    issueW0(blockIdx.x);
     issueY(blockIdx.x);
-    if (tid < C / 2) {
-        const int which = tid / (C / 4), c4 = (tid % (C / 4)) * 4;
-        *reinterpret_cast<f32x4*>(Bs + which * C + c4) = *reinterpret_cast<const f32x4*>((which ? p.b2 : p.b1) + c4);
-    }
+    issueB(blockIdx.x);
 
   for (int tile = blockIdx.x; tile < total; tile += gridDim.x) {
     const int nxt = tile + (int)gridDim.x < total ? tile + (int)gridDim.x : tile;
-    int b, m0, Lb;
-    tile_of(tile, b, m0, Lb);
+    int tlocal, b, m0, Lb;
+    const ResPairProblem& pq = problem_of(tile, tlocal);
+    tile_of(pq, tlocal, b, m0, Lb);
+    const int k = pq.k, d = pq.dil;
+    const int p2 = (k - 1) / 2;
+    const int BMo = R1 - (k - 1);
+    const int R0 = R1 + (k - 1) * d;
+    const int NS1 = (k + TPS - 1) / TPS, NS = 2 * NS1;
+    const float alpha = pq.alpha;
     const int t_row0 = m0 - p2;
     const long seg = (long)b * p.L * C;
-    const __amdgpu_buffer_rsrc_t yrsrc = __builtin_amdgcn_make_buffer_rsrc(const_cast<unsigned short*>(p.y16 + seg), 0, Lb * C * 2, 0x00020000);
-    const __amdgpu_buffer_rsrc_t orsrc = __builtin_amdgcn_make_buffer_rsrc(p.out16 + seg, 0, Lb * C * 2, 0x00020000);
+    const __amdgpu_buffer_rsrc_t yrsrc = __builtin_amdgcn_make_buffer_rsrc(const_cast<unsigned short*>(pq.y16 + seg), 0, Lb * C * 2, 0x00020000);
+    const __amdgpu_buffer_rsrc_t orsrc = __builtin_amdgcn_make_buffer_rsrc(pq.out16 + seg, 0, Lb * C * 2, 0x00020000);
+    const __amdgpu_buffer_rsrc_t w1rsrc = __builtin_amdgcn_make_buffer_rsrc(const_cast<unsigned short*>(pq.w1), 0, k * C * C * 2, 0x00020000);
+    const __amdgpu_buffer_rsrc_t w2rsrc = __builtin_amdgcn_make_buffer_rsrc(const_cast<unsigned short*>(pq.w2), 0, k * C * C * 2, 0x00020000);
+    auto issueW = [&](int s) {
+        const bool second = s >= NS1;
+        const int soff = __builtin_amdgcn_readfirstlane((second ? s - NS1 : s) * WBYTES);
+#pragma unroll
+        for (int i = 0; i < WSLOTS; ++i)
+            rw[i] = __builtin_amdgcn_raw_buffer_load_b128(second ? w2rsrc : w1rsrc, (tid + i * NT) * 16, soff, 0);
+    };
 
     storeW(Ws);
     issueW(1);
@@ -119,6 +142,7 @@
             *reinterpret_cast<f16x8*>(Ys + r * YS + (YPAD ? yc << 4 : (yc << 4) ^ rpn_swz<ROWB>(r))) = h;
         }
     }
+    if (tid < C / 2) *reinterpret_cast<f32x4*>(Bs + bwhich * C + bc4) = rb;
     __syncthreads();
 
     f32x4 acc[4][TN];
@@ -179,7 +203,7 @@
         const int q = second ? s - NS1 : s;
         const int tap0 = q * TPS;
         if (s == NS - 1) {
-            issueW(0);
+            issueW0(nxt);
             if constexpr (!ACC) issueY(nxt);
         }
         compute(tap0, second, min(TPS, k - tap0), Ws + (s & 1) * WBYTES);
@@ -250,6 +274,7 @@
         }
     }
     __syncthreads();
+    issueB(nxt);
     {
 #pragma unroll
         for (int it = 0; it < OPASS; ++it) {
@@ -263,7 +288,7 @@
 #pragma unroll
             for (int e = 0; e < 8; ++e) {
                 const float a = e < 4 ? a0[e] : a1[e - 4];
-                float v = (a + (float)rh[e]) * p.alpha;
+                float v = (a + (float)rh[e]) * alpha;
                 if constexpr (ACC) v += (float)ph[e];
                 out[e] = (_Float16)v;
             }
@@ -277,38 +302,79 @@
 
 template <int C, int R1, int WARPS_M, int TPS>
 static int respair_launch(si_ctx* ctx, const ResPairParams& p, hipStream_t st) {
-    const int BMo = R1 - (p.k - 1);
+    static_assert(R1 == si_respair_tile_rows(C), "the host-side tile table counts with the kernel's tile height");
     const size_t lds = (size_t)(R1 + RPN_HALO) * (C * 2 + (C == 64 ? 32 : 0)) + 2 * (size_t)TPS * C * C * 2 + 2 * (size_t)C * 4;
-    const bool vl = p.lens != nullptr;
-    auto kern = vl ? (p.accumulate ? respair_kernel<C, R1, WARPS_M, TPS, true, true> : respair_kernel<C, R1, WARPS_M, TPS, false, true>)
-                   : (p.accumulate ? respair_kernel<C, R1, WARPS_M, TPS, true, false> : respair_kernel<C, R1, WARPS_M, TPS, false, false>);
+    const bool vl = p.lens != nullptr, acc = p.pr[0].accumulate != 0;
+    auto kern = vl ? (acc ? respair_kernel<C, R1, WARPS_M, TPS, true, true> : respair_kernel<C, R1, WARPS_M, TPS, false, true>)
+                   : (acc ? respair_kernel<C, R1, WARPS_M, TPS, true, false> : respair_kernel<C, R1, WARPS_M, TPS, false, false>);
     if (int rc = si_ensure_dyn_lds(ctx, reinterpret_cast<const void*>(kern), lds)) return rc;
-    const int total = vl ? (int)si_vl_tiles(p.lens_host, p.B, BMo) : ((p.L + BMo - 1) / BMo) * p.B;
+    ResPairParams pk = p;
+    const int total = (int)si_respair_count_tiles(pk, R1);
     if (total <= 0) return SI_OK;
-    ResPairParams pk = p;
-    pk.total_tiles = total;
     const int grid = std::min(total, si_num_cus(ctx) * (WARPS_M == 4 ? 2 : 1));
     char name[48];
-    snprintf(name, sizeof(name), p.accumulate ? "respair_f16_c%d_acc" : "respair_f16_c%d", C);
-    double rows = (double)p.B * p.L;
-    if (vl) { rows = 0; for (int b = 0; b < p.B; ++b) rows += p.lens_host[b]; }
-    const double elems = rows * C;
-    si_prof_begin(ctx, name, 2.0 * 2.0 * elems * C * p.k, elems * (2.0 + 2.0 + (p.accumulate ? 2.0 : 0.0)) + 2.0 * 2.0 * p.k * C * C, st);
+    snprintf(name, sizeof(name), acc ? "respair_f16_c%d_acc" : "respair_f16_c%d", C);
+    const SiPairWork work = si_respair_work(pk, C);
+    si_prof_begin(ctx, name, work.flops, work.bytes, st);
     hipLaunchKernelGGL(kern, dim3(grid), dim3(64 * WARPS_M), lds, st, pk);
     si_prof_end(ctx, st);
     SI_HIP_CHECK(hipGetLastError());
     return SI_OK;
 }
 
+int si_launch_respair_multi(si_ctx* ctx, int C, const ResPairParams& p, hipStream_t st) {
+    if (p.nprob < 1 || p.nprob > SI_RESPAIR_MAX_PROBLEMS) return si_fail(ctx, SI_EINVAL, "respair: %d problems in one launch (1..%d)", p.nprob, SI_RESPAIR_MAX_PROBLEMS);
+    if ((C != 32 && C != 64 && C != 128 && C != 256) || ((long)p.L + 1024) * C * 2 >= (1L << 31)) return 1;
+    for (int q = 0; q < p.nprob; ++q) {
+        const ResPairProblem& r = p.pr[q];
+        if (r.k < 3 || r.k > 11 || (r.k & 1) == 0 || (r.k - 1) * r.dil > 50 || !r.b1 || !r.b2) return 1;
+        if (r.out_slope != 1.f && C < 128) return 1;
+        if ((r.accumulate != 0) != (p.pr[0].accumulate != 0)) return si_fail(ctx, SI_EINVAL, "respair: the problems of one launch accumulate or none does");
+        if (q > 0 && r.k > p.pr[q - 1].k) return si_fail(ctx, SI_EINVAL, "respair: the problems of one launch are listed in descending kernel size");
+    }
+    if ((p.lens == nullptr) != (p.lens_host == nullptr)) return si_fail(ctx, SI_EINVAL, "respair: ragged batches need the lengths on the device and on the host");
+    if (C >= 128) return si_launch_respair_wide(ctx, C, p, st);
+    return C == 32 ? respair_launch<32, 256, 4, 11>(ctx, p, st) : respair_launch<64, 512, 8, 4>(ctx, p, st);
+}
+
 int si_launch_respair(si_ctx* ctx, int C, const unsigned short* y16, unsigned short* out16, const void* w1, const void* w2,
                       const float* b1, const float* b2, int B, int L, int k, int dil, float alpha, int accumulate, hipStream_t st,
                       const int32_t* lens, const int32_t* lens_host, float out_slope) {
-    if ((C != 32 && C != 64 && C != 128 && C != 256) || k < 3 || k > 11 || (k & 1) == 0 || (k - 1) * dil > 50 ||
-        ((long)L + 1024) * C * 2 >= (1L << 31)) return 1;
-    if (!b1 || !b2) return 1;
-    if ((lens == nullptr) != (lens_host == nullptr)) return si_fail(ctx, SI_EINVAL, "respair: ragged batches need the lengths on the device and on the host");
-    ResPairParams p{y16, out16, static_cast<const unsigned short*>(w1), static_cast<const unsigned short*>(w2), b1, b2, B, L, k, dil, alpha, accumulate, lens, lens_host, 0, out_slope};
-    if (out_slope != 1.f && C < 128) return 1;
-    if (C >= 128) return si_launch_respair_wide(ctx, C, p, st);
-    return C == 32 ? respair_launch<32, 256, 4, 11>(ctx, p, st) : respair_launch<64, 512, 8, 4>(ctx, p, st);
-}
+    ResPairParams p{};
+    p.pr[0] = ResPairProblem{y16, out16, static_cast<const unsigned short*>(w1), static_cast<const unsigned short*>(w2), b1, b2, k, dil, alpha, accumulate, out_slope, 0, 0};
+    p.nprob = 1; p.B = B; p.L = L; p.lens = lens; p.lens_host = lens_host;
+    return si_launch_respair_multi(ctx, C, p, st);
+}
+
+extern "C" int si_respair_tile_table(int C, int B, int L, const int32_t* lens, int nprob, const int32_t* k, int32_t* table, int capacity,
+                                     int32_t* counts) {
+    const int R1 = si_respair_tile_rows(C);
+    if (!R1 || B < 1 || L < 1 || nprob < 1 || nprob > SI_RESPAIR_MAX_PROBLEMS || !k || capacity < 0 || (capacity > 0 && !table)) return SI_EINVAL;
+    ResPairParams p{};
+    p.nprob = nprob; p.B = B; p.L = L; p.lens_host = lens;
+    for (int q = 0; q < nprob; ++q) {
+        if (k[q] < 3 || k[q] > 11 || (k[q] & 1) == 0) return SI_EINVAL;
+        p.pr[q].k = k[q];
+    }
+    const long total = si_respair_count_tiles(p, R1);
+    for (int q = 0; q < SI_RESPAIR_MAX_PROBLEMS; ++q) if (counts) counts[q] = p.pr[q].tiles;
+    for (int t = 0; t < total && t < capacity; ++t) {
+        const SiPairTile pt = si_respair_problem_of(p.pr[0].tiles, p.pr[1].tiles, t);
+        const int BMo = R1 - (k[pt.problem] - 1);
+        int clip = 0, row0 = 0;
+        if (lens) {
+            int left = pt.local;
+            for (clip = 0; clip < B; ++clip) {
+                const int nb = lens[clip] > 0 ? (lens[clip] + BMo - 1) / BMo : 0;
+                if (left < nb) break;
+                left -= nb;
+            }
+            row0 = left * BMo;
+        } else {
+            clip = pt.local / p.pr[pt.problem].tiles_x;
+            row0 = (pt.local - clip * p.pr[pt.problem].tiles_x) * BMo;
+        }
+        table[3 * t] = pt.problem; table[3 * t + 1] = clip; table[3 * t + 2] = row0;
+    }
+    return (int)total;
+}
diff --git a/speech_inpainting_amd/csrc/respair_wide.hip b/speech_inpainting_amd/csrc/respair_wide.hip
--- a/speech_inpainting_amd/csrc/respair_wide.hip
+++ b/speech_inpainting_amd/csrc/respair_wide.hip
@@ -68,26 +68,86 @@
     const int tid = threadIdx.x, lane = tid & 63, wave = tid >> 6;
     const int r16 = lane & 15, kg = lane >> 4;
     const int wm0 = (wave / WARPS_N) * 64, wn0 = (wave % WARPS_N) * 64;
-    const int k = p.k, d = p.dil;
-    const int p1 = d * (k - 1) / 2, p2 = (k - 1) / 2;
+    const int total = p.total_tiles;
+    const int tiles0 = p.pr[0].tiles, tiles1 = p.pr[1].tiles;
+    auto problem_of = [&](int t, int& local) -> const ResPairProblem& {
+        const SiPairTile pt = si_respair_problem_of(tiles0, tiles1, t);
+        local = pt.local;
+        return p.pr[__builtin_amdgcn_readfirstlane(pt.problem)];
+    };
+    auto tile_of = [&](const ResPairProblem& q, int local, int& tb, int& tm0, int& tL) {
+        const int bmo = R1 - (q.k - 1);
+        if constexpr (VL) {
+            const SiVlTile v = si_vl_tile(p.lens, p.B, bmo, local);
+            tb = __builtin_amdgcn_readfirstlane(v.b); tm0 = __builtin_amdgcn_readfirstlane(v.row0); tL = __builtin_amdgcn_readfirstlane(v.L);
+        }
+        else { tb = local / q.tiles_x; tm0 = (local - tb * q.tiles_x) * bmo; tL = p.L; }
+    };
+
+    const int wc = tid % CPRW, wr0 = tid / CPRW;
+    u32x4 rw[WSLOTS];
+    auto issueW0 = [&](int t) {
+        int local;
+        const ResPairProblem& q = problem_of(t, local);
+        const __amdgpu_buffer_rsrc_t rs = __builtin_amdgcn_make_buffer_rsrc(const_cast<unsigned short*>(q.w1), 0, q.k * C * C * 2, 0x00020000);
+#pragma unroll
+        for (int i = 0; i < WSLOTS; ++i) rw[i] = __builtin_amdgcn_raw_buffer_load_b128(rs, ((wr0 + i * WRPP) * C + 8 * wc) * 2, 0, 0);
+    };
+    auto storeW1 = [&](char* dst, int i) {
+        const int n = wr0 + i * WRPP;
+        *reinterpret_cast<u32x4*>(dst + n * ROWBW + ((wc << 4) ^ swz16<ROWBW>(n))) = rw[i];
+    };
+    auto storeW = [&](char* dst) {
+#pragma unroll
+        for (int i = 0; i < WSLOTS; ++i) storeW1(dst, i);
+    };
+    const int yc = tid % CPRY, yr0 = tid / CPRY;
+    u32x4 ry[YSLOTS];
+    auto issueY = [&](int t) {
+        int local, tb, tm0, tL;
+        const ResPairProblem& q = problem_of(t, local);
+        tile_of(q, local, tb, tm0, tL);
+        const int trow0 = tm0 - (q.k - 1) / 2 - q.dil * (q.k - 1) / 2;
+        const __amdgpu_buffer_rsrc_t rs = __builtin_amdgcn_make_buffer_rsrc(const_cast<unsigned short*>(q.y16 + (long)tb * p.L * C), 0, tL * C * 2, 0x00020000);
+#pragma unroll
+        for (int i = 0; i < YSLOTS; ++i)
+            ry[i] = __builtin_amdgcn_raw_buffer_load_b128(rs, ((trow0 + yr0 + i * YRPP) * C + 8 * yc) * 2, 0, 0);
+    };
+
+    const int bwhich = (tid / (C / 4)) & 1, bc4 = (tid % (C / 4)) * 4;
+    f32x4 rb;
+    auto issueB = [&](int t) {
+        int local;
+        const ResPairProblem& q = problem_of(t, local);
+        rb = *reinterpret_cast<const f32x4*>((bwhich ? q.b2 : q.b1) + bc4);
+    };
+    const int preW = (wn0 + r16) * ROWBW + (swz16<ROWBW>(wn0 + r16) ^ (kg << 4));
+    issueW0(blockIdx.x);
+    issueY(blockIdx.x);
+    issueB(blockIdx.x);
+    RPW_TL_DECL
+
+  for (int tile = blockIdx.x; tile < total; tile += gridDim.x) {
+    const int nxt = tile + (int)gridDim.x < total ? tile + (int)gridDim.x : tile;
+    int tlocal, b, m0, Lb;
+    const ResPairProblem& pq = problem_of(tile, tlocal);
+    tile_of(pq, tlocal, b, m0, Lb);
+    const int k = pq.k, d = pq.dil;
+    const int p2 = (k - 1) / 2;
     const int BMo = R1 - (k - 1);
     const int R0 = R1 + (k - 1) * d;
-    const int tiles_x = (p.L + BMo - 1) / BMo;
-    const int total = VL ? p.total_tiles : tiles_x * p.B;
-    auto tile_of = [&](int t, int& tb, int& tm0, int& tL) {
-        if constexpr (VL) { const SiVlTile v = si_vl_tile(p.lens, p.B, BMo, t); tb = v.b; tm0 = v.row0; tL = v.L; }
-        else { tb = t / tiles_x; tm0 = (t - tb * tiles_x) * BMo; tL = p.L; }
-    };
-    const __amdgpu_buffer_rsrc_t w1rsrc = __builtin_amdgcn_make_buffer_rsrc(const_cast<unsigned short*>(p.w1), 0, k * C * C * 2, 0x00020000);
-    const __amdgpu_buffer_rsrc_t w2rsrc = __builtin_amdgcn_make_buffer_rsrc(const_cast<unsigned short*>(p.w2), 0, k * C * C * 2, 0x00020000);
-
     const int NS1 = k * NCH, NS = 2 * NS1;
-    const int wc = tid % CPRW, wr0 = tid / CPRW;
-    u32x4 rw[WSLOTS];
+    const float alpha = pq.alpha, out_slope = pq.out_slope;
+    const int t_row0 = m0 - p2;
+    const long seg = (long)b * p.L * C;
+    const __amdgpu_buffer_rsrc_t yrsrc = __builtin_amdgcn_make_buffer_rsrc(const_cast<unsigned short*>(pq.y16 + seg), 0, Lb * C * 2, 0x00020000);
+    const __amdgpu_buffer_rsrc_t orsrc = __builtin_amdgcn_make_buffer_rsrc(pq.out16 + seg, 0, Lb * C * 2, 0x00020000);
+    const __amdgpu_buffer_rsrc_t w1rsrc = __builtin_amdgcn_make_buffer_rsrc(const_cast<unsigned short*>(pq.w1), 0, k * C * C * 2, 0x00020000);
+    const __amdgpu_buffer_rsrc_t w2rsrc = __builtin_amdgcn_make_buffer_rsrc(const_cast<unsigned short*>(pq.w2), 0, k * C * C * 2, 0x00020000);
     auto issueW1 = [&](int s, int i) {
         const bool second = s >= NS1;
-        const int q = second ? s - NS1 : s;
-        const int tap = q / NCH, ch = q - tap * NCH;
+        const int sq = second ? s - NS1 : s;
+        const int tap = sq / NCH, ch = sq - tap * NCH;
         const int soff = __builtin_amdgcn_readfirstlane((tap * C * C + ch * BKW) * 2);
         const int n = wr0 + i * WRPP;
         rw[i] = __builtin_amdgcn_raw_buffer_load_b128(second ? w2rsrc : w1rsrc, (n * C + 8 * wc) * 2, soff, 0);
@@ -96,43 +156,6 @@
 #pragma unroll
         for (int i = 0; i < WSLOTS; ++i) issueW1(s, i);
     };
-    auto storeW1 = [&](char* dst, int i) {
-        const int n = wr0 + i * WRPP;
-        *reinterpret_cast<u32x4*>(dst + n * ROWBW + ((wc << 4) ^ swz16<ROWBW>(n))) = rw[i];
-    };
-    auto storeW = [&](char* dst) {
-#pragma unroll
-        for (int i = 0; i < WSLOTS; ++i) storeW1(dst, i);
-    };
-    const int yc = tid % CPRY, yr0 = tid / CPRY;
-    u32x4 ry[YSLOTS];
-    auto issueY = [&](int t) {
-        int tb, tm0, tL;
-        tile_of(t, tb, tm0, tL);
-        const int trow0 = tm0 - p2 - p1;
-        const __amdgpu_buffer_rsrc_t rs = __builtin_amdgcn_make_buffer_rsrc(const_cast<unsigned short*>(p.y16 + (long)tb * p.L * C), 0, tL * C * 2, 0x00020000);
-#pragma unroll
-        for (int i = 0; i < YSLOTS; ++i)
-            ry[i] = __builtin_amdgcn_raw_buffer_load_b128(rs, ((trow0 + yr0 + i * YRPP) * C + 8 * yc) * 2, 0, 0);
-    };
-
-    if (tid < C / 2) {
-        const int which = tid / (C / 4), c4 = (tid % (C / 4)) * 4;
-        *reinterpret_cast<f32x4*>(Bs + which * C + c4) = *reinterpret_cast<const f32x4*>((which ? p.b2 : p.b1) + c4);
-    }
-    const int preW = (wn0 + r16) * ROWBW + (swz16<ROWBW>(wn0 + r16) ^ (kg << 4));
-    issueW(0);
-    issueY(blockIdx.x);
-    RPW_TL_DECL
-
-  for (int tile = blockIdx.x; tile < total; tile += gridDim.x) {
-    const int nxt = tile + (int)gridDim.x < total ? tile + (int)gridDim.x : tile;
-    int b, m0, Lb;
-    tile_of(tile, b, m0, Lb);
-    const int t_row0 = m0 - p2;
-    const long seg = (long)b * p.L * C;
-    const __amdgpu_buffer_rsrc_t yrsrc = __builtin_amdgcn_make_buffer_rsrc(const_cast<unsigned short*>(p.y16 + seg), 0, Lb * C * 2, 0x00020000);
-    const __amdgpu_buffer_rsrc_t orsrc = __builtin_amdgcn_make_buffer_rsrc(p.out16 + seg, 0, Lb * C * 2, 0x00020000);
 
     storeW(Ws);
     issueW(1);
@@ -145,6 +168,7 @@
             *reinterpret_cast<f16x8*>(Ys + r * ROWBY + ((yc << 4) ^ swz16<ROWBY>(r))) = h;
         }
     }
+    if (tid < C / 2) *reinterpret_cast<f32x4*>(Bs + bwhich * C + bc4) = rb;
     __syncthreads();
     RPW_TL(0)
 
@@ -280,9 +304,10 @@
     RPW_TL_W1(1)
     __syncthreads();
     RPW_TL(4)
-    issueW(0);
+    issueW0(nxt);
+    issueB(nxt);
     {
-        const bool oact = p.out_slope != 0.f && p.out_slope != 1.f;
+        const bool oact = out_slope != 0.f && out_slope != 1.f;
 #pragma unroll
         for (int it = 0; it < OPASS; ++it) {
             const int o = or0 + it * ORPP;
@@ -295,9 +320,9 @@
 #pragma unroll
             for (int e = 0; e < 8; ++e) {
                 const float a = e < 4 ? a0[e] : a1[e - 4];
-                float v = (a + (float)rh[e]) * p.alpha;
+                float v = (a + (float)rh[e]) * alpha;
                 if constexpr (ACC) v += (float)ph[e];
-                if (oact) v = v > 0.f ? v : v * p.out_slope;
+                if (oact) v = v > 0.f ? v : v * out_slope;
                 out[e] = (_Float16)v;
             }
             __builtin_amdgcn_raw_buffer_store_b128(__builtin_bit_cast(u32x4, out), orsrc, goff[it], 0, 0);
@@ -312,25 +337,21 @@
 }
 
 template <int C, int R1, int WARPS_M, int WARPS_N, int BKW>
-static int respair_wide_launch(si_ctx* ctx, const ResPairParams& p0, hipStream_t st) {
-    const ResPairParams& p = p0;
-    const int BMo = R1 - (p.k - 1);
+static int respair_wide_launch(si_ctx* ctx, const ResPairParams& p, hipStream_t st) {
+    static_assert(R1 == si_respair_tile_rows(C), "the host-side tile table counts with the kernel's tile height");
     const size_t lds = (size_t)(R1 + RPW_HALO) * C * 2 + 2 * (size_t)C * BKW * 2 + 2 * (size_t)C * 4;
-    const bool vl = p0.lens != nullptr;
-    auto kern = vl ? (p.accumulate ? respair_wide_kernel<C, R1, WARPS_M, WARPS_N, BKW, true, true> : respair_wide_kernel<C, R1, WARPS_M, WARPS_N, BKW, false, true>)
-                   : (p.accumulate ? respair_wide_kernel<C, R1, WARPS_M, WARPS_N, BKW, true, false> : respair_wide_kernel<C, R1, WARPS_M, WARPS_N, BKW, false, false>);
+    const bool vl = p.lens != nullptr, acc = p.pr[0].accumulate != 0;
+    auto kern = vl ? (acc ? respair_wide_kernel<C, R1, WARPS_M, WARPS_N, BKW, true, true> : respair_wide_kernel<C, R1, WARPS_M, WARPS_N, BKW, false, true>)
+                   : (acc ? respair_wide_kernel<C, R1, WARPS_M, WARPS_N, BKW, true, false> : respair_wide_kernel<C, R1, WARPS_M, WARPS_N, BKW, false, false>);
     if (int rc = si_ensure_dyn_lds(ctx, reinterpret_cast<const void*>(kern), lds)) return rc;
-    const int total = vl ? (int)si_vl_tiles(p.lens_host, p.B, BMo) : ((p.L + BMo - 1) / BMo) * p.B;
+    ResPairParams pk = p;
+    const int total = (int)si_respair_count_tiles(pk, R1);
     if (total <= 0) return SI_OK;
-    ResPairParams pk = p0;
-    pk.total_tiles = total;
     const int grid = std::min(total, si_num_cus(ctx) * (WARPS_M * WARPS_N == 4 ? 2 : 1));
     char name[48];
-    snprintf(name, sizeof(name), p.accumulate ? "respair_f16_c%d_acc" : "respair_f16_c%d", C);
-    double rows = (double)p.B * p.L;
-    if (vl) { rows = 0; for (int b = 0; b < p.B; ++b) rows += p.lens_host[b]; }
-    const double elems = rows * C;
-    si_prof_begin(ctx, name, 2.0 * 2.0 * elems * C * p.k, elems * (2.0 + 2.0 + (p.accumulate ? 2.0 : 0.0)) + 2.0 * 2.0 * p.k * C * C, st);
+    snprintf(name, sizeof(name), acc ? "respair_f16_c%d_acc" : "respair_f16_c%d", C);
+    const SiPairWork work = si_respair_work(pk, C);
+    si_prof_begin(ctx, name, work.flops, work.bytes, st);
     hipLaunchKernelGGL(kern, dim3(grid), dim3(64 * WARPS_M * WARPS_N), lds, st, pk);
     si_prof_end(ctx, st);
     SI_HIP_CHECK(hipGetLastError());
diff --git a/speech_inpainting_amd/native.py b/speech_inpainting_amd/native.py
--- a/speech_inpainting_amd/native.py
+++ b/speech_inpainting_amd/native.py
@@ -29,7 +29,7 @@
            "si_quiet_runs_ch", "si_cut_rate_ch", "si_patch_rate_ch", "si_dead_runs", "si_level_runs", "si_cut_pair", "si_cut_pair_ch",
            "si_plan_weights", "si_pack_weights_host", "si_burst_runs",
            "si_invalid_runs", "si_cut_rate_valid", "si_cut_pair_valid", "si_cut_clips_valid", "si_mend_runs",
-           "si_impulse_runs", "si_impulse_residual"]
+           "si_impulse_runs", "si_impulse_residual", "si_respair_tile_table"]
 SI_MAX_SPANS = 16
 SI_MAX_CHANNELS = 8
 SAMPLE_F32, SAMPLE_S16, SAMPLE_S24 = 0, 1, 2
@@ -357,6 +357,7 @@
     lib.si_impulse_runs.argtypes = [vp, vp, i32, i32, i32, i32, i32, i32, i32, i32, C.c_float, C.c_float, C.c_float, i32, vp, i32, vp, vp, vp]
     lib.si_impulse_residual.argtypes = [vp, vp, i32, i32, i32, i32, i32, vp, vp]
     lib.si_plan_weights.argtypes = [C.POINTER(ModelDesc), C.POINTER(sz)]
+    lib.si_respair_tile_table.argtypes = [i32, i32, i32, vp, i32, vp, vp, i32, vp]
     lib.si_pack_weights_host.argtypes = [C.POINTER(ModelDesc), vp, sz, C.c_char_p, vp, sz, C.POINTER(sz), C.c_char_p, sz]
     lib.si_num_frames.argtypes = [vp, i32]
     lib.si_vocoder_samples.argtypes = [vp, i32, i32]
@@ -384,6 +385,20 @@
     n = C.c_size_t(0)
     rc = lib.si_plan_weights(C.byref(desc), C.byref(n))
     return rc, int(n.value), lib.si_last_error(None).decode()
+
+
+def respair_tile_table(C_: int, B: int, L: int, ks, lens=None):
+    lib = load_library()
+    k = np.asarray(ks, dtype=np.int32)
+    ln = None if lens is None else np.ascontiguousarray(lens, dtype=np.int32)
+    lp = C.c_void_p(0) if ln is None else ln.ctypes.data_as(C.c_void_p)
+    counts = np.zeros(3, dtype=np.int32)
+    total = lib.si_respair_tile_table(C_, B, L, lp, len(k), k.ctypes.data_as(C.c_void_p), C.c_void_p(0), 0, counts.ctypes.data_as(C.c_void_p))
+    if total < 0:
+        raise ValueError(f"si_respair_tile_table refused C={C_} B={B} L={L} k={list(ks)}: {total}")
+    table = np.zeros((max(total, 1), 3), dtype=np.int32)
+    lib.si_respair_tile_table(C_, B, L, lp, len(k), k.ctypes.data_as(C.c_void_p), table.ctypes.data_as(C.c_void_p), total, counts.ctypes.data_as(C.c_void_p))
+    return table[:total], counts
 
 
 def pack_weights_host(desc: ModelDesc, blob: np.ndarray, index: str, capacity: Optional[int] = None, slack: int = 0):
```
